# ArmingLou/seed-vc

Hardware: AMD Instinct MI355X
Metric: mel_frames_per_sec (higher is better)
Workload: dtype f16; 1 GPU; seed-uvit-tat-xlsr-tiny CFM 25 steps cfg 0.7 + HiFT, batch 64 x (P=430,S=430) per GPU; batch_per_gpu=64, global_batch=64, prompt_frames=430, diffusion_steps=25, vocoder_precision=fp16p8, lanes_per_gpu=2, parallelism=utterance-sharded x1, audio gather on rank 0

## Files before the change

### include/seedvc_hip.h

```cpp
#ifndef SEEDVC_HIP_H
#define SEEDVC_HIP_H

#include <stdint.h>

#ifdef __cplusplus
extern "C" {
#endif

#define SVC_ABI_VERSION 1

typedef struct svc_tensor_desc {
    const char* name;
    const float* data;
    int ndim;
    int64_t shape[4];
} svc_tensor_desc_t;

typedef struct svc_dit_config {
    int version;
    int hidden_dim, num_heads, depth, in_channels, content_dim, style_dim;
    int final_layer_type;
    int time_as_token, style_as_token, uvit_skip_connection, long_skip_connection, style_condition;
    int wn_hidden_dim, wn_num_layers, wn_kernel_size, wn_dilation_rate;
} svc_dit_config_t;

typedef struct svc_dit svc_dit_t;

int svc_dit_create(const svc_dit_config_t* cfg, const svc_tensor_desc_t* weights, int n_weights,
                   void* stream, svc_dit_t** out);
void svc_dit_destroy(svc_dit_t* m);

int svc_dit_set_microbatch(svc_dit_t* m, int utterances);

int svc_dit_set_fused_min_rows(svc_dit_t* m, long rows);
int svc_dit_fused_available(svc_dit_t* m);
int svc_dit_set_graphs(svc_dit_t* m, int on);

typedef struct svc_cfm_args {
    int B;
    int T;
    int P;
    const float* mu;
    const float* prompt;
    const float* style;
    const float* z;
    const int64_t* x_lens;
    const int64_t* prompt_lens;
    int n_timesteps;
    float temperature;
    float cfg_rate[2];
    int random_voice;
    float* out;
} svc_cfm_args_t;

int svc_cfm_sample(svc_dit_t* m, const svc_cfm_args_t* args, void* stream);

int svc_cfm_sample_seeded(svc_dit_t* m, const svc_cfm_args_t* args, const uint64_t* seeds, void* stream);
int svc_cfm_noise_draws(uint64_t seed, int C, int T, float* z, void* stream);

int svc_dit_forward(svc_dit_t* m, int N, int T, const float* x, const float* prompt_x, const int64_t* x_lens,
                    float t, const float* style, const float* mu, float* out, void* stream);

typedef struct svc_bigvgan_config {
    int num_mels, upsample_initial_channel, num_upsamples, num_kernels;
    int upsample_rates[8], upsample_kernel_sizes[8];
    int resblock_kernel_sizes[4], resblock_dilation_sizes[4][3];
    int use_tanh_at_final, use_bias_at_final, snake_logscale, snakebeta;
    int precision;
} svc_bigvgan_config_t;
typedef struct svc_bigvgan svc_bigvgan_t;
int svc_bigvgan_create(const svc_bigvgan_config_t* cfg, const svc_tensor_desc_t* weights, int n_weights,
                       void* stream, svc_bigvgan_t** out);
void svc_bigvgan_destroy(svc_bigvgan_t* m);
int svc_bigvgan_forward(svc_bigvgan_t* m, const float* mel, int B, int S, float* out, void* stream);
int svc_bigvgan_forward_ragged(svc_bigvgan_t* m, const float* mel, const int32_t* lens, int B, int S, float* out, void* stream);

typedef struct svc_hift_config {
    int in_channels, base_channels, nb_harmonics, sampling_rate;
    float nsf_alpha, nsf_sigma, nsf_voiced_threshold;
    int num_upsamples, upsample_rates[4], upsample_kernel_sizes[4];
    int istft_n_fft, istft_hop;
    int num_kernels, resblock_kernel_sizes[4], resblock_dilation_sizes[4][3];
    int source_resblock_kernel_sizes[4], source_resblock_dilation_sizes[4][3];
    float lrelu_slope, audio_limit;
    int f0_cond_channels;
    int precision;
} svc_hift_config_t;
typedef struct svc_hift svc_hift_t;
int svc_hift_create(const svc_hift_config_t* cfg, const svc_tensor_desc_t* weights, int n_weights,
                    void* stream, svc_hift_t** out);
void svc_hift_destroy(svc_hift_t* m);
int svc_hift_forward(svc_hift_t* m, const float* mel, const float* f0, const float* phase0, const float* noise,
                     int B, int S, float* out, float* f0_out, void* stream);
int svc_hift_forward_ragged(svc_hift_t* m, const float* mel, const int32_t* lens, const float* f0, const float* phase0,
                            const float* noise, int B, int S, float* out, float* f0_out, void* stream);
int svc_hift_forward_seeded(svc_hift_t* m, const float* mel, const int32_t* lens, const float* f0, const uint64_t* seeds, int B,
                            int S, float* out, float* f0_out, void* stream);
int svc_hift_noise_draws(uint64_t seed, int NH, long n, float* phase0, float* noise, void* stream);
int svc_bigvgan_set_microbatch(svc_bigvgan_t* m, int utterances);
int svc_hift_set_microbatch(svc_hift_t* m, int utterances);

typedef struct svc_ar_config {
    int dim, n_head, n_local_heads, head_dim, n_layer, intermediate_size, vocab_size, max_seq_len;
    float rope_base, norm_eps;
} svc_ar_config_t;
typedef struct svc_ar svc_ar_t;
int svc_ar_create(const svc_ar_config_t* cfg, const svc_tensor_desc_t* weights, int n_weights, void* stream, svc_ar_t** out);
void svc_ar_destroy(svc_ar_t* m);
int svc_ar_reset(svc_ar_t* m, void* stream);
int svc_ar_forward_generate(svc_ar_t* m, const float* x, int S, const int64_t* input_pos, const int64_t* kv_pos,
                            float* logits_out, void* stream);
int svc_ar_decode_step(svc_ar_t* m, const float* x, int set_pos, int64_t input_pos, int64_t kv_pos, float* logits_out,
                       void* stream);
int svc_ar_generate(svc_ar_t* m, const float* x_prefill, int S, const int64_t* input_pos, const int64_t* kv_pos,
                    const float* exp_noise, int max_new, int min_tokens_before_eos, float temperature, float top_p,
                    float repetition_penalty, int check_every, int32_t* tokens_out, int32_t* n_tokens, void* stream);
int svc_ar_set_max_batch(svc_ar_t* m, int max_batch, void* stream);
int svc_ar_prefill_slot(svc_ar_t* m, int slot, const float* x, int S, const int64_t* input_pos, const int64_t* kv_pos,
                        float* logits_out, void* stream);
int svc_ar_decode_step_batch(svc_ar_t* m, int B, const float* x, int set_pos, const int64_t* input_pos, const int64_t* kv_pos,
                             float* logits_out, void* stream);
int svc_ar_generate_batch(svc_ar_t* m, int B, const float* x_prefill, const int32_t* S, const int64_t* input_pos,
                          const int64_t* kv_pos, const float* exp_noise, int max_new, int min_tokens_before_eos, float temperature,
                          float top_p, float repetition_penalty, int check_every, int32_t* tokens_out, int32_t* n_tokens,
                          void* stream);
int svc_ar_generate_batch_seeded(svc_ar_t* m, int B, const float* x_prefill, const int32_t* S, const int64_t* input_pos,
                                 const int64_t* kv_pos, const uint64_t* seeds, int max_new, int min_tokens_before_eos,
                                 float temperature, float top_p, float repetition_penalty, int check_every, int32_t* tokens_out,
                                 int32_t* n_tokens, void* stream);
int svc_ar_exp_draws(svc_ar_t* m, uint64_t seed, int step0, int n_steps, float* out, void* stream);
int svc_ar_prefill_batch(svc_ar_t* m, int n, const int32_t* slots, const float* x, const int32_t* S, const int64_t* input_pos,
                         const int64_t* kv_pos, float* logits_out, void* stream);
int svc_ar_set_prefill_rows(svc_ar_t* m, int rows);
int svc_ar_prefill_passes(svc_ar_t* m);
typedef struct svc_ar_request {
    int32_t slot;
    int32_t S;
    const float* exp_noise;
    uint64_t seed;
    int32_t max_new;
    int32_t min_tokens_before_eos;
    float temperature, top_p, repetition_penalty;
    int32_t* tokens_out;
} svc_ar_request_t;
int svc_ar_admit(svc_ar_t* m, int n, const svc_ar_request_t* requests, const float* x_prefill, const int64_t* input_pos,
                 const int64_t* kv_pos, void* stream);
int svc_ar_run(svc_ar_t* m, int n_steps, int32_t* n_tokens, int32_t* done, void* stream);
int svc_ar_retire(svc_ar_t* m, int slot, void* stream);
int svc_ar_session_active(svc_ar_t* m);
int svc_ar_sample(svc_ar_t* m, const float* logits, const int32_t* prev_tokens, int n_prev, int suppress_token,
                  float temperature, float top_p, float repetition_penalty, const float* exp_noise, int32_t* idx_out,
                  float* probs_out, void* stream);

typedef struct svc_lr_config {
    int channels, in_channels, out_channels;
    int is_discrete, codebook_size;
    int n_convs;
    int interpolate;
    int has_final_conv;
    int f0_condition, n_f0_bins;
} svc_lr_config_t;
typedef struct svc_lr svc_lr_t;
int svc_lr_create(const svc_lr_config_t* cfg, const svc_tensor_desc_t* weights, int n_weights, void* stream, svc_lr_t** out);
void svc_lr_destroy(svc_lr_t* m);
int svc_lr_forward(svc_lr_t* m, const float* x, const int64_t* tokens, const int32_t* in_lens, int B, int tin_max,
                   const int32_t* ylens, int tout_max, const float* f0, const int32_t* f0_lens, int tf0_max, float* out,
                   void* stream);

int svc_v2_assemble_cond(const float* prompt_cond, const int32_t* prompt_lens, const float* cond, const int32_t* cond_lens, int B,
                         int Pmax, int Smax, int Dc, int T, float* out, void* stream);
int svc_mel_strip_prompt(const float* mel, const int32_t* prompt_lens, const int32_t* x_lens, int B, int C, int T, int Smax,
                         float pad_value, float* out, void* stream);

int svc_anti_alias_act_fwd(const void* x, void* y, const float* up12, const float* down12,
                           const float* log_alpha, const float* log_beta, int B, int C, int L, int dtype,
                           void* stream);

typedef struct svc_mel svc_mel_t;
int svc_mel_create(int n_fft, int hop, int win, int n_mels, const float* window, const float* mel_basis, void* stream,
                   svc_mel_t** out);
void svc_mel_destroy(svc_mel_t* m);
int svc_mel_frames(const svc_mel_t* m, int L);
int svc_mel_forward(svc_mel_t* m, const float* y, int B, int L, float* out, void* stream);
int svc_mel_min_len(int n_fft, int hop);
int svc_mel_forward_ragged(svc_mel_t* m, const float* y, const int32_t* lens, int B, int L, float pad_value, float* out, void* stream);

typedef struct svc_resampler svc_resampler_t;
int svc_resampler_create(int o, int n, int width, int ntaps, const int32_t* first, const float* taps, void* stream,
                         svc_resampler_t** out);
void svc_resampler_destroy(svc_resampler_t* r);
long svc_resample_len(int o, int n, long L);
long svc_resampler_tile(const svc_resampler_t* r);
int svc_resample(svc_resampler_t* r, const float* x, const int32_t* lens, int B, long L, float* out, long Lout, void* stream);

typedef struct svc_campplus_config {
    int feat_dim, embedding_size, growth_rate, bn_size, init_channels, m_channels;
    int n_blocks, block_layers[4], block_kernel[4], block_dilation[4];
    int seg_len;
} svc_campplus_config_t;
typedef struct svc_campplus svc_campplus_t;
int svc_campplus_create(const svc_campplus_config_t* cfg, const svc_tensor_desc_t* weights, int n_weights, void* stream,
                        svc_campplus_t** out);
void svc_campplus_destroy(svc_campplus_t* m);
int svc_campplus_forward(svc_campplus_t* m, const float* feat, int B, int T, float* out, void* stream);
int svc_kaldi_fbank_frames(int n_samples);
int svc_kaldi_fbank(svc_campplus_t* m, const float* wave, int n_samples, float* out, void* stream);
int svc_kaldi_fbank_ragged(svc_campplus_t* m, const float* wave, const int32_t* lens, int B, int L, int subtract_mean, float* out,
                           void* stream);
int svc_campplus_forward_ragged(svc_campplus_t* m, const float* feat, const int32_t* lens, int B, int T, float* out, void* stream);

typedef struct svc_rmvpe_config {
    int n_mels;
    int en_de_layers;
    int inter_layers;
    int n_blocks;
    int en_out_channels;
    int gru_hidden;
    int n_bins;
} svc_rmvpe_config_t;
typedef struct svc_rmvpe svc_rmvpe_t;
int svc_rmvpe_create(const svc_rmvpe_config_t* cfg, const svc_tensor_desc_t* weights, int n_weights, const float* mel_basis, void* stream,
                     svc_rmvpe_t** out);
void svc_rmvpe_destroy(svc_rmvpe_t* m);
int svc_rmvpe_frames(int n_samples);
int svc_rmvpe_min_len(void);
int svc_rmvpe_set_plane_budget(svc_rmvpe_t* m, long long bytes);
int svc_rmvpe_set_timing(svc_rmvpe_t* m, int on);
int svc_rmvpe_last_timing(svc_rmvpe_t* m, float* ms4);
int svc_rmvpe_mel(svc_rmvpe_t* m, const float* wave, const int32_t* lens, int B, int L, float* mel_out, void* stream);
int svc_rmvpe_salience(svc_rmvpe_t* m, const float* mel, const int32_t* frame_lens, int B, int T, float* out, void* stream);
int svc_rmvpe_decode(const float* salience, const int32_t* frame_lens, int B, int T, float thred, float* f0_out, void* stream);
int svc_rmvpe_f0(svc_rmvpe_t* m, const float* wave, const int32_t* lens, int B, int L, float thred, float* f0_out, void* stream);
int svc_f0_adjust(const float* f0_alt, const int32_t* alt_lens, const float* f0_ori, const int32_t* ori_lens, int B, int Talt, int Tori,
                  int auto_adjust, const float* semitones, float* out, float* medians, void* stream);

typedef struct svc_whisper_config {
    int n_mels, d_model, n_heads, n_layers, ffn_dim, max_source_positions, precision;
} svc_whisper_config_t;
typedef struct svc_whisper svc_whisper_t;

int svc_whisper_create(const svc_whisper_config_t* cfg, const svc_tensor_desc_t* weights, int n_weights, const float* mel_basis, void* stream,
                       svc_whisper_t** out);
void svc_whisper_destroy(svc_whisper_t* m);
int svc_whisper_n_windows(int P, int overlap_rows, long n_samples);
int svc_whisper_rows(int P, int overlap_rows, long n_samples);
int svc_whisper_set_window_group(svc_whisper_t* m, int windows);
int svc_whisper_set_timing(svc_whisper_t* m, int on);
int svc_whisper_last_timing(svc_whisper_t* m, float* ms4);
int svc_whisper_mel(svc_whisper_t* m, const float* wave, const int32_t* lens, int B, int L, float* feat, void* stream);
int svc_whisper_encode(svc_whisper_t* m, const float* feat, int B, float* out, void* stream);
int svc_whisper_content(svc_whisper_t* m, const float* wave, const int32_t* lens, int B, int L, int overlap_rows, float* out, int Rmax,
                        void* stream);

typedef struct svc_w2v_config {
    int conv_dim, n_conv, conv_kernel[8], conv_stride[8];
    int d_model, n_heads, n_layers, ffn_dim, pos_k, pos_groups;
    int feat_extract_norm_layer, do_stable_layer_norm, conv_bias;
    int window_samples;
    int precision;
} svc_w2v_config_t;
typedef struct svc_w2v svc_w2v_t;

int svc_w2v_create(const svc_w2v_config_t* cfg, const svc_tensor_desc_t* weights, int n_weights, void* stream, svc_w2v_t** out);
void svc_w2v_destroy(svc_w2v_t* m);
long svc_w2v_frames(const svc_w2v_config_t* cfg, long n_samples);
int svc_w2v_n_windows(const svc_w2v_config_t* cfg, int overlap_rows, long n_samples);
int svc_w2v_rows(const svc_w2v_config_t* cfg, int overlap_rows, long n_samples);
int svc_w2v_set_window_group(svc_w2v_t* m, int windows);
int svc_w2v_set_timing(svc_w2v_t* m, int on);
int svc_w2v_last_timing(svc_w2v_t* m, float* ms4);
int svc_w2v_normalize(svc_w2v_t* m, const float* wave, const int32_t* lens, int B, int L, float* out, void* stream);
int svc_w2v_features(svc_w2v_t* m, const float* wave_norm, const int32_t* lens, int B, int L, float* out, int Tmax, void* stream);
int svc_w2v_posconv(svc_w2v_t* m, const float* h, const int32_t* rows, int B, int T, float* out, void* stream);
int svc_w2v_encode(svc_w2v_t* m, const float* h, const int32_t* rows, int B, int T, float* out, void* stream);
int svc_w2v_content(svc_w2v_t* m, const float* wave, const int32_t* lens, int B, int L, int overlap_rows, float* out, int Rmax, void* stream);

#define SVC_ASTRAL_MAX_HEADS 2
typedef struct svc_astral_head_config {
    int dim, intermediate_dim;
    int n_blocks;
    int bits;
    int dw_kernel;
} svc_astral_head_config_t;
typedef struct svc_astral_config {
    svc_w2v_config_t ssl;
    int n_heads;
    svc_astral_head_config_t head[SVC_ASTRAL_MAX_HEADS];
} svc_astral_config_t;
typedef struct svc_astral svc_astral_t;

int svc_astral_create(const svc_astral_config_t* cfg, const svc_tensor_desc_t* ssl_weights, int n_ssl_weights,
                      const svc_tensor_desc_t* const* head_weights, const int* n_head_weights, void* stream, svc_astral_t** out);
void svc_astral_destroy(svc_astral_t* m);
int svc_astral_n_windows(const svc_astral_config_t* cfg, int overlap_rows, long n_samples);
int svc_astral_rows(const svc_astral_config_t* cfg, int overlap_rows, long n_samples);
int svc_astral_set_window_group(svc_astral_t* m, int windows);
int svc_astral_set_timing(svc_astral_t* m, int on);
int svc_astral_last_timing(svc_astral_t* m, float* ms4);
int svc_astral_ssl(svc_astral_t* m, const float* wave, const int32_t* lens, int B, int L, float* out, int T, void* stream);
int svc_astral_convnext(svc_astral_t* m, int head, const float* h, const int32_t* rows, int B, int T, float* x, void* stream);
int svc_astral_logits(svc_astral_t* m, int head, const float* x, const int32_t* rows, int B, int T, float* z, void* stream);
int svc_op_bsq_index(const float* z, int32_t* index, long rows, int bits, void* stream);
int svc_tokens_reduce(const int32_t* tokens, const int32_t* rows, int B, int R, int32_t* out, int32_t* counts, void* stream);
int svc_astral_tokens(svc_astral_t* m, const float* wave, const int32_t* lens, int B, int L, int overlap_rows, int32_t* tokens, int Rmax,
                      int reduce_head, int32_t* reduced, int32_t* counts, void* stream);

int svc_crossfade(float* chunk2, const float* chunk1_tail, const double* fade_in, const double* fade_out, int n,
                  void* stream);

int svc_chunks_gather_cond(const float* prompt_cond, const int32_t* prompt_lens, int U, int Pmax, const float* cond, int R,
                           const int32_t* utt, const int32_t* row0, const int32_t* rows, int N, int Dc, int T, float* mu,
                           void* stream);
int svc_chunks_assemble(const float* wave, long long stride, const int32_t* lens, const int32_t* first, const int32_t* last, int N,
                        const double* fade_in, const double* fade_out, int ov, float* out, long long out_len, void* stream);

int svc_sola_step(const float* wave, long long stride, int start, int N, float* sola_state, int max_slots, const int32_t* slots,
                  const float* fade_in, const float* fade_out, int block, int Lb, int Ls, float* out, int32_t* offsets,
                  void* stream);

int svc_rt_out(const svc_resampler_t* r,
               const float* wave, long long stride, int start, int n_in, int N,
               float* sola_state, int max_slots, const int32_t* slots,
               const int32_t* speech,
               const float* fade_in, const float* fade_out, int block, int Lb, int Ls,
               float* infer,
               float* out, int32_t* offsets, void* stream);

int svc_rt_push_tiles(int L16);
long long svc_rt_ring_floats(int max_slots, int L16);
int svc_rt_push(const svc_resampler_t* r,
                const float* block, long long stride, int Lin,
                int N, const int32_t* slots, int max_slots,
                int zc, int z16,
                float* hist,
                float* ring,
                int L16,
                float* ctx,
                void* stream);

int svc_rt_push_gated(const svc_resampler_t* r, const float* block, long long stride, int Lin, int N, const int32_t* slots,
                      int max_slots, int zc, int z16, float* hist, float* ring, int L16, float* ctx,
                      const float* gate_pow,
                      float* gate_e,
                      int32_t* gate_mask,
                      void* stream);

int svc_op_linear(const float* a, const float* w, const float* bias, float* c, int M, int N, int K, int dtype,
                  int act, void* stream);
int svc_op_conv1d(const float* x, const float* w, const float* bias, float* y, int B, int L, int Cin, int Cout,
                  int k, int dilation, int stride, int pad_left, int Lout, int pad_mode, int dtype, void* stream);
typedef struct {
    const float* x; const uint16_t* a_hi; const uint16_t* a_lo;
    const float* w; const float* bias;
    int32_t B, L, Cin, Cout, k, dilation, pad_left, Lout, dtype;
    const int32_t* seq_len;
    const float* res; const float* res2;
    float out_scale; int32_t act; float act_slope;
    int32_t c_rows, c_off;
    const float* post_a; const float* post_ib; int32_t next_p8;
    int32_t bm, force_gemm;
    float* y; uint16_t* plane_hi; uint16_t* plane_lo;
    int32_t took;
} svc_conv1d_ex_t;
int svc_op_conv1d_ex(svc_conv1d_ex_t* args, void* stream);
int svc_op_conv1d_last_took(void);
int svc_op_conv_transpose1d(const float* x, const float* w, const float* bias, float* y, int B, int L, int Cin,
                            int Cout, int k, int stride, int dtype, void* stream);
int svc_op_attention(const float* q, const float* k, const float* v, float* out, int N, int T, int H,
                     const int64_t* kv_lens_host, void* stream);
int svc_op_rmsnorm(const float* x, const float* gamma, const float* w, const float* b, int add_one, float* y,
                   int rows, int D, void* stream);
int svc_op_layernorm(const float* x, const float* gamma, const float* beta, float* y, int rows, int D, float eps, void* stream);

int svc_op_layernorm_gelu(const float* x, const float* gamma, const float* beta, float* y, int rows, int D, float eps, void* stream);

int svc_op_gemm_bench(int M, int N, int K, int dtype, int epi, int iters, int debug, float* out_ms, void* stream);
int svc_op_gemm_forms_diff(int M, int N, int K, int epi, int debug_a, int debug_b, long long* n_diff, void* stream);

int svc_prof_enable(int on);
int svc_prof_collect(double* out, int n_cls);

const char* svc_last_error(void);
int svc_abi_version(void);

#ifdef __cplusplus
}
#endif
#endif
```

### seed-vc_amd/_lib.py

```python
import ctypes as C
import os

import torch

_HERE = os.path.dirname(os.path.abspath(__file__))
LIB_PATH = os.path.join(_HERE, "libseedvc_hip.so")

EXPORTS = [
    "svc_abi_version", "svc_last_error",
    "svc_dit_create", "svc_dit_destroy", "svc_dit_set_microbatch", "svc_dit_set_fused_min_rows", "svc_dit_fused_available", "svc_dit_set_graphs", "svc_cfm_sample", "svc_dit_forward",
    "svc_cfm_sample_seeded", "svc_cfm_noise_draws", "svc_hift_forward_seeded", "svc_hift_noise_draws",
    "svc_bigvgan_create", "svc_bigvgan_destroy", "svc_bigvgan_forward", "svc_bigvgan_forward_ragged", "svc_bigvgan_set_microbatch",
    "svc_hift_create", "svc_hift_destroy", "svc_hift_forward", "svc_hift_forward_ragged", "svc_hift_set_microbatch",
    "svc_anti_alias_act_fwd",
    "svc_ar_create", "svc_ar_destroy", "svc_ar_reset", "svc_ar_forward_generate", "svc_ar_decode_step", "svc_ar_sample", "svc_ar_generate",
    "svc_ar_set_max_batch", "svc_ar_prefill_slot", "svc_ar_decode_step_batch", "svc_ar_generate_batch",
    "svc_ar_generate_batch_seeded", "svc_ar_exp_draws", "svc_v2_assemble_cond", "svc_mel_strip_prompt",
    "svc_ar_prefill_batch", "svc_ar_set_prefill_rows", "svc_ar_prefill_passes", "svc_ar_admit", "svc_ar_run", "svc_ar_retire",
    "svc_ar_session_active",
    "svc_lr_create", "svc_lr_destroy", "svc_lr_forward", "svc_crossfade",
    "svc_chunks_gather_cond", "svc_chunks_assemble", "svc_sola_step", "svc_rt_push", "svc_rt_push_tiles", "svc_rt_ring_floats",
    "svc_rt_out", "svc_rt_push_gated",
    "svc_campplus_create", "svc_campplus_destroy", "svc_campplus_forward", "svc_kaldi_fbank_frames", "svc_kaldi_fbank",
    "svc_kaldi_fbank_ragged", "svc_campplus_forward_ragged",
    "svc_mel_create", "svc_mel_destroy", "svc_mel_frames", "svc_mel_forward", "svc_mel_forward_ragged", "svc_mel_min_len",
    "svc_resampler_create", "svc_resampler_destroy", "svc_resample_len", "svc_resampler_tile", "svc_resample",
    "svc_rmvpe_create", "svc_rmvpe_destroy", "svc_rmvpe_frames", "svc_rmvpe_min_len", "svc_rmvpe_set_plane_budget", "svc_rmvpe_set_timing", "svc_rmvpe_last_timing", "svc_rmvpe_mel",
    "svc_rmvpe_salience", "svc_rmvpe_decode", "svc_rmvpe_f0", "svc_f0_adjust",
    "svc_whisper_create", "svc_whisper_destroy", "svc_whisper_n_windows", "svc_whisper_rows", "svc_whisper_set_window_group",
    "svc_whisper_set_timing", "svc_whisper_last_timing", "svc_whisper_mel", "svc_whisper_encode", "svc_whisper_content",
    "svc_w2v_create", "svc_w2v_destroy", "svc_w2v_frames", "svc_w2v_n_windows", "svc_w2v_rows", "svc_w2v_set_window_group",
    "svc_w2v_set_timing", "svc_w2v_last_timing", "svc_w2v_normalize", "svc_w2v_features", "svc_w2v_posconv", "svc_w2v_encode",
    "svc_w2v_content",
    "svc_astral_create", "svc_astral_destroy", "svc_astral_n_windows", "svc_astral_rows", "svc_astral_set_window_group",
    "svc_astral_set_timing", "svc_astral_last_timing", "svc_astral_ssl", "svc_astral_convnext", "svc_astral_logits", "svc_astral_tokens",
    "svc_op_bsq_index", "svc_tokens_reduce",
    "svc_prof_enable", "svc_prof_collect",
    "svc_op_linear", "svc_op_conv1d", "svc_op_conv1d_ex", "svc_op_conv1d_last_took", "svc_op_conv_transpose1d", "svc_op_attention", "svc_op_rmsnorm",
    "svc_op_layernorm", "svc_op_layernorm_gelu",
]


class TensorDesc(C.Structure):
    _fields_ = [("name", C.c_char_p), ("data", C.c_void_p), ("ndim", C.c_int), ("shape", C.c_int64 * 4)]


class DitConfig(C.Structure):
    _fields_ = [(n, C.c_int) for n in (
        "version", "hidden_dim", "num_heads", "depth", "in_channels", "content_dim", "style_dim",
        "final_layer_type", "time_as_token", "style_as_token", "uvit_skip_connection", "long_skip_connection",
        "style_condition", "wn_hidden_dim", "wn_num_layers", "wn_kernel_size", "wn_dilation_rate")]


class CfmArgs(C.Structure):
    _fields_ = [("B", C.c_int), ("T", C.c_int), ("P", C.c_int),
                ("mu", C.c_void_p), ("prompt", C.c_void_p), ("style", C.c_void_p), ("z", C.c_void_p),
                ("x_lens", C.POINTER(C.c_int64)), ("prompt_lens", C.POINTER(C.c_int64)),
                ("n_timesteps", C.c_int), ("temperature", C.c_float), ("cfg_rate", C.c_float * 2),
                ("random_voice", C.c_int), ("out", C.c_void_p)]


class BigVGANConfig(C.Structure):
    _fields_ = [("num_mels", C.c_int), ("upsample_initial_channel", C.c_int), ("num_upsamples", C.c_int),
                ("num_kernels", C.c_int), ("upsample_rates", C.c_int * 8), ("upsample_kernel_sizes", C.c_int * 8),
                ("resblock_kernel_sizes", C.c_int * 4), ("resblock_dilation_sizes", (C.c_int * 3) * 4),
                ("use_tanh_at_final", C.c_int), ("use_bias_at_final", C.c_int), ("snake_logscale", C.c_int),
                ("snakebeta", C.c_int), ("precision", C.c_int)]


class HiftConfig(C.Structure):
    _fields_ = [("in_channels", C.c_int), ("base_channels", C.c_int), ("nb_harmonics", C.c_int),
                ("sampling_rate", C.c_int), ("nsf_alpha", C.c_float), ("nsf_sigma", C.c_float),
                ("nsf_voiced_threshold", C.c_float), ("num_upsamples", C.c_int), ("upsample_rates", C.c_int * 4),
                ("upsample_kernel_sizes", C.c_int * 4), ("istft_n_fft", C.c_int), ("istft_hop", C.c_int),
                ("num_kernels", C.c_int), ("resblock_kernel_sizes", C.c_int * 4),
                ("resblock_dilation_sizes", (C.c_int * 3) * 4), ("source_resblock_kernel_sizes", C.c_int * 4),
                ("source_resblock_dilation_sizes", (C.c_int * 3) * 4), ("lrelu_slope", C.c_float),
                ("audio_limit", C.c_float), ("f0_cond_channels", C.c_int), ("precision", C.c_int)]


class ArConfig(C.Structure):
    _fields_ = [(n, C.c_int) for n in ("dim", "n_head", "n_local_heads", "head_dim", "n_layer", "intermediate_size",
                                       "vocab_size", "max_seq_len")] + [("rope_base", C.c_float), ("norm_eps", C.c_float)]


class ArRequest(C.Structure):
    _fields_ = [("slot", C.c_int32), ("S", C.c_int32), ("exp_noise", C.c_void_p), ("seed", C.c_uint64), ("max_new", C.c_int32),
                ("min_tokens_before_eos", C.c_int32), ("temperature", C.c_float), ("top_p", C.c_float),
                ("repetition_penalty", C.c_float), ("tokens_out", C.c_void_p)]


class CampplusConfig(C.Structure):
    _fields_ = [(n, C.c_int) for n in ("feat_dim", "embedding_size", "growth_rate", "bn_size", "init_channels", "m_channels", "n_blocks")] + \
               [("block_layers", C.c_int * 4), ("block_kernel", C.c_int * 4), ("block_dilation", C.c_int * 4), ("seg_len", C.c_int)]


class RmvpeConfig(C.Structure):
    _fields_ = [(n, C.c_int) for n in ("n_mels", "en_de_layers", "inter_layers", "n_blocks", "en_out_channels", "gru_hidden", "n_bins")]


class WhisperConfig(C.Structure):
    _fields_ = [(n, C.c_int) for n in ("n_mels", "d_model", "n_heads", "n_layers", "ffn_dim", "max_source_positions", "precision")]


class W2vConfig(C.Structure):
    _fields_ = [("conv_dim", C.c_int), ("n_conv", C.c_int), ("conv_kernel", C.c_int * 8), ("conv_stride", C.c_int * 8)] + \
               [(n, C.c_int) for n in ("d_model", "n_heads", "n_layers", "ffn_dim", "pos_k", "pos_groups", "feat_extract_norm_layer",
                                       "do_stable_layer_norm", "conv_bias", "window_samples", "precision")]


class AstralHeadConfig(C.Structure):
    _fields_ = [(n, C.c_int) for n in ("dim", "intermediate_dim", "n_blocks", "bits", "dw_kernel")]


class AstralConfig(C.Structure):
    _fields_ = [("ssl", W2vConfig), ("n_heads", C.c_int), ("head", AstralHeadConfig * 2)]


class LrConfig(C.Structure):
    _fields_ = [(n, C.c_int) for n in ("channels", "in_channels", "out_channels", "is_discrete", "codebook_size", "n_convs",
                                       "interpolate", "has_final_conv", "f0_condition", "n_f0_bins")]


class Conv1dEx(C.Structure):
    _fields_ = [("x", C.c_void_p), ("a_hi", C.c_void_p), ("a_lo", C.c_void_p), ("w", C.c_void_p), ("bias", C.c_void_p)] + \
               [(n, C.c_int32) for n in ("B", "L", "Cin", "Cout", "k", "dilation", "pad_left", "Lout", "dtype")] + \
               [("seq_len", C.POINTER(C.c_int32)), ("res", C.c_void_p), ("res2", C.c_void_p),
                ("out_scale", C.c_float), ("act", C.c_int32), ("act_slope", C.c_float), ("c_rows", C.c_int32), ("c_off", C.c_int32),
                ("post_a", C.c_void_p), ("post_ib", C.c_void_p), ("next_p8", C.c_int32), ("bm", C.c_int32), ("force_gemm", C.c_int32),
                ("y", C.c_void_p), ("plane_hi", C.c_void_p), ("plane_lo", C.c_void_p), ("took", C.c_int32)]


_lib = None


def lib():
    global _lib
    if _lib is None:
        if not os.path.exists(LIB_PATH):
            raise ImportError(f"{LIB_PATH} is missing: run `python -c 'import __graft_entry__ as g; g.build()'` "
                              f"(hipcc --offload-arch=gfx950); there is no CPU fallback")
        l = C.CDLL(LIB_PATH)
        l.svc_last_error.restype = C.c_char_p
        if l.svc_abi_version() != 1:
            raise ImportError("libseedvc_hip.so ABI version mismatch")
        l.svc_sola_step.argtypes = [C.c_void_p, C.c_longlong, C.c_int, C.c_int, C.c_void_p, C.c_int, C.POINTER(C.c_int32),
                                    C.c_void_p, C.c_void_p, C.c_int, C.c_int, C.c_int, C.c_void_p, C.c_void_p, C.c_void_p]
        l.svc_rt_push.argtypes = [C.c_void_p, C.c_void_p, C.c_longlong, C.c_int, C.c_int, C.POINTER(C.c_int32), C.c_int, C.c_int, C.c_int,
                                  C.c_void_p, C.c_void_p, C.c_int, C.c_void_p, C.c_void_p]
        l.svc_rt_push_gated.argtypes = l.svc_rt_push.argtypes[:-1] + [C.POINTER(C.c_float), C.c_void_p, C.c_void_p, C.c_void_p]
        l.svc_rt_out.argtypes = [C.c_void_p, C.c_void_p, C.c_longlong, C.c_int, C.c_int, C.c_int, C.c_void_p, C.c_int, C.POINTER(C.c_int32),
                                 C.POINTER(C.c_int32), C.c_void_p, C.c_void_p, C.c_int, C.c_int, C.c_int, C.c_void_p, C.c_void_p,
                                 C.c_void_p, C.c_void_p]
        l.svc_rt_push_tiles.argtypes = [C.c_int]
        l.svc_rt_ring_floats.argtypes = [C.c_int, C.c_int]
        l.svc_rt_ring_floats.restype = C.c_longlong
        l.svc_hift_forward_ragged.argtypes = [C.c_void_p, C.c_void_p, C.POINTER(C.c_int32), C.c_void_p, C.c_void_p, C.c_void_p,
                                              C.c_int, C.c_int, C.c_void_p, C.c_void_p, C.c_void_p]
        l.svc_op_conv1d_ex.argtypes = [C.POINTER(Conv1dEx), C.c_void_p]
        l.svc_cfm_sample_seeded.argtypes = [C.c_void_p, C.POINTER(CfmArgs), C.POINTER(C.c_uint64), C.c_void_p]
        l.svc_cfm_noise_draws.argtypes = [C.c_uint64, C.c_int, C.c_int, C.c_void_p, C.c_void_p]
        l.svc_hift_forward_seeded.argtypes = [C.c_void_p, C.c_void_p, C.POINTER(C.c_int32), C.c_void_p, C.POINTER(C.c_uint64),
                                              C.c_int, C.c_int, C.c_void_p, C.c_void_p, C.c_void_p]
        l.svc_hift_noise_draws.argtypes = [C.c_uint64, C.c_int, C.c_long, C.c_void_p, C.c_void_p, C.c_void_p]
        l.svc_mel_forward_ragged.argtypes = [C.c_void_p, C.c_void_p, C.POINTER(C.c_int32), C.c_int, C.c_int, C.c_float, C.c_void_p,
                                             C.c_void_p]
        l.svc_kaldi_fbank_ragged.argtypes = [C.c_void_p, C.c_void_p, C.POINTER(C.c_int32), C.c_int, C.c_int, C.c_int, C.c_void_p,
                                             C.c_void_p]
        l.svc_campplus_forward_ragged.argtypes = [C.c_void_p, C.c_void_p, C.POINTER(C.c_int32), C.c_int, C.c_int, C.c_void_p, C.c_void_p]
        i32p = C.POINTER(C.c_int32)
        l.svc_resampler_create.argtypes = [C.c_int, C.c_int, C.c_int, C.c_int, i32p, C.POINTER(C.c_float), C.c_void_p, C.POINTER(C.c_void_p)]
        l.svc_resampler_destroy.argtypes = [C.c_void_p]
        l.svc_resampler_destroy.restype = None
        l.svc_resample_len.argtypes = [C.c_int, C.c_int, C.c_long]
        l.svc_resample_len.restype = C.c_long
        l.svc_resampler_tile.argtypes = [C.c_void_p]
        l.svc_resampler_tile.restype = C.c_long
        l.svc_resample.argtypes = [C.c_void_p, C.c_void_p, i32p, C.c_int, C.c_long, C.c_void_p, C.c_long, C.c_void_p]
        l.svc_rmvpe_create.argtypes = [C.POINTER(RmvpeConfig), C.c_void_p, C.c_int, C.c_void_p, C.c_void_p, C.POINTER(C.c_void_p)]
        l.svc_rmvpe_set_plane_budget.argtypes = [C.c_void_p, C.c_longlong]
        l.svc_rmvpe_set_timing.argtypes = [C.c_void_p, C.c_int]
        l.svc_rmvpe_last_timing.argtypes = [C.c_void_p, C.POINTER(C.c_float)]
        l.svc_rmvpe_mel.argtypes = [C.c_void_p, C.c_void_p, i32p, C.c_int, C.c_int, C.c_void_p, C.c_void_p]
        l.svc_rmvpe_salience.argtypes = [C.c_void_p, C.c_void_p, i32p, C.c_int, C.c_int, C.c_void_p, C.c_void_p]
        l.svc_rmvpe_decode.argtypes = [C.c_void_p, i32p, C.c_int, C.c_int, C.c_float, C.c_void_p, C.c_void_p]
        l.svc_rmvpe_f0.argtypes = [C.c_void_p, C.c_void_p, i32p, C.c_int, C.c_int, C.c_float, C.c_void_p, C.c_void_p]
        l.svc_f0_adjust.argtypes = [C.c_void_p, i32p, C.c_void_p, i32p, C.c_int, C.c_int, C.c_int, C.c_int, C.POINTER(C.c_float),
                                    C.c_void_p, C.c_void_p, C.c_void_p]
        l.svc_whisper_create.argtypes = [C.POINTER(WhisperConfig), C.c_void_p, C.c_int, C.c_void_p, C.c_void_p, C.POINTER(C.c_void_p)]
        l.svc_whisper_destroy.argtypes = [C.c_void_p]
        l.svc_whisper_n_windows.argtypes = [C.c_int, C.c_int, C.c_long]
        l.svc_whisper_rows.argtypes = [C.c_int, C.c_int, C.c_long]
        l.svc_whisper_set_window_group.argtypes = [C.c_void_p, C.c_int]
        l.svc_whisper_set_timing.argtypes = [C.c_void_p, C.c_int]
        l.svc_whisper_last_timing.argtypes = [C.c_void_p, C.POINTER(C.c_float)]
        l.svc_whisper_mel.argtypes = [C.c_void_p, C.c_void_p, i32p, C.c_int, C.c_int, C.c_void_p, C.c_void_p]
        l.svc_whisper_encode.argtypes = [C.c_void_p, C.c_void_p, C.c_int, C.c_void_p, C.c_void_p]
        l.svc_whisper_content.argtypes = [C.c_void_p, C.c_void_p, i32p, C.c_int, C.c_int, C.c_int, C.c_void_p, C.c_int, C.c_void_p]
        cp = C.POINTER(W2vConfig)
        l.svc_w2v_create.argtypes = [cp, C.c_void_p, C.c_int, C.c_void_p, C.POINTER(C.c_void_p)]
        l.svc_w2v_destroy.argtypes = [C.c_void_p]
        l.svc_w2v_frames.argtypes = [cp, C.c_long]
        l.svc_w2v_frames.restype = C.c_long
        l.svc_w2v_n_windows.argtypes = [cp, C.c_int, C.c_long]
        l.svc_w2v_rows.argtypes = [cp, C.c_int, C.c_long]
        l.svc_w2v_set_window_group.argtypes = [C.c_void_p, C.c_int]
        l.svc_w2v_set_timing.argtypes = [C.c_void_p, C.c_int]
        l.svc_w2v_last_timing.argtypes = [C.c_void_p, C.POINTER(C.c_float)]
        l.svc_w2v_normalize.argtypes = [C.c_void_p, C.c_void_p, i32p, C.c_int, C.c_int, C.c_void_p, C.c_void_p]
        l.svc_w2v_features.argtypes = [C.c_void_p, C.c_void_p, i32p, C.c_int, C.c_int, C.c_void_p, C.c_int, C.c_void_p]
        l.svc_w2v_posconv.argtypes = [C.c_void_p, C.c_void_p, i32p, C.c_int, C.c_int, C.c_void_p, C.c_void_p]
        l.svc_w2v_encode.argtypes = [C.c_void_p, C.c_void_p, i32p, C.c_int, C.c_int, C.c_void_p, C.c_void_p]
        l.svc_w2v_content.argtypes = [C.c_void_p, C.c_void_p, i32p, C.c_int, C.c_int, C.c_int, C.c_void_p, C.c_int, C.c_void_p]
        ap = C.POINTER(AstralConfig)
        l.svc_astral_create.argtypes = [ap, C.c_void_p, C.c_int, C.POINTER(C.c_void_p), C.POINTER(C.c_int), C.c_void_p, C.POINTER(C.c_void_p)]
        l.svc_astral_destroy.argtypes = [C.c_void_p]
        l.svc_astral_n_windows.argtypes = [ap, C.c_int, C.c_long]
        l.svc_astral_rows.argtypes = [ap, C.c_int, C.c_long]
        l.svc_astral_set_window_group.argtypes = [C.c_void_p, C.c_int]
        l.svc_astral_set_timing.argtypes = [C.c_void_p, C.c_int]
        l.svc_astral_last_timing.argtypes = [C.c_void_p, C.POINTER(C.c_float)]
        l.svc_astral_ssl.argtypes = [C.c_void_p, C.c_void_p, i32p, C.c_int, C.c_int, C.c_void_p, C.c_int, C.c_void_p]
        l.svc_astral_convnext.argtypes = [C.c_void_p, C.c_int, C.c_void_p, i32p, C.c_int, C.c_int, C.c_void_p, C.c_void_p]
        l.svc_astral_logits.argtypes = [C.c_void_p, C.c_int, C.c_void_p, i32p, C.c_int, C.c_int, C.c_void_p, C.c_void_p]
        l.svc_op_bsq_index.argtypes = [C.c_void_p, C.c_void_p, C.c_long, C.c_int, C.c_void_p]
        l.svc_tokens_reduce.argtypes = [C.c_void_p, i32p, C.c_int, C.c_int, C.c_void_p, C.c_void_p, C.c_void_p]
        l.svc_astral_tokens.argtypes = [C.c_void_p, C.c_void_p, i32p, C.c_int, C.c_int, C.c_int, C.c_void_p, C.c_int, C.c_int, C.c_void_p,
                                        C.c_void_p, C.c_void_p]
        l.svc_op_layernorm_gelu.argtypes = [C.c_void_p, C.c_void_p, C.c_void_p, C.c_void_p, C.c_int, C.c_int, C.c_float, C.c_void_p]
        l.svc_op_layernorm.argtypes = [C.c_void_p, C.c_void_p, C.c_void_p, C.c_void_p, C.c_int, C.c_int, C.c_float, C.c_void_p]
        _lib = l
    return _lib


def check(rc):
    if rc != 0:
        raise RuntimeError("seedvc_hip: " + (lib().svc_last_error() or b"unknown error").decode())


def stream_ptr():
    return C.c_void_p(torch.cuda.current_stream().cuda_stream)


def ptr(t):
    return C.c_void_p(t.data_ptr()) if t is not None else C.c_void_p(0)


def f32c(t, device=None):
    t = t.detach()
    if device is not None:
        t = t.to(device)
    return t.to(torch.float32).contiguous()


def make_descs(state_dict, device):
    keep, items = [], []
    for k, v in state_dict.items():
        if not torch.is_tensor(v) or not (v.is_floating_point()):
            continue
        if v.dim() > 4:
            continue
        t = f32c(v, device)
        keep.append(t)
        items.append((k, t))
    arr = (TensorDesc * len(items))()
    for i, (k, t) in enumerate(items):
        kb = k.encode()
        keep.append(kb)
        arr[i].name = kb
        arr[i].data = t.data_ptr()
        arr[i].ndim = t.dim()
        for j in range(4):
            arr[i].shape[j] = t.shape[j] if j < t.dim() else 1
    return arr, len(items), keep


def int_list(v):
    return [int(x) for x in (v.tolist() if torch.is_tensor(v) else v)]


def i64_host(values):
    if values is None:
        return None
    vals = [int(v) for v in values]
    return (C.c_int64 * len(vals))(*vals)


def i32_host(values):
    return (C.c_int32 * len(values))(*values)


def seed_ints(seeds, n, what):
    vals = int_list(seeds)
    if len(vals) != n:
        raise ValueError(f"{what}: {len(vals)} seeds for {n} utterances")
    for v in vals:
        if not 0 <= v < 1 << 64:
            raise ValueError(f"{what}: seed {v} is outside [0, 2^64)")
    return vals


def seeds_host(seeds, n, what):
    return (C.c_uint64 * n)(*seed_ints(seeds, n, what))
```

### seed-vc_amd/cfm.py

```python
import ctypes as C

import torch

from . import _lib
from .specs import dit_config


def _cfg_struct(cfg):
    c = _lib.DitConfig()
    c.version = cfg["version"]
    c.hidden_dim, c.num_heads, c.depth = cfg["D"], cfg["H"], cfg["L"]
    c.in_channels, c.content_dim, c.style_dim = cfg["C"], cfg["Dc"], cfg["style_dim"]
    c.final_layer_type = 1 if cfg["head"] == "wavenet" else 0
    c.time_as_token, c.style_as_token = int(cfg["time_as_token"]), int(cfg["style_as_token"])
    c.uvit_skip_connection, c.long_skip_connection = int(cfg["uvit"]), int(cfg["long_skip"])
    c.style_condition = int(cfg["style_condition"])
    c.wn_hidden_dim = cfg.get("wn_dim", 0)
    c.wn_num_layers = cfg.get("wn_layers", 0)
    c.wn_kernel_size = cfg.get("wn_kernel", 0)
    c.wn_dilation_rate = cfg.get("wn_dilation", 1)
    return c


class Estimator:

    def __init__(self, cfg, state_dict, device="cuda:0"):
        self.cfg = cfg
        self.device = torch.device(device)
        self.in_channels = cfg["C"]
        self._h = C.c_void_p()
        with torch.cuda.device(self.device):
            descs, n, keep = _lib.make_descs(state_dict, self.device)
            cs = _cfg_struct(cfg)
            _lib.check(_lib.lib().svc_dit_create(C.byref(cs), descs, n, _lib.stream_ptr(), C.byref(self._h)))
            torch.cuda.current_stream().synchronize()
        del keep

    def setup_caches(self, max_batch_size=1, max_seq_length=8192):
        return None

    def set_microbatch(self, n):
        _lib.check(_lib.lib().svc_dit_set_microbatch(self._h, int(n)))

    def set_fused_min_rows(self, rows):
        _lib.check(_lib.lib().svc_dit_set_fused_min_rows(self._h, C.c_long(int(rows))))

    def set_graphs(self, on):
        _lib.check(_lib.lib().svc_dit_set_graphs(self._h, int(bool(on))))

    @property
    def fused_available(self):
        return bool(_lib.lib().svc_dit_fused_available(self._h))

    def __call__(self, x, prompt_x, x_lens, t, style, cond, mask_content=False):
        N, Cc, T = x.shape
        with torch.cuda.device(self.device):
            x, prompt_x, style, cond = (_lib.f32c(a, self.device) for a in (x, prompt_x, style, cond))
            out = torch.empty_like(x)
            tval = float(t.reshape(-1)[0]) if torch.is_tensor(t) else float(t)
            lens = None
            if x_lens is not None:
                xl = _lib.int_list(x_lens)
                if len(xl) == 1 and N > 1:
                    xl = xl * N
                lens = _lib.i64_host(xl)
            _lib.check(_lib.lib().svc_dit_forward(self._h, N, T, _lib.ptr(x), _lib.ptr(prompt_x), lens,
                                                  C.c_float(tval), _lib.ptr(style), _lib.ptr(cond), _lib.ptr(out),
                                                  _lib.stream_ptr()))
        return out

    def close(self):
        if self._h:
            _lib.lib().svc_dit_destroy(self._h)
            self._h = C.c_void_p()

    def __del__(self):
        try:
            self.close()
        except Exception:
            pass


class CFM:

    def __init__(self, cfg, state_dict, device="cuda:0"):
        self.cfg = cfg
        self.estimator = Estimator(cfg, state_dict, device)
        self.in_channels = cfg["C"]
        self.device = self.estimator.device

    @classmethod
    def from_preset(cls, name, state_dict, device="cuda:0", **overrides):
        return cls(dit_config(name, **overrides), state_dict, device)

    @torch.inference_mode()
    def inference(self, mu, x_lens, prompt, style, f0=None, n_timesteps=10, temperature=1.0,
                  inference_cfg_rate=0.5, random_voice=False, z=None, prompt_lens=None, seeds=None):
        if seeds is not None and z is not None:
            raise ValueError("CFM.inference: give seeds or z, not both")
        seeds_keep = _lib.seeds_host(seeds, mu.size(0), "CFM.inference") if seeds is not None else None
        if self.cfg["version"] == 2 and not isinstance(f0, (type(None), torch.Tensor)):
            n_timesteps, f0 = f0, None
        B, T = mu.size(0), mu.size(1)
        dev = self.device
        with torch.cuda.device(dev):
            mu, prompt, style = (_lib.f32c(a, dev) for a in (mu, prompt, style))
            if seeds is None:
                if z is None:
                    z = torch.randn([B, self.in_channels, T], device=dev)
                z = _lib.f32c(z, dev)
            out = torch.empty(B, self.in_channels, T, device=dev, dtype=torch.float32)
            a = _lib.CfmArgs()
            a.B, a.T, a.P = B, T, prompt.size(-1)
            a.mu, a.prompt, a.style, a.out = (t.data_ptr() for t in (mu, prompt, style, out))
            a.z = z.data_ptr() if z is not None else None
            xl = None
            if x_lens is not None:
                xl = _lib.int_list(x_lens)
                if len(xl) == 1 and B > 1:
                    xl = xl * B
            lens_keep = _lib.i64_host(xl)
            plens_keep = _lib.i64_host(prompt_lens)
            a.x_lens = lens_keep
            a.prompt_lens = plens_keep
            a.n_timesteps = int(n_timesteps)
            a.temperature = float(temperature)
            if isinstance(inference_cfg_rate, (list, tuple)):
                a.cfg_rate[0], a.cfg_rate[1] = float(inference_cfg_rate[0]), float(inference_cfg_rate[1])
            else:
                a.cfg_rate[0], a.cfg_rate[1] = float(inference_cfg_rate), float(inference_cfg_rate)
            a.random_voice = int(bool(random_voice))
            if seeds_keep is not None:
                _lib.check(_lib.lib().svc_cfm_sample_seeded(self.estimator._h, C.byref(a), seeds_keep, _lib.stream_ptr()))
            else:
                _lib.check(_lib.lib().svc_cfm_sample(self.estimator._h, C.byref(a), _lib.stream_ptr()))
        return out

    @torch.inference_mode()
    def noise_draws(self, seed, T):
        seed = _lib.seeds_host([seed], 1, "CFM.noise_draws")[0]
        with torch.cuda.device(self.device):
            z = torch.empty(1, self.in_channels, int(T), device=self.device, dtype=torch.float32)
            _lib.check(_lib.lib().svc_cfm_noise_draws(seed, self.in_channels, int(T), _lib.ptr(z), _lib.stream_ptr()))
        return z
```

### seed-vc_amd/csrc/common.h

```cpp
#pragma once
#include <atomic>
#include <hip/hip_runtime.h>
#include <stdint.h>
#include <stdio.h>
#include <string>

namespace svc {

typedef _Float16 half_t;
typedef _Float16 half8 __attribute__((ext_vector_type(8)));
typedef _Float16 half4 __attribute__((ext_vector_type(4)));
typedef _Float16 half2v __attribute__((ext_vector_type(2)));
typedef float float4v __attribute__((ext_vector_type(4)));
typedef unsigned int u32x4 __attribute__((ext_vector_type(4)));

void set_error(const std::string& msg);
const char* get_error();

#define SVC_CHECK_HIP(expr)                                                                  \
    do {                                                                                     \
        hipError_t _e = (expr);                                                              \
        if (_e != hipSuccess) {                                                              \
            svc::set_error(std::string(#expr) + ": " + hipGetErrorString(_e) + " at " + __FILE__ + \
                           ":" + std::to_string(__LINE__));                                  \
            return 1;                                                                        \
        }                                                                                    \
    } while (0)

#define SVC_REQUIRE(cond, msg)                                                               \
    do {                                                                                     \
        if (!(cond)) {                                                                       \
            svc::set_error(std::string("requirement failed: ") + #cond + " -- " + (msg));    \
            return 1;                                                                        \
        }                                                                                    \
    } while (0)

__device__ __forceinline__ float sin_sq(float x) {
    const float n = rintf(x * 0.318309886183790672f);
    float r = fmaf(n, -3.140625f, x);
    r = fmaf(n, -9.67502593994140625e-4f, r);
    r = fmaf(n, -1.509957990978376e-7f, r);
    const float r2 = r * r;
    float p = fmaf(r2, 2.6348154733568663e-06f, -0.00019822761532850564f);
    p = fmaf(p, r2, 0.008333242498338223f);
    p = fmaf(p, r2, -0.1666666567325592f);
    const float sn = fmaf(p * r2, r, r);
    return sn * sn;
}

struct DeviceState {
    int device = -1;
    void* zero_page = nullptr;
    std::atomic<unsigned long long> kconv_attr{0};
    std::atomic<bool> fused_attr{false};
};
DeviceState* device_state();
int current_device();

enum { PROF_KGEMM_F16 = 0, PROF_KGEMM_F32 = 1, PROF_ATTN = 2, PROF_FUSED = 3, PROF_N = 4 };
bool prof_enabled();
void prof_begin(int cls, hipStream_t st);
void prof_end(int cls, double flops, double bytes, hipStream_t st, unsigned long long tag = 0);

template <int MAXA, int DPT>
__device__ __forceinline__ void wait_tiles(int ahead) {
    static_assert(MAXA * DPT <= 63, "vmcnt is a 6-bit counter");
    if constexpr (MAXA <= 0) {
        asm volatile("s_waitcnt vmcnt(0)" ::: "memory");
    } else {
        if (ahead >= MAXA) asm volatile("s_waitcnt vmcnt(%0)" ::"n"(MAXA * DPT) : "memory");
        else wait_tiles<MAXA - 1, DPT>(ahead);
    }
}

__device__ __forceinline__ float act_apply(float v, int act, float slope);
__device__ __forceinline__ uint4 pack8(const float* v) {
    half8 h;
#pragma unroll
    for (int j = 0; j < 8; ++j) h[j] = (half_t)v[j];
    return *reinterpret_cast<uint4*>(&h);
}

static inline int cdiv(long a, long b) { return (int)((a + b - 1) / b); }
static inline long round_up(long a, long b) { return (a + b - 1) / b * b; }

constexpr int KG_MAX_TAPS = 48;

enum { KG_PAD_ZERO = 0, KG_PAD_REFLECT = 1, KG_PAD_CLAMP = 2 };
enum { KG_ACT_NONE = 0, KG_ACT_SILU = 1, KG_ACT_ELU = 2, KG_ACT_LRELU = 3, KG_ACT_TANH = 4, KG_ACT_ABS = 5,
       KG_ACT_CLAMP = 6 , KG_ACT_SIGMOID = 7,
       KG_ACT_GELU = 8  };
enum {
    KG_EPI_STORE = 0,
    KG_EPI_SWIGLU = 1,
    KG_EPI_TANHSIG = 2,
    KG_EPI_QKV_ROPE = 3,
    KG_EPI_STORE_GELU = 4,
};

__device__ __forceinline__ float gelu_erf(float v) { return 0.5f * v * (1.0f + erff(v * 0.70710678118654752f)); }

__device__ __forceinline__ float act_apply(float v, int act, float slope) {
    switch (act) {
        case KG_ACT_SILU: return v / (1.0f + __expf(-v));
        case KG_ACT_ELU: return v > 0.f ? v : (expm1f(v));
        case KG_ACT_LRELU: return v > 0.f ? v : v * slope;
        case KG_ACT_TANH: return tanhf(v);
        case KG_ACT_ABS: return fabsf(v);
        case KG_ACT_CLAMP: return fminf(fmaxf(v, -slope), slope);
        case KG_ACT_SIGMOID: return 1.0f / (1.0f + __expf(-v));
        default: return v;
    }
}
__device__ __forceinline__ void act_apply8(float* v, int act, float slope) {
#define SVC_ACT8(A)                                                     \
    case A:                                                             \
        _Pragma("unroll") for (int j = 0; j < 8; ++j) v[j] = act_apply(v[j], A, slope); \
        break;
    switch (act) {
        SVC_ACT8(KG_ACT_SILU)
        SVC_ACT8(KG_ACT_ELU)
        SVC_ACT8(KG_ACT_LRELU)
        SVC_ACT8(KG_ACT_TANH)
        SVC_ACT8(KG_ACT_ABS)
        SVC_ACT8(KG_ACT_CLAMP)
        SVC_ACT8(KG_ACT_SIGMOID)
        default: break;
    }
#undef SVC_ACT8
}

struct KGemmParams {
    const void* a_ptr[KG_MAX_TAPS];
    long a_ld[KG_MAX_TAPS];
    int a_shift[KG_MAX_TAPS];
    int a_ktiles[KG_MAX_TAPS];
    int n_taps;
    int Lout, a_seq_rows, a_off, a_stride, a_len, pad_mode;
    int reflect_min;
    const int* seq_len;
    const void* zero_page;
    float prof_flop_scale;
    int debug;
    int group_n;
    const void* w;
    long ldw;
    int M, N;
    int c_seq_rows, c_off;
    float* c32; long ldc32;
    half_t* c16; long ldc16;
    const float* post_a; const float* post_ib; int post_n; half_t* c16_lo;
    const float* bias;
    const float* rowvec; long ld_rowvec;
    const float* gate;   long ld_gate;
    const float* res;    long ldres;
    const float* res2;   long ldres2;
    float out_scale;
    int act; float act_slope;
    int post_relu;
    int vec_ok;
    const float* rope;
    int rope_D;
    float q_scale;
    half_t* vt; long vt_seq_stride; long vt_ld;
    int vt_mode;
};

int kgemm_launch(const KGemmParams& p, int dtype , int epi, hipStream_t st);
int kgemm_big_launch(const KGemmParams& p, int epi, hipStream_t st);

struct KConvParams {
    const void* a_hi; const void* a_lo;
    const void* w; long ldw;
    const float* bias;
    int B, Lin, Lout, N, cin_pad, k, dil, pad_left, nsub;
    int c_seq_rows, c_off;
    float* c32; long ldc32;
    half_t* c16; half_t* c16_lo; long ldc16;
    const float* post_a; const float* post_ib; int post_n;
    const float* res; long ldres;
    const float* res2; long ldres2;
    float out_scale;
    int act; float act_slope;
    const void* zero_page;
    int w8_exp;
    int c16_lo_fmt;
    const int* seq_len;
    int bm;
    int* took;
};
bool kconv_enabled();
int kconv_launch(const KConvParams& p, hipStream_t st);
__device__ __forceinline__ unsigned lo_pair_p8(float hi_as_float, float lo) {
    const float a = __builtin_amdgcn_fmed3f(hi_as_float, -448.f, 448.f), b = __builtin_amdgcn_fmed3f(lo * 2048.f, -448.f, 448.f);
    return (unsigned)__builtin_amdgcn_cvt_pk_fp8_f32(a, b, 0, false) & 0xffffu;
}
int kconv_pack_p8(const float* src, unsigned short* dst, int n0, int n1, int n2, long s0, long s1, long s2, long d0, long d1, long d2,
                  const float* scale, int* exp_out, hipStream_t st);

struct PanelParams {
    int M;
    int Lout, seq_rows, row_off;
    const half_t* wstream;
    int n_slots;
    float eps;
    int do_post;
    const half_t* ao;
    float* x;
    const float* gate_a; const float* gate_f;
    const float* g_ffn; const float* w_f; const float* b_f; int add_one;
    int I;
    half_t* c16;
    int do_skip;
    const half_t* skip_in; const float* bskip;
    int do_qkv;
    const float* g_attn; const float* w_a; const float* b_a;
    const float* rope; float q_scale;
    half_t* qk; half_t* vt; long vt_seq_stride; long vt_ld; int vt_mode;
    int do_final;
    const float* g_fin; const float* w_fin; const float* b_fin; half_t* n16;
};
bool fused_supported(int D, int I);
long fused_stream_halfs(int D, int I, bool post, bool skip, bool qkv);
long fused_pack_stream(half_t* dst, int D, int I, const float* wo, const float* w1, const float* w3, const float* w2,
                       const float* wskip, const float* wqkv, hipStream_t st);
int fused_panel_launch(const PanelParams& p, int D, bool gated, hipStream_t st);

struct AttnParams {
    const half_t* q; const half_t* k; long ld_qk;
    const half_t* vt; long vt_seq_stride; long vt_ld;
    half_t* out; long ld_out;
    int n_seq, H, seq_rows, Tq;
    int q_start;
    const int* kv_len; int kv_len_const;
    int vt_perm;
    int qt_form;
    float* out32;
};
__host__ __device__ inline int vt_perm_pos(int pos) {
    return (pos & ~31) | (((pos >> 2) & 3) << 3) | (((pos >> 4) & 1) << 2) | (pos & 3);
}
__host__ __device__ inline int vt_perm_pos16(int pos) {
    return (pos & ~12) | ((pos & 4) << 1) | ((pos & 8) >> 1);
}
__host__ __device__ inline int vt_pos(int pos, int mode) {
    return mode == 2 ? vt_perm_pos16(pos) : (mode == 1 ? vt_perm_pos(pos) : pos);
}
int attention_vt_mode(int n_seq, int H, int Tq);
int attention_launch(const AttnParams& p, hipStream_t st);
int attention_permute_vt(half_t* vt, long rows, long vt_ld, int mode, hipStream_t st);

int rmsnorm_mod_launch(const float* x, long ldx, half_t* y, long ldy, const float* gamma,
                       const float* w, const float* b, long ld_wb, int add_one,
                       int rows, int D, int seq_rows, float eps, hipStream_t st);
int layernorm_mod_launch(const float* x, long ldx, half_t* y, long ldy, const float* scale,
                         const float* shift, int rows, int D, float eps, hipStream_t st);

}
```

### seed-vc_amd/csrc/dit.hip

```cpp
#include <math.h>
#include <string.h>

#include <algorithm>
#include <vector>

#include "model_util.h"
#include "noise.h"

using namespace svc;

namespace {
constexpr int MAX_STREAMS = 3;
constexpr int ROPE_POS = 8192;

float bf16_round(float f) {
    uint32_t u;
    memcpy(&u, &f, 4);
    u = (u + 0x7FFF + ((u >> 16) & 1)) & 0xFFFF0000u;
    memcpy(&f, &u, 4);
    return f;
}

std::vector<float> linspace01(int n) {
    std::vector<float> v(n);
    const float step = 1.0f / (float)(n - 1);
    const int half = n / 2;
    for (int i = 0; i < n; ++i) v[i] = i < half ? 0.0f + step * (float)i : 1.0f - step * (float)(n - 1 - i);
    return v;
}
}

struct svc_dit {
    svc_dit_config_t cfg;
    int D, H, L, C, Dc, S, I, W, NL, WK, npre, C16, C32;
    bool v2, wavenet, adaptive_blocks;
    Arena wts, ws;
    struct StepGraph {
        std::vector<float> key;
        hipGraphExec_t exec = nullptr;
        int seen = 0;
    };
    std::vector<StepGraph> graphs;
    hipStream_t cap_stream = nullptr;
    int use_graphs = 0;
    void drop_graphs() {
        for (auto& g : graphs) if (g.exec) (void)hipGraphExecDestroy(g.exec);
        graphs.clear();
    }
    PinnedRing staging;
    hipStream_t create_stream;
    int device = -1;

    struct Layer {
        half_t *wqkv, *wo, *w13, *w2, *wskip;
        float *bskip, *g_attn, *g_ffn;
        half_t* stream = nullptr;
        int stream_slots = 0;
    };
    half_t* stream_pre = nullptr;
    int stream_pre_slots = 0;
    bool fused_ok = false;
    long fused_min_rows = 10240;
    std::vector<Layer> layers;
    float* g_final;
    std::vector<int> emit, recv;
    float *te_w0, *te_b0, *te_w2, *te_b2, *te_freqs;
    float *te2_w0, *te2_b0, *te2_w2, *te2_b2, *te2_freqs;
    float *mod_w, *mod_b;
    int mod_n;
    int mod_layer_n;
    half_t* w_merge_x;
    float* w_stat;
    float* stat_const;
    float* w_style_merge;
    float *style_in_w, *style_in_b;
    half_t *head_wa, *head_w2;
    float *head_b0, *head_b2;
    half_t *w_longskip, *w_conv1, *w_resproj, *w_fl, *w_conv2;
    float *b_longskip, *b_conv1, *b_resproj, *b_fl, *b_conv2;
    float *wn_cond_w, *wn_cond_b, *fl_mod_w, *fl_mod_b;
    std::vector<half_t*> wn_in, wn_res, wn_skip;
    std::vector<float*> wn_res_b, wn_skip_b;
    half_t* wn_tail = nullptr;
    float* b_tail = nullptr;
    long acts_stride = 0;
    float* rope;

    int cap_streams = 0, cap_B = 0, cap_T = 0, cap_steps = 0;
    int seq_rows = 0, vt_ld = 0;
    float *x32, *xin, *st_term, *v32, *u_rowvec, *tok_style, *prompt32, *wnx32, *flin32;
    half_t *x16, *n16, *qk16, *vt, *ao16, *ff16, *h16, *hm16, *xr16, *wnx16, *acts16, *fl16, *fo16;
    std::vector<half_t*> skip16;
    int *d_kvlen, *d_convlen, *d_plen;
    unsigned long long* d_seeds = nullptr;
    int* d_convlen_w = nullptr;
    int win0 = 0;
    float *d_tvals, *d_tfeat, *d_th, *d_t1, *d_t1s, *d_t2, *d_mod, *d_gcond, *d_flmod, *d_stylevec;
    int microbatch = 0;

    int pack(const StateDict& sd, hipStream_t st);
    int reserve(int n_streams, int B, int T, int n_steps, hipStream_t st);
    int tables(const std::vector<float>& tvals, hipStream_t st);
    int statics(int n_streams, const int (*flags)[3], int B, int T, const float* mu, const float* style_dev,
                hipStream_t st);
    int run_group(const svc_cfm_args_t* a, const uint64_t* seeds, int b0, int nb, int n_streams, const int (*flags)[3],
                  const std::vector<float>& tvals, const std::vector<float>& dts, float c0, float ca, float cb,
                  int stream_a, int stream_b, hipStream_t st);
    int sample(const svc_cfm_args_t* a, const uint64_t* seeds, hipStream_t st);
    int body(int n_streams, int B, int T, int step, hipStream_t st);
    int body_fused(int n_streams, int B, int T, int step, hipStream_t st);
    int head(int n_streams, int B, int T, int step, hipStream_t st);
};

namespace {

int pack_block(int dtype, const float* src, long src_ld, long src_col, int N, int K, void* dst, long ldw, long dst_col,
               long dst_row0, long dst_row_step, const float* scale, hipStream_t st) {
    return pack_any(dtype, src + src_col, dst, dst_row0 * ldw + dst_col, N, 1, K, src_ld, 0, 1, dst_row_step * ldw, 0, 1,
                    scale, st);
}

float* copy_vec(Arena& ar, const float* src, long n, hipStream_t st) {
    float* d = ar.alloc_n<float>(n, st);
    if (!d) return nullptr;
    if (hipMemcpyAsync(d, src, n * sizeof(float), hipMemcpyDeviceToDevice, st) != hipSuccess) {
        set_error("hipMemcpyAsync failed");
        return nullptr;
    }
    return d;
}

}

#define GETW(var, name, ...)                                              \
    const svc_tensor_desc_t* var = sd.get(name);                          \
    if (require_shape(var, name, {__VA_ARGS__})) return 1;

int svc_dit::pack(const StateDict& sd, hipStream_t st) {
    const long Dp = round_up(D, 128);
    auto new16 = [&](long rows, long ld) { return wts.alloc_n<half_t>(round_up(rows, 128) * ld, st); };
    layers.resize(L);
    for (int i = 0; i < L; ++i) {
        const std::string p = "transformer.layers." + std::to_string(i) + ".";
        Layer& ly = layers[i];
        GETW(wqkv, p + "attention.wqkv.weight", 3 * D, D);
        GETW(wo, p + "attention.wo.weight", D, D);
        GETW(w1, p + "feed_forward.w1.weight", I, D);
        GETW(w3, p + "feed_forward.w3.weight", I, D);
        GETW(w2, p + "feed_forward.w2.weight", D, I);
        ly.wqkv = new16(3 * D, D);
        ly.wo = new16(D, D);
        ly.w13 = new16(2 * I, D);
        ly.w2 = new16(D, I);
        if (!ly.wqkv || !ly.wo || !ly.w13 || !ly.w2) return 1;
        if (pack_block(0, wqkv->data, D, 0, 3 * D, D, ly.wqkv, D, 0, 0, 1, nullptr, st)) return 1;
        if (pack_block(0, wo->data, D, 0, D, D, ly.wo, D, 0, 0, 1, nullptr, st)) return 1;
        if (pack_block(0, w1->data, D, 0, I, D, ly.w13, D, 0, 0, 2, nullptr, st)) return 1;
        if (pack_block(0, w3->data, D, 0, I, D, ly.w13, D, 0, 1, 2, nullptr, st)) return 1;
        if (pack_block(0, w2->data, I, 0, D, I, ly.w2, I, 0, 0, 1, nullptr, st)) return 1;
        const std::string an = v2 ? p + "attention_norm.norm.weight" : p + "attention_norm.norm.weight";
        const std::string fn = v2 ? p + "ffn_norm.weight" : p + "ffn_norm.norm.weight";
        GETW(ga, an, D);
        GETW(gf, fn, D);
        ly.g_attn = copy_vec(wts, ga->data, D, st);
        ly.g_ffn = copy_vec(wts, gf->data, D, st);
        if (!ly.g_attn || !ly.g_ffn) return 1;
        ly.wskip = nullptr;
        ly.bskip = nullptr;
        if (std::find(recv.begin(), recv.end(), i) != recv.end()) {
            GETW(ws_, p + "skip_in_linear.weight", D, 2 * D);
            GETW(bs_, p + "skip_in_linear.bias", D);
            ly.wskip = new16(D, 2 * D);
            if (!ly.wskip) return 1;
            if (pack_block(0, ws_->data, 2 * D, 0, D, 2 * D, ly.wskip, 2 * D, 0, 0, 1, nullptr, st)) return 1;
            ly.bskip = copy_vec(wts, bs_->data, D, st);
            if (!ly.bskip) return 1;
        }
    }
    {
        GETW(gn, "transformer.norm.norm.weight", D);
        g_final = copy_vec(wts, gn->data, D, st);
        if (!g_final) return 1;
    }
    fused_ok = fused_supported(D, I);
    if (fused_ok) {
        auto W = [&](const std::string& k) { return sd.get(k)->data; };
        const int slot_halfs = (D / 16) * 512;
        for (int i = 0; i < L; ++i) {
            const std::string p = "transformer.layers." + std::to_string(i) + ".";
            const bool last = i == L - 1;
            const bool nskip = !last && layers[i + 1].wskip != nullptr;
            const std::string pn = "transformer.layers." + std::to_string(i + 1) + ".";
            const long halfs = fused_stream_halfs(D, I, true, nskip, !last);
            layers[i].stream = wts.alloc_n<half_t>(halfs, st);
            if (!layers[i].stream) return 1;
            const long wr = fused_pack_stream(layers[i].stream, D, I, W(p + "attention.wo.weight"), W(p + "feed_forward.w1.weight"),
                                              W(p + "feed_forward.w3.weight"), W(p + "feed_forward.w2.weight"),
                                              nskip ? W(pn + "skip_in_linear.weight") : nullptr,
                                              last ? nullptr : W(pn + "attention.wqkv.weight"), st);
            if (wr != halfs) { set_error("fused stream packing failed"); return 1; }
            layers[i].stream_slots = (int)(halfs / slot_halfs);
        }
        const long halfs = fused_stream_halfs(D, I, false, false, true);
        stream_pre = wts.alloc_n<half_t>(halfs, st);
        if (!stream_pre) return 1;
        if (fused_pack_stream(stream_pre, D, I, nullptr, nullptr, nullptr, nullptr, nullptr,
                              W("transformer.layers.0.attention.wqkv.weight"), st) != halfs) { set_error("fused stream packing failed"); return 1; }
        stream_pre_slots = (int)(halfs / slot_halfs);
    }
    mod_layer_n = adaptive_blocks ? (v2 ? 6 * D : 4 * D) : 0;
    mod_n = L * mod_layer_n + 2 * D;
    mod_w = wts.alloc_n<float>((long)mod_n * D, st);
    mod_b = wts.alloc_n<float>(mod_n, st);
    if (!mod_w || !mod_b) return 1;
    auto put_mod = [&](const std::string& wname, const std::string& bname, int rows, long row0) -> int {
        GETW(w, wname, rows, D);
        GETW(b, bname, rows);
        if (pack_f32_launch(w->data, mod_w + row0 * D, rows, 1, D, D, 0, 1, D, 0, 1, nullptr, st)) return 1;
        SVC_CHECK_HIP(hipMemcpyAsync(mod_b + row0, b->data, rows * sizeof(float), hipMemcpyDeviceToDevice, st));
        return 0;
    };
    for (int i = 0; i < L && adaptive_blocks; ++i) {
        const std::string p = "transformer.layers." + std::to_string(i) + ".";
        if (v2) {
            if (put_mod(p + "attention_norm.linear.weight", p + "attention_norm.linear.bias", 6 * D, (long)i * mod_layer_n)) return 1;
        } else {
            if (put_mod(p + "attention_norm.project_layer.weight", p + "attention_norm.project_layer.bias", 2 * D, (long)i * mod_layer_n)) return 1;
            if (put_mod(p + "ffn_norm.project_layer.weight", p + "ffn_norm.project_layer.bias", 2 * D, (long)i * mod_layer_n + 2 * D)) return 1;
        }
    }
    if (v2) {
        if (put_mod("transformer.norm.linear.weight", "transformer.norm.linear.bias", 2 * D, (long)L * mod_layer_n)) return 1;
    } else {
        if (put_mod("transformer.norm.project_layer.weight", "transformer.norm.project_layer.bias", 2 * D, (long)L * mod_layer_n)) return 1;
    }
    auto put_temb = [&](const std::string& p, int dim, float** w0, float** b0, float** w2, float** b2, float** fr) -> int {
        GETW(a, p + ".mlp.0.weight", dim, 256);
        GETW(b, p + ".mlp.0.bias", dim);
        GETW(c, p + ".mlp.2.weight", dim, dim);
        GETW(d, p + ".mlp.2.bias", dim);
        *w0 = copy_vec(wts, a->data, (long)dim * 256, st);
        *b0 = copy_vec(wts, b->data, dim, st);
        *w2 = copy_vec(wts, c->data, (long)dim * dim, st);
        *b2 = copy_vec(wts, d->data, dim, st);
        if (!*w0 || !*b0 || !*w2 || !*b2) return 1;
        if (const auto* f = sd.get(p + ".freqs")) {
            if (require_shape(f, p + ".freqs", {128})) return 1;
            *fr = copy_vec(wts, f->data, 128, st);
        } else {
            std::vector<float> h(128);
            for (int i = 0; i < 128; ++i) h[i] = expf(-logf(10000.0f) * (float)i / 128.0f);
            *fr = wts.alloc_n<float>(128, st);
            if (*fr) SVC_CHECK_HIP(hipMemcpyAsync(*fr, h.data(), 512, hipMemcpyHostToDevice, st));
            SVC_CHECK_HIP(hipStreamSynchronize(st));
        }
        return *fr ? 0 : 1;
    };
    if (put_temb("t_embedder", D, &te_w0, &te_b0, &te_w2, &te_b2, &te_freqs)) return 1;

    const bool style_in_merge = !v2 && cfg.style_condition && !cfg.style_as_token;
    const int Kin = D + 2 * C + (style_in_merge ? S : 0);
    GETW(wm, "cond_x_merge_linear.weight", D, Kin);
    GETW(bm, "cond_x_merge_linear.bias", D);
    GETW(wcp, "cond_projection.weight", D, Dc);
    GETW(bcp, "cond_projection.bias", D);
    w_merge_x = new16(D, C16);
    if (!w_merge_x) return 1;
    if (pack_block(0, wm->data, Kin, 0, D, C, w_merge_x, C16, 0, 0, 1, nullptr, st)) return 1;
    const long Ks = C32 + Dc;
    w_stat = wts.alloc_n<float>(Dp * Ks, st);
    stat_const = wts.alloc_n<float>(D, st);
    if (!w_stat || !stat_const) return 1;
    if (pack_block(1, wm->data, Kin, C, D, C, w_stat, Ks, 0, 0, 1, nullptr, st)) return 1;
    {
        float* wcpT = ws.alloc_n<float>((long)Dc * D, st);
        if (!wcpT) return 1;
        if (pack_f32_launch(wcp->data, wcpT, D, 1, Dc, Dc, 0, 1, 1, 0, D, nullptr, st)) return 1;
        if (small_linear_launch(wm->data + 2 * C, Kin, wcpT, D, nullptr, w_stat + C32, Ks, D, Dc, D, KG_ACT_NONE, st)) return 1;
        if (small_linear_launch(bcp->data, D, wm->data + 2 * C, Kin, bm->data, stat_const, D, 1, D, D, KG_ACT_NONE, st)) return 1;
    }
    w_style_merge = nullptr;
    if (style_in_merge) {
        w_style_merge = wts.alloc_n<float>((long)D * S, st);
        if (!w_style_merge) return 1;
        if (pack_f32_launch(wm->data + 2 * C + D, w_style_merge, D, 1, S, Kin, 0, 1, S, 0, 1, nullptr, st)) return 1;
    }
    style_in_w = style_in_b = nullptr;
    if (v2 || cfg.style_as_token) {
        GETW(sw, "style_in.weight", D, S);
        GETW(sb, "style_in.bias", D);
        style_in_w = copy_vec(wts, sw->data, (long)D * S, st);
        style_in_b = copy_vec(wts, sb->data, D, st);
        if (!style_in_w || !style_in_b) return 1;
    }
    if (!wavenet) {
        GETW(a, "final_mlp.0.weight", D, D);
        GETW(b, "final_mlp.0.bias", D);
        GETW(c, "final_mlp.2.weight", C, D);
        GETW(d, "final_mlp.2.bias", C);
        head_wa = new16(D, D);
        head_w2 = new16(C, D);
        if (!head_wa || !head_w2) return 1;
        if (pack_block(0, a->data, D, 0, D, D, head_wa, D, 0, 0, 1, nullptr, st)) return 1;
        if (pack_block(0, c->data, D, 0, C, D, head_w2, D, 0, 0, 1, nullptr, st)) return 1;
        head_b0 = copy_vec(wts, b->data, D, st);
        head_b2 = copy_vec(wts, d->data, C, st);
        if (!head_b0 || !head_b2) return 1;
    } else {
        if (put_temb("t_embedder2", W, &te2_w0, &te2_b0, &te2_w2, &te2_b2, &te2_freqs)) return 1;
        if (cfg.long_skip_connection) {
            GETW(a, "skip_linear.weight", D, D + C);
            GETW(b, "skip_linear.bias", D);
            w_longskip = new16(D, D + C16);
            if (!w_longskip) return 1;
            if (pack_block(0, a->data, D + C, 0, D, D + C, w_longskip, D + C16, 0, 0, 1, nullptr, st)) return 1;
            b_longskip = copy_vec(wts, b->data, D, st);
            if (!b_longskip) return 1;
        }
        GETW(c1w, "conv1.weight", W, D);
        GETW(c1b, "conv1.bias", W);
        GETW(rpw, "res_projection.weight", W, D);
        GETW(rpb, "res_projection.bias", W);
        GETW(c2w, "conv2.weight", C, W, 1);
        GETW(c2b, "conv2.bias", C);
        w_conv1 = new16(W, D);
        w_resproj = new16(W, D);
        w_conv2 = new16(C, W);
        if (!w_conv1 || !w_resproj || !w_conv2) return 1;
        if (pack_block(0, c1w->data, D, 0, W, D, w_conv1, D, 0, 0, 1, nullptr, st)) return 1;
        if (pack_block(0, rpw->data, D, 0, W, D, w_resproj, D, 0, 0, 1, nullptr, st)) return 1;
        if (pack_block(0, c2w->data, W, 0, C, W, w_conv2, W, 0, 0, 1, nullptr, st)) return 1;
        b_conv1 = copy_vec(wts, c1b->data, W, st);
        b_resproj = copy_vec(wts, rpb->data, W, st);
        b_conv2 = copy_vec(wts, c2b->data, C, st);
        if (!b_conv1 || !b_resproj || !b_conv2) return 1;
        {
            WeightSrc fl;
            if (resolve_weight(sd, "final_layer.linear", wts, st, &fl)) return 1;
            if (require_shape(fl.desc, "final_layer.linear.weight", {W, W})) return 1;
            GETW(flb, "final_layer.linear.bias", W);
            GETW(mw, "final_layer.adaLN_modulation.1.weight", 2 * W, W);
            GETW(mb, "final_layer.adaLN_modulation.1.bias", 2 * W);
            w_fl = new16(W, W);
            if (!w_fl) return 1;
            if (pack_block(0, fl.v, W, 0, W, W, w_fl, W, 0, 0, 1, fl.scale, st)) return 1;
            b_fl = copy_vec(wts, flb->data, W, st);
            fl_mod_w = copy_vec(wts, mw->data, 2L * W * W, st);
            fl_mod_b = copy_vec(wts, mb->data, 2 * W, st);
            if (!b_fl || !fl_mod_w || !fl_mod_b) return 1;
        }
        {
            WeightSrc cl;
            if (resolve_weight(sd, "wavenet.cond_layer.conv.conv", wts, st, &cl)) return 1;
            if (require_shape(cl.desc, "wavenet.cond_layer.conv.conv.weight", {2L * W * NL, W, 1})) return 1;
            GETW(clb, "wavenet.cond_layer.conv.conv.bias", 2L * W * NL);
            wn_cond_w = wts.alloc_n<float>(2L * W * NL * W, st);
            wn_cond_b = wts.alloc_n<float>(2L * W * NL, st);
            float* tmp_b = ws.alloc_n<float>(2L * W * NL, st);
            if (!wn_cond_w || !wn_cond_b || !tmp_b) return 1;
            wn_in.resize(NL);
            wn_res.assign(NL, nullptr);
            wn_skip.resize(NL);
            wn_res_b.assign(NL, nullptr);
            wn_skip_b.resize(NL);
            for (int i = 0; i < NL; ++i) {
                const std::string li = std::to_string(i);
                for (int half = 0; half < 2; ++half) {
                    const long src_row0 = 2L * W * i + (long)half * W;
                    if (pack_f32_launch(cl.v + src_row0 * W, wn_cond_w + (2L * W * i + half) * W, W, 1, W, W, 0, 1, 2L * W, 0, 1,
                                        cl.scale ? cl.scale + src_row0 : nullptr, st)) return 1;
                    if (pack_f32_launch(clb->data + src_row0, tmp_b + 2L * W * i + half, W, 1, 1, 1, 0, 0, 2, 0, 0, nullptr, st)) return 1;
                }
                WeightSrc in;
                if (resolve_weight(sd, "wavenet.in_layers." + li + ".conv.conv", wts, st, &in)) return 1;
                if (require_shape(in.desc, "wavenet.in_layers." + li + ".conv.conv.weight", {2L * W, W, WK})) return 1;
                GETW(inb, "wavenet.in_layers." + li + ".conv.conv.bias", 2L * W);
                wn_in[i] = new16(2 * W, (long)WK * W);
                float* inb_perm = ws.alloc_n<float>(2L * W, st);
                if (!wn_in[i] || !inb_perm) return 1;
                for (int half = 0; half < 2; ++half) {
                    if (pack_f16_launch(in.v + (long)half * W * W * WK, wn_in[i] + (long)half * WK * W, W, WK, W,
                                        (long)W * WK, 1, WK, 2L * WK * W, W, 1, in.scale ? in.scale + (long)half * W : nullptr, st)) return 1;
                    if (pack_f32_launch(inb->data + (long)half * W, inb_perm + half, W, 1, 1, 1, 0, 0, 2, 0, 0, nullptr, st)) return 1;
                }
                {
                    float* dst = wn_cond_b + 2L * W * i;
                    if (add_rowvec_launch(dst, tmp_b + 2L * W * i, 0, inb_perm, 1, 2 * W, st)) return 1;
                }
                WeightSrc rs;
                const int rs_out = i < NL - 1 ? 2 * W : W;
                if (resolve_weight(sd, "wavenet.res_skip_layers." + li + ".conv.conv", wts, st, &rs)) return 1;
                if (require_shape(rs.desc, "wavenet.res_skip_layers." + li + ".conv.conv.weight", {rs_out, W, 1})) return 1;
                GETW(rsb, "wavenet.res_skip_layers." + li + ".conv.conv.bias", rs_out);
                const long skip_row0 = i < NL - 1 ? W : 0;
                if (i < NL - 1) {
                    wn_res[i] = new16(W, W);
                    if (!wn_res[i]) return 1;
                    if (pack_block(0, rs.v, W, 0, W, W, wn_res[i], W, 0, 0, 1, rs.scale, st)) return 1;
                    wn_res_b[i] = copy_vec(wts, rsb->data, W, st);
                    if (!wn_res_b[i]) return 1;
                }
                wn_skip[i] = new16(W, W);
                if (!wn_skip[i]) return 1;
                if (pack_block(0, rs.v + skip_row0 * W, W, 0, W, W, wn_skip[i], W, 0, 0, 1,
                               rs.scale ? rs.scale + skip_row0 : nullptr, st)) return 1;
                wn_skip_b[i] = copy_vec(wts, rsb->data + skip_row0, W, st);
                if (!wn_skip_b[i]) return 1;
            }
        }
    }
    if (wavenet) {
        const long Kt = (long)NL * W + D;
        wn_tail = new16(W, Kt);
        b_tail = wts.alloc_n<float>(W, st);
        if (!wn_tail || !b_tail) return 1;
        for (int i = 0; i < NL; ++i)
            SVC_CHECK_HIP(hipMemcpy2DAsync(wn_tail + (long)i * W, Kt * 2, wn_skip[i], (size_t)W * 2, (size_t)W * 2, W, hipMemcpyDeviceToDevice, st));
        SVC_CHECK_HIP(hipMemcpy2DAsync(wn_tail + (long)NL * W, Kt * 2, w_resproj, (size_t)D * 2, (size_t)D * 2, W, hipMemcpyDeviceToDevice, st));
        if (add_rowvec_launch(b_tail, b_resproj, 0, wn_skip_b[0], 1, W, st)) return 1;
        for (int i = 1; i < NL; ++i)
            if (add_rowvec_launch(b_tail, b_tail, 0, wn_skip_b[i], 1, W, st)) return 1;
    }
    {
        std::vector<float> tab((size_t)ROPE_POS * 32 * 2);
        for (int i = 0; i < 32; ++i) {
            const float e = (float)(2 * i) / 64.0f;
            const float f = 1.0f / powf(10000.0f, e);
            for (int t = 0; t < ROPE_POS; ++t) {
                const float a = (float)t * f;
                float c = (float)cos((double)a), s = (float)sin((double)a);
                if (v2) { c = bf16_round(c); s = bf16_round(s); }
                tab[((size_t)t * 32 + i) * 2] = c;
                tab[((size_t)t * 32 + i) * 2 + 1] = s;
            }
        }
        rope = wts.alloc_n<float>(tab.size(), st);
        if (!rope) return 1;
        SVC_CHECK_HIP(hipMemcpyAsync(rope, tab.data(), tab.size() * 4, hipMemcpyHostToDevice, st));
        SVC_CHECK_HIP(hipStreamSynchronize(st));
    }
    SVC_CHECK_HIP(hipStreamSynchronize(st));
    ws.release();
    return 0;
}

int svc_dit::reserve(int n_streams, int B, int T, int n_steps, hipStream_t st) {
    if (n_streams <= cap_streams && B <= cap_B && T <= cap_T && n_steps <= cap_steps) {
        seq_rows = (int)round_up(T + npre, 8);
        vt_ld = (int)round_up(seq_rows, 64);
        return 0;
    }
    SVC_CHECK_HIP(hipStreamSynchronize(st));
    drop_graphs();
    ws.release();
    cap_streams = std::max(cap_streams, n_streams);
    cap_B = std::max(cap_B, B);
    cap_T = std::max(cap_T, T);
    cap_steps = std::max(cap_steps, n_steps);
    const long rows_seq = round_up(cap_T + npre, 8);
    const long nseq = (long)cap_streams * cap_B;
    const long M = nseq * rows_seq;
    const long vtl = round_up(rows_seq, 64);
    x32 = ws.alloc_n<float>((long)cap_B * rows_seq * C16, st);
    x16 = ws.alloc_n<half_t>(M * C16, st);
    xin = ws.alloc_n<float>(M * D, st);
    st_term = ws.alloc_n<float>(M * D, st);
    v32 = ws.alloc_n<float>(M * C16, st);
    u_rowvec = ws.alloc_n<float>(nseq * D, st);
    tok_style = ws.alloc_n<float>(nseq * D, st);
    prompt32 = ws.alloc_n<float>((long)cap_B * rows_seq * C32, st);
    n16 = ws.alloc_n<half_t>(M * D, st);
    qk16 = ws.alloc_n<half_t>(M * 2 * D, st);
    vt = ws.alloc_n<half_t>(nseq * D * vtl, st);
    ao16 = ws.alloc_n<half_t>(M * D, st);
    ff16 = ws.alloc_n<half_t>(M * I, st);
    h16 = ws.alloc_n<half_t>(M * D, st);
    skip16.assign(emit.size(), nullptr);
    for (auto& p : skip16) {
        p = ws.alloc_n<half_t>(M * D, st);
        if (!p) return 1;
    }
    if (!x32 || !x16 || !xin || !st_term || !v32 || !u_rowvec || !tok_style || !prompt32 || !n16 || !qk16 || !vt ||
        !ao16 || !ff16 || !h16)
        return 1;
    hm16 = xr16 = wnx16 = acts16 = fl16 = fo16 = nullptr;
    wnx32 = flin32 = nullptr;
    if (!wavenet) {
        hm16 = ws.alloc_n<half_t>(M * D, st);
        if (!hm16) return 1;
    } else {
        xr16 = ws.alloc_n<half_t>(M * D, st);
        wnx32 = ws.alloc_n<float>(M * W, st);
        wnx16 = ws.alloc_n<half_t>(M * W, st);
        acts_stride = M * W;
        acts16 = ws.alloc_n<half_t>((long)NL * acts_stride, st);
        flin32 = ws.alloc_n<float>(M * W, st);
        fl16 = ws.alloc_n<half_t>(M * W, st);
        fo16 = ws.alloc_n<half_t>(M * W, st);
        if (!xr16 || !wnx32 || !wnx16 || !acts16 || !flin32 || !fl16 || !fo16) return 1;
    }
    d_kvlen = ws.alloc_n<int>(nseq, st);
    d_convlen = ws.alloc_n<int>(nseq, st);
    d_convlen_w = ws.alloc_n<int>(nseq, st);
    d_plen = ws.alloc_n<int>(cap_B, st);
    d_seeds = ws.alloc_n<unsigned long long>(cap_B, st);
    const long Sx = cap_steps;
    d_tvals = ws.alloc_n<float>(Sx, st);
    d_tfeat = ws.alloc_n<float>(Sx * 256, st);
    d_th = ws.alloc_n<float>(Sx * std::max(D, W), st);
    d_t1 = ws.alloc_n<float>(Sx * D, st);
    d_t1s = ws.alloc_n<float>(Sx * D, st);
    d_t2 = ws.alloc_n<float>(Sx * std::max(W, 1), st);
    d_mod = ws.alloc_n<float>(Sx * mod_n, st);
    d_gcond = ws.alloc_n<float>(Sx * std::max(2L * W * NL, 1L), st);
    d_flmod = ws.alloc_n<float>(Sx * std::max(2 * W, 1), st);
    d_stylevec = ws.alloc_n<float>((long)cap_B * D, st);
    if (!d_kvlen || !d_convlen || !d_convlen_w || !d_plen || !d_seeds || !d_tvals || !d_tfeat || !d_th || !d_t1 || !d_t1s || !d_t2 || !d_mod ||
        !d_gcond || !d_flmod || !d_stylevec)
        return 1;
    seq_rows = (int)round_up(T + npre, 8);
    vt_ld = (int)round_up(seq_rows, 64);
    SVC_CHECK_HIP(hipStreamSynchronize(st));
    return 0;
}

int svc_dit::tables(const std::vector<float>& tvals, hipStream_t st) {
    const int n = (int)tvals.size();
    {
        float* h = reinterpret_cast<float*>(staging.acquire(n * sizeof(float)));
        if (!h) return 1;
        memcpy(h, tvals.data(), n * sizeof(float));
        SVC_CHECK_HIP(hipMemcpyAsync(d_tvals, h, n * sizeof(float), hipMemcpyHostToDevice, st));
        if (staging.commit(st)) return 1;
    }
    if (timestep_feat_launch(d_tvals, te_freqs, d_tfeat, n, st)) return 1;
    if (small_linear_launch(d_tfeat, 256, te_w0, 256, te_b0, d_th, D, n, D, 256, KG_ACT_SILU, st)) return 1;
    if (small_linear_launch(d_th, D, te_w2, D, te_b2, d_t1, D, n, D, D, KG_ACT_NONE, st)) return 1;
    if (silu_launch(d_t1, d_t1s, (long)n * D, st)) return 1;
    if (small_linear_launch(v2 ? d_t1s : d_t1, D, mod_w, D, mod_b, d_mod, mod_n, n, mod_n, D, KG_ACT_NONE, st)) return 1;
    if (wavenet) {
        if (small_linear_launch(d_tfeat, 256, te2_w0, 256, te2_b0, d_th, W, n, W, 256, KG_ACT_SILU, st)) return 1;
        if (small_linear_launch(d_th, W, te2_w2, W, te2_b2, d_t2, W, n, W, W, KG_ACT_NONE, st)) return 1;
        if (small_linear_launch(d_t2, W, wn_cond_w, W, wn_cond_b, d_gcond, 2L * W * NL, n, 2 * W * NL, W, KG_ACT_NONE, st)) return 1;
        if (small_linear_launch(d_t1s, D, fl_mod_w, W, fl_mod_b, d_flmod, 2 * W, n, 2 * W, W, KG_ACT_NONE, st)) return 1;
    }
    return 0;
}


namespace {
KGemmParams gemm_base(int M, int N, int Lout) {
    KGemmParams p;
    memset(&p, 0, sizeof(p));
    p.M = M;
    p.N = N;
    p.Lout = Lout;
    p.a_seq_rows = Lout;
    p.c_seq_rows = Lout;
    p.a_stride = 1;
    p.a_len = Lout;
    p.n_taps = 1;
    p.vec_ok = 1;
    return p;
}
}

int svc_dit::body(int n_streams, int B, int T, int step, hipStream_t st) {
    const int nseq = n_streams * B;
    const int M = nseq * seq_rows;
    const float* mod = d_mod + (long)step * mod_n;
    if (prefix_rows_launch(xin, nseq, seq_rows, D, npre, T + npre, d_t1 + (long)step * D, tok_style,
                           cfg.time_as_token ? 1 : 0, st)) return 1;
    {
        KGemmParams p = gemm_base(nseq * T, D, T);
        p.a_ptr[0] = x16; p.a_ld[0] = C16; p.a_ktiles[0] = C16 / 64;
        p.a_seq_rows = seq_rows; p.a_len = T;
        p.w = w_merge_x; p.ldw = C16;
        p.c_seq_rows = seq_rows; p.c_off = npre;
        p.c32 = xin; p.ldc32 = D;
        p.res = st_term; p.ldres = D;
        if (kgemm_launch(p, 0, KG_EPI_STORE, st)) return 1;
    }
    if (fused_ok && (long)M >= fused_min_rows) {
        if (body_fused(n_streams, B, T, step, st)) return 1;
        return head(n_streams, B, T, step, st);
    }
    const int Lw = seq_rows - win0;
    auto gemm_win = [&](int N) {
        KGemmParams p = gemm_base(nseq * Lw, N, Lw);
        p.a_seq_rows = seq_rows; p.c_seq_rows = seq_rows;
        p.a_off = win0; p.c_off = win0;
        return p;
    };
    size_t emit_i = 0;
    std::vector<int> skip_stack;
    for (int i = 0; i < L; ++i) {
        const bool tail_only = i == L - 1 && win0 > 0;

        const Layer& ly = layers[i];
        const float* lmod = adaptive_blocks ? mod + (long)i * mod_layer_n : nullptr;
        const bool is_recv = ly.wskip != nullptr;
        if (is_recv) {
            const int src = skip_stack.back();
            skip_stack.pop_back();
            KGemmParams p = gemm_base(M, D, seq_rows);
            p.n_taps = 2;
            p.a_ptr[0] = h16; p.a_ld[0] = D; p.a_ktiles[0] = D / 64;
            p.a_ptr[1] = skip16[src]; p.a_ld[1] = D; p.a_ktiles[1] = D / 64;
            p.w = ly.wskip; p.ldw = 2 * D;
            p.bias = ly.bskip;
            p.c32 = xin; p.ldc32 = D;
            if (kgemm_launch(p, 0, KG_EPI_STORE, st)) return 1;
        }
        const float *w_a = nullptr, *b_a = nullptr, *gate_a = nullptr, *w_f = nullptr, *b_f = nullptr, *gate_f = nullptr;
        if (lmod) {
            if (v2) {
                b_a = lmod; w_a = lmod + D; gate_a = lmod + 2 * D;
                b_f = lmod + 3 * D; w_f = lmod + 4 * D; gate_f = lmod + 5 * D;
            } else {
                w_a = lmod; b_a = lmod + D; w_f = lmod + 2 * D; b_f = lmod + 3 * D;
            }
        }
        if (rmsnorm_mod_launch(xin, D, n16, D, ly.g_attn, w_a, b_a, 0, v2 ? 1 : 0, M, D, seq_rows, 1e-5f, st)) return 1;
        {
            KGemmParams p = gemm_base(M, 3 * D, seq_rows);
            p.a_ptr[0] = n16; p.a_ld[0] = D; p.a_ktiles[0] = D / 64;
            p.w = ly.wqkv; p.ldw = D;
            p.c16 = qk16; p.ldc16 = 2 * D;
            p.rope = rope; p.rope_D = D; p.q_scale = 0.125f * 1.4426950408889634f;
            p.vt = vt; p.vt_seq_stride = (long)D * vt_ld; p.vt_ld = vt_ld; p.vt_mode = attention_vt_mode(nseq, H, seq_rows);
            if (kgemm_launch(p, 0, KG_EPI_QKV_ROPE, st)) return 1;
        }
        {
            AttnParams a;
            memset(&a, 0, sizeof(a));
            a.q = qk16; a.k = qk16 + D; a.ld_qk = 2 * D;
            a.vt = vt; a.vt_seq_stride = (long)D * vt_ld; a.vt_ld = vt_ld; a.vt_perm = attention_vt_mode(nseq, H, seq_rows);
            a.out = ao16; a.ld_out = D;
            a.n_seq = nseq; a.H = H; a.seq_rows = seq_rows; a.Tq = seq_rows;
            a.q_start = tail_only ? win0 : 0;
            a.kv_len = d_kvlen;
            if (attention_launch(a, st)) return 1;
        }
        {
            KGemmParams p = tail_only ? gemm_win(D) : gemm_base(M, D, seq_rows);
            p.a_ptr[0] = ao16; p.a_ld[0] = D; p.a_ktiles[0] = D / 64;
            p.w = ly.wo; p.ldw = D;
            p.gate = gate_a; p.ld_gate = 0;
            p.res = xin; p.ldres = D;
            p.c32 = xin; p.ldc32 = D;
            if (kgemm_launch(p, 0, KG_EPI_STORE, st)) return 1;
        }
        if (rmsnorm_mod_launch(xin, D, n16, D, ly.g_ffn, w_f, b_f, 0, v2 ? 1 : 0, M, D, seq_rows, 1e-5f, st)) return 1;
        {
            KGemmParams p = tail_only ? gemm_win(2 * I) : gemm_base(M, 2 * I, seq_rows);
            p.a_ptr[0] = n16; p.a_ld[0] = D; p.a_ktiles[0] = D / 64;
            p.w = ly.w13; p.ldw = D;
            p.c16 = ff16; p.ldc16 = I;
            if (kgemm_launch(p, 0, KG_EPI_SWIGLU, st)) return 1;
        }
        {
            KGemmParams p = tail_only ? gemm_win(D) : gemm_base(M, D, seq_rows);
            p.a_ptr[0] = ff16; p.a_ld[0] = I; p.a_ktiles[0] = I / 64;
            p.w = ly.w2; p.ldw = I;
            p.gate = gate_f; p.ld_gate = 0;
            p.res = xin; p.ldres = D;
            p.c32 = xin; p.ldc32 = D;
            const bool is_emit = std::find(emit.begin(), emit.end(), i) != emit.end();
            const bool next_recv = i + 1 < L && layers[i + 1].wskip != nullptr;
            if (is_emit) {
                p.c16 = skip16[emit_i]; p.ldc16 = D;
                skip_stack.push_back((int)emit_i);
                ++emit_i;
            } else if (next_recv) {
                p.c16 = h16; p.ldc16 = D;
            }
            if (kgemm_launch(p, 0, KG_EPI_STORE, st)) return 1;
        }
    }
    {
        const float* fm = mod + (long)L * mod_layer_n;
        const float* w = fm;
        const float* b = fm + D;
        if (rmsnorm_mod_launch(xin, D, n16, D, g_final, w, b, 0, v2 ? 1 : 0, M, D, seq_rows, 1e-5f, st)) return 1;
    }
    return head(n_streams, B, T, step, st);
}

int svc_dit::head(int n_streams, int B, int T, int step, hipStream_t st) {
    const int nseq = n_streams * B;
    const int M = nseq * seq_rows;
    const int Lw = seq_rows - win0;
    auto gemm_win = [&](int N) {
        KGemmParams p = gemm_base(nseq * Lw, N, Lw);
        p.a_seq_rows = seq_rows; p.c_seq_rows = seq_rows;
        p.a_off = win0; p.c_off = win0;
        return p;
    };
    if (!wavenet) {
        {
            KGemmParams p = gemm_win(D);
            p.a_ptr[0] = n16; p.a_ld[0] = D; p.a_ktiles[0] = D / 64;
            p.w = head_wa; p.ldw = D; p.bias = head_b0; p.act = KG_ACT_SILU;
            p.c16 = hm16; p.ldc16 = D;
            if (kgemm_launch(p, 0, KG_EPI_STORE, st)) return 1;
        }
        {
            KGemmParams p = gemm_win(C);
            p.a_ptr[0] = hm16; p.a_ld[0] = D; p.a_ktiles[0] = D / 64;
            p.w = head_w2; p.ldw = D; p.bias = head_b2;
            p.c32 = v32; p.ldc32 = C16;
            if (kgemm_launch(p, 0, KG_EPI_STORE, st)) return 1;
        }
        return 0;
    }
    const half_t* xres16 = n16;
    if (cfg.long_skip_connection) {
        KGemmParams p = gemm_win(D);
        p.n_taps = 2;
        p.a_ptr[0] = n16; p.a_ld[0] = D; p.a_ktiles[0] = D / 64;
        p.a_ptr[1] = x16; p.a_ld[1] = C16; p.a_ktiles[1] = C16 / 64;
        p.w = w_longskip; p.ldw = D + C16; p.bias = b_longskip;
        p.c16 = xr16; p.ldc16 = D;
        if (kgemm_launch(p, 0, KG_EPI_STORE, st)) return 1;
        xres16 = xr16;
    }
    {
        KGemmParams p = gemm_win(W);
        p.a_ptr[0] = xres16; p.a_ld[0] = D; p.a_ktiles[0] = D / 64;
        p.w = w_conv1; p.ldw = D; p.bias = b_conv1;
        p.c32 = wnx32; p.ldc32 = W; p.c16 = wnx16; p.ldc16 = W;
        if (kgemm_launch(p, 0, KG_EPI_STORE, st)) return 1;
    }
    for (int i = 0; i < NL; ++i) {
        int dil = 1;
        for (int j = 0; j < i; ++j) dil *= cfg.wn_dilation_rate;
        {
            KGemmParams p = gemm_win(2 * W);
            p.n_taps = WK;
            const int total = (WK - 1) * dil;
            const int left = total - total / 2;
            for (int t = 0; t < WK; ++t) {
                p.a_ptr[t] = wnx16; p.a_ld[t] = W; p.a_ktiles[t] = W / 64; p.a_shift[t] = t * dil - left;
            }
            p.pad_mode = KG_PAD_REFLECT;
            p.reflect_min = std::max(left, total - left) + 1;
            p.seq_len = d_convlen_w;
            p.w = wn_in[i]; p.ldw = (long)WK * W;
            p.rowvec = d_gcond + (long)step * 2 * W * NL + 2L * W * i; p.ld_rowvec = 0;
            p.c16 = acts16 + (long)i * acts_stride; p.ldc16 = W;
            if (kgemm_launch(p, 0, KG_EPI_TANHSIG, st)) return 1;
        }
        if (i < NL - 1) {
            KGemmParams p = gemm_win(W);
            p.a_ptr[0] = acts16 + (long)i * acts_stride; p.a_ld[0] = W; p.a_ktiles[0] = W / 64;
            p.w = wn_res[i]; p.ldw = W; p.bias = wn_res_b[i];
            p.res = wnx32; p.ldres = W;
            p.c32 = wnx32; p.ldc32 = W; p.c16 = wnx16; p.ldc16 = W;
            if (kgemm_launch(p, 0, KG_EPI_STORE, st)) return 1;
        }
    }
    {
        KGemmParams p = gemm_win(W);
        p.n_taps = NL + 1;
        for (int i = 0; i < NL; ++i) {
            p.a_ptr[i] = acts16 + (long)i * acts_stride; p.a_ld[i] = W; p.a_ktiles[i] = W / 64;
        }
        p.a_ptr[NL] = xres16; p.a_ld[NL] = D; p.a_ktiles[NL] = D / 64;
        p.w = wn_tail; p.ldw = (long)NL * W + D; p.bias = b_tail;
        p.c32 = flin32; p.ldc32 = W;
        if (kgemm_launch(p, 0, KG_EPI_STORE, st)) return 1;
    }
    {
        const float* fm = d_flmod + (long)step * 2 * W;
        if (layernorm_mod_launch(flin32, W, fl16, W, fm + W, fm, M, W, 1e-6f, st)) return 1;
    }
    {
        KGemmParams p = gemm_win(W);
        p.a_ptr[0] = fl16; p.a_ld[0] = W; p.a_ktiles[0] = W / 64;
        p.w = w_fl; p.ldw = W; p.bias = b_fl;
        p.c16 = fo16; p.ldc16 = W;
        if (kgemm_launch(p, 0, KG_EPI_STORE, st)) return 1;
    }
    {
        KGemmParams p = gemm_win(C);
        p.a_ptr[0] = fo16; p.a_ld[0] = W; p.a_ktiles[0] = W / 64;
        p.w = w_conv2; p.ldw = W; p.bias = b_conv2;
        p.c32 = v32; p.ldc32 = C16;
        if (kgemm_launch(p, 0, KG_EPI_STORE, st)) return 1;
    }
    return 0;
}

int svc_dit::body_fused(int n_streams, int B, int T, int step, hipStream_t st) {
    const int nseq = n_streams * B;
    const int M = nseq * seq_rows;
    const float* mod = d_mod + (long)step * mod_n;
    auto mods = [&](int i, const float** w_a, const float** b_a, const float** gate_a, const float** w_f, const float** b_f,
                    const float** gate_f) {
        *w_a = *b_a = *gate_a = *w_f = *b_f = *gate_f = nullptr;
        if (!adaptive_blocks) return;
        const float* lmod = mod + (long)i * mod_layer_n;
        if (v2) {
            *b_a = lmod; *w_a = lmod + D; *gate_a = lmod + 2 * D;
            *b_f = lmod + 3 * D; *w_f = lmod + 4 * D; *gate_f = lmod + 5 * D;
        } else {
            *w_a = lmod; *b_a = lmod + D; *w_f = lmod + 2 * D; *b_f = lmod + 3 * D;
        }
    };
    auto base = [&]() {
        PanelParams p;
        memset(&p, 0, sizeof(p));
        p.M = M; p.Lout = seq_rows; p.seq_rows = seq_rows; p.row_off = 0;
        p.eps = 1e-5f; p.add_one = v2 ? 1 : 0; p.I = I; p.x = xin;
        return p;
    };
    auto set_qkv = [&](PanelParams& p, int layer) {
        const float *w_a, *b_a, *ga, *w_f, *b_f, *gf;
        mods(layer, &w_a, &b_a, &ga, &w_f, &b_f, &gf);
        p.do_qkv = 1;
        p.g_attn = layers[layer].g_attn; p.w_a = w_a; p.b_a = b_a;
        p.rope = rope; p.q_scale = 0.125f * 1.4426950408889634f;
        p.qk = qk16; p.vt = vt; p.vt_seq_stride = (long)D * vt_ld; p.vt_ld = vt_ld; p.vt_mode = attention_vt_mode(nseq, H, seq_rows);
    };
    {
        PanelParams p = base();
        p.wstream = stream_pre; p.n_slots = stream_pre_slots;
        set_qkv(p, 0);
        if (fused_panel_launch(p, D, v2, st)) return 1;
    }
    size_t emit_i = 0;
    std::vector<int> skip_stack;
    for (int i = 0; i < L; ++i) {
        const bool last = i == L - 1;
        const bool tail_only = last && win0 > 0;
        {
            AttnParams a;
            memset(&a, 0, sizeof(a));
            a.q = qk16; a.k = qk16 + D; a.ld_qk = 2 * D;
            a.vt = vt; a.vt_seq_stride = (long)D * vt_ld; a.vt_ld = vt_ld; a.vt_perm = attention_vt_mode(nseq, H, seq_rows);
            a.out = ao16; a.ld_out = D;
            a.n_seq = nseq; a.H = H; a.seq_rows = seq_rows; a.Tq = seq_rows;
            a.q_start = tail_only ? win0 : 0;
            a.kv_len = d_kvlen;
            if (attention_launch(a, st)) return 1;
        }
        PanelParams p = base();
        const float *w_a, *b_a, *ga, *w_f, *b_f, *gf;
        mods(i, &w_a, &b_a, &ga, &w_f, &b_f, &gf);
        p.wstream = layers[i].stream; p.n_slots = layers[i].stream_slots;
        p.do_post = 1; p.ao = ao16;
        p.gate_a = ga; p.gate_f = gf; p.g_ffn = layers[i].g_ffn; p.w_f = w_f; p.b_f = b_f;
        if (std::find(emit.begin(), emit.end(), i) != emit.end()) {
            p.c16 = skip16[emit_i];
            skip_stack.push_back((int)emit_i);
            ++emit_i;
        }
        if (!last) {
            if (layers[i + 1].wskip) {
                p.do_skip = 1;
                p.skip_in = skip16[skip_stack.back()];
                skip_stack.pop_back();
                p.bskip = layers[i + 1].bskip;
            }
            set_qkv(p, i + 1);
        } else {
            const float* fm = mod + (long)L * mod_layer_n;
            p.do_final = 1; p.g_fin = g_final; p.w_fin = fm; p.b_fin = fm + D; p.n16 = n16;
            if (tail_only) { p.Lout = seq_rows - win0; p.row_off = win0; p.M = nseq * p.Lout; }
        }
        if (fused_panel_launch(p, D, v2, st)) return 1;
    }
    return 0;
}

int svc_dit::statics(int n_streams, const int (*flags)[3], int B, int T, const float* mu, const float* style_dev,
                     hipStream_t st) {
    const long Ks = C32 + Dc;
    if (w_style_merge)
        if (small_linear_launch(style_dev, S, w_style_merge, S, nullptr, d_stylevec, D, B, D, S, KG_ACT_NONE, st)) return 1;
    for (int j = 0; j < n_streams; ++j) {
        const bool use_p = flags[j][0], use_s = flags[j][1], use_m = flags[j][2];
        float* u = u_rowvec + (long)j * B * D;
        if (add_rowvec_launch(u, (use_s && w_style_merge) ? d_stylevec : nullptr, D, stat_const, B, D, st)) return 1;
        float* dst = st_term + (long)j * B * seq_rows * D;
        {
            KGemmParams p = gemm_base(B * T, D, T);
            p.a_ptr[0] = mu; p.a_ld[0] = Dc; p.a_ktiles[0] = use_m ? Dc / 32 : 0;
            p.a_seq_rows = T; p.a_len = T;
            p.w = w_stat + C32; p.ldw = Ks;
            p.c_seq_rows = seq_rows; p.c_off = npre;
            p.c32 = dst; p.ldc32 = D;
            p.rowvec = u; p.ld_rowvec = D;
            if (kgemm_launch(p, 1, KG_EPI_STORE, st)) return 1;
        }
        if (use_p) {
            KGemmParams p = gemm_base(B * T, D, T);
            p.a_ptr[0] = prompt32; p.a_ld[0] = C32; p.a_ktiles[0] = C32 / 32;
            p.a_seq_rows = seq_rows; p.a_len = T;
            p.w = w_stat; p.ldw = Ks;
            p.c_seq_rows = seq_rows; p.c_off = npre;
            p.c32 = dst; p.ldc32 = D;
            p.res = dst; p.ldres = D;
            if (kgemm_launch(p, 1, KG_EPI_STORE, st)) return 1;
        }
        if (style_in_w) {
            float* tk = tok_style + (long)j * B * D;
            if (use_s) {
                if (small_linear_launch(style_dev, S, style_in_w, S, style_in_b, tk, D, B, D, S, KG_ACT_NONE, st)) return 1;
            } else {
                if (add_rowvec_launch(tk, nullptr, 0, style_in_b, B, D, st)) return 1;
            }
        }
    }
    return 0;
}

namespace {
__global__ void init_state_kernel(float* __restrict__ x, long ldx, half_t* __restrict__ x16, long ldx16, int rows, int B,
                                  int T, int C, const int* __restrict__ prompt_len, int n_copies, long copy_stride) {
    const long i = (long)blockIdx.x * blockDim.x + threadIdx.x;
    if (i >= (long)B * T * C) return;
    const int c = (int)(i % C);
    const long bt = i / C;
    const int t = (int)(bt % T), b = (int)(bt / T);
    const long o = ((long)b * rows + t) * ldx + c;
    float v = x[o];
    if (t < prompt_len[b]) v = 0.f;
    x[o] = v;
    for (int k = 0; k < n_copies; ++k) x16[k * copy_stride + ((long)b * rows + t) * ldx16 + c] = (half_t)v;
}

__global__ __launch_bounds__(256) void init_state_seeded_kernel(const unsigned long long* __restrict__ seeds, float temperature,
                                                                float* __restrict__ x, long ldx, half_t* __restrict__ x16, long ldx16,
                                                                int rows, int B, int T, int C, const int* __restrict__ prompt_len,
                                                                int n_copies, long copy_stride) {
    const long i = (long)blockIdx.x * blockDim.x + threadIdx.x;
    const int C4 = C >> 2;
    if (i >= (long)B * rows * C4) return;
    const int c4 = (int)(i % C4);
    const long bt = i / C4;
    const int t = (int)(bt % rows), b = (int)(bt / rows);
    float v[4] = {0.f, 0.f, 0.f, 0.f};
    if (t < T && t >= prompt_len[b]) {
        noise_normal4(seeds[b], NOISE_CFM_Z, (unsigned)c4, (unsigned)t, v);
#pragma unroll
        for (int j = 0; j < 4; ++j) v[j] *= temperature;
    }
    const long row = (long)b * rows + t;
    *reinterpret_cast<float4v*>(x + row * ldx + 4 * c4) = (float4v){v[0], v[1], v[2], v[3]};
    if (t < T) {
        const half4 h = {(half_t)v[0], (half_t)v[1], (half_t)v[2], (half_t)v[3]};
        for (int k = 0; k < n_copies; ++k) *reinterpret_cast<half4*>(x16 + k * copy_stride + row * ldx16 + 4 * c4) = h;
    }
}

__global__ void euler_kernel(float* __restrict__ x, long ldx, half_t* __restrict__ x16, long ldx16, int rows,
                             const float* __restrict__ v, long ldv, long v_stream_stride, int v_off, int B, int T, int C,
                             const int* __restrict__ prompt_len, float dt, float c0, float ca, float cb, int stream_a,
                             int stream_b, int n_copies, long copy_stride) {
    const long i = (long)blockIdx.x * blockDim.x + threadIdx.x;
    if (i >= (long)B * T * C) return;
    const int c = (int)(i % C);
    const long bt = i / C;
    const int t = (int)(bt % T), b = (int)(bt / T);
    const long vo = ((long)b * rows + v_off + t) * ldv + c;
    float d = c0 * v[vo];
    if (stream_a >= 0) d -= ca * v[vo + stream_a * v_stream_stride];
    if (stream_b >= 0) d -= cb * v[vo + stream_b * v_stream_stride];
    const long xo = ((long)b * rows + t) * ldx + c;
    float nx = x[xo] + dt * d;
    if (t < prompt_len[b]) nx = 0.f;
    x[xo] = nx;
    for (int k = 0; k < n_copies; ++k) x16[k * copy_stride + ((long)b * rows + t) * ldx16 + c] = (half_t)nx;
}

__global__ void prompt_rows_kernel(const float* __restrict__ src, int C, int P, float* __restrict__ dst, long ld, int rows,
                                   int T, const int* __restrict__ prompt_len, int B) {
    const long i = (long)blockIdx.x * blockDim.x + threadIdx.x;
    if (i >= (long)B * T * C) return;
    const int t = (int)(i % T);
    const long bc = i / T;
    const int c = (int)(bc % C), b = (int)(bc / C);
    const float v = (t < prompt_len[b] && t < P) ? src[((long)b * C + c) * P + t] : 0.f;
    dst[((long)b * rows + t) * ld + c] = v;
}
}

int svc_dit::run_group(const svc_cfm_args_t* a, const uint64_t* seeds, int b0, int nb, int n_streams, const int (*flags)[3],
                       const std::vector<float>& tvals, const std::vector<float>& dts, float c0, float ca, float cb,
                       int stream_a, int stream_b, hipStream_t st) {
    const int T = a->T, P = a->P;
    const int n_steps = (int)tvals.size();
    if (reserve(n_streams, nb, T, n_steps, st)) return 1;
    std::vector<int> kv(n_streams * nb), cv(n_streams * nb), pl(nb);
    for (int b = 0; b < nb; ++b) {
        const int len = a->x_lens ? (int)a->x_lens[b0 + b] : T;
        const int plen = a->prompt_lens ? (int)a->prompt_lens[b0 + b] : P;
        SVC_REQUIRE(len >= 1 && len <= T, "x_lens out of range");
        SVC_REQUIRE(plen >= 0 && plen <= P && plen <= len, "prompt_lens out of range");
        pl[b] = plen;
        for (int j = 0; j < n_streams; ++j) {
            kv[j * nb + b] = len + npre;
            cv[j * nb + b] = len;
        }
    }
    {
        int halo = 0;
        if (wavenet) {
            int dil = 1;
            for (int i = 0; i < NL; ++i) {
                const int total = (WK - 1) * dil;
                halo += total - total / 2;
                dil *= cfg.wn_dilation_rate;
            }
        }
        const int min_pl = *std::min_element(pl.begin(), pl.end());
        win0 = std::max(0, npre + min_pl - halo) & ~7;
    }
    std::vector<int> cvw(cv.size());
    for (size_t i = 0; i < cv.size(); ++i) cvw[i] = cv[i] - (win0 - npre > 0 ? win0 - npre : 0);
    {
        const size_t n = kv.size();
        const size_t n_int = round_up(3 * n + pl.size(), 2);
        int* h = reinterpret_cast<int*>(staging.acquire(n_int * sizeof(int) + (seeds ? (size_t)nb * 8 : 0)));
        if (!h) return 1;
        memcpy(h, kv.data(), n * 4); memcpy(h + n, cv.data(), n * 4); memcpy(h + 2 * n, cvw.data(), n * 4);
        memcpy(h + 3 * n, pl.data(), pl.size() * 4);
        if (seeds) {
            memcpy(h + n_int, seeds + b0, (size_t)nb * 8);
            SVC_CHECK_HIP(hipMemcpyAsync(d_seeds, h + n_int, (size_t)nb * 8, hipMemcpyHostToDevice, st));
        }
        SVC_CHECK_HIP(hipMemcpyAsync(d_kvlen, h, n * 4, hipMemcpyHostToDevice, st));
        SVC_CHECK_HIP(hipMemcpyAsync(d_convlen, h + n, n * 4, hipMemcpyHostToDevice, st));
        SVC_CHECK_HIP(hipMemcpyAsync(d_convlen_w, h + 2 * n, n * 4, hipMemcpyHostToDevice, st));
        SVC_CHECK_HIP(hipMemcpyAsync(d_plen, h + 3 * n, pl.size() * 4, hipMemcpyHostToDevice, st));
        if (staging.commit(st)) return 1;
    }
    if (tables(tvals, st)) return 1;

    const long copy_stride = (long)nb * seq_rows * C16;
    const long n_el = (long)nb * T * C;
    if (seeds) {
        hipLaunchKernelGGL(init_state_seeded_kernel, dim3(cdiv((long)nb * seq_rows * (C / 4), 256)), dim3(256), 0, st, d_seeds,
                           a->temperature, x32, (long)C16, x16, (long)C16, seq_rows, nb, T, C, d_plen, n_streams, copy_stride);
    } else {
        if (bct_to_btc_launch(a->z + (long)b0 * C * T, nb, C, T, x32, C16, nullptr, 0, seq_rows, T, a->temperature, st)) return 1;
        hipLaunchKernelGGL(init_state_kernel, dim3(cdiv(n_el, 256)), dim3(256), 0, st, x32, (long)C16, x16, (long)C16, seq_rows,
                           nb, T, C, d_plen, n_streams, copy_stride);
    }
    SVC_CHECK_HIP(hipGetLastError());
    hipLaunchKernelGGL(prompt_rows_kernel, dim3(cdiv(n_el, 256)), dim3(256), 0, st, a->prompt + (long)b0 * C * P, C, P,
                       prompt32, (long)C32, seq_rows, T, d_plen, nb);
    SVC_CHECK_HIP(hipGetLastError());
    if (statics(n_streams, flags, nb, T, a->mu + (long)b0 * T * Dc, a->style + (long)b0 * S, st)) return 1;

    auto steps = [&](hipStream_t s_) -> int {
        for (int s = 0; s < n_steps; ++s) {
            if (body(n_streams, nb, T, s, s_)) return 1;
            hipLaunchKernelGGL(euler_kernel, dim3(cdiv(n_el, 256)), dim3(256), 0, s_, x32, (long)C16, x16, (long)C16, seq_rows,
                               v32, (long)C16, (long)nb * seq_rows * C16, npre, nb, T, C, d_plen, dts[s], c0, ca, cb,
                               stream_a, stream_b, n_streams, copy_stride);
            SVC_CHECK_HIP(hipGetLastError());
        }
        return 0;
    };
    static const int graph_env = [] { const char* e = getenv("SVC_DIT_GRAPH"); return e ? (e[0] == '0' ? 0 : 1) : -1; }();
    bool done = false;
    if ((graph_env >= 0 ? graph_env : use_graphs) && !prof_enabled()) {
        std::vector<float> key = {(float)n_streams, (float)nb, (float)T, (float)n_steps, (float)win0, (float)seq_rows, c0, ca, cb,
                                  (float)stream_a, (float)stream_b, (float)fused_min_rows};
        key.insert(key.end(), dts.begin(), dts.end());
        StepGraph* g = nullptr;
        for (auto& c : graphs) if (c.key == key) { g = &c; break; }
        if (!g) {
            if (graphs.size() >= 8) { if (graphs.front().exec) (void)hipGraphExecDestroy(graphs.front().exec); graphs.erase(graphs.begin()); }
            graphs.push_back(StepGraph());
            g = &graphs.back();
            g->key = key;
        }
        if (g->seen++ >= 1 && !g->exec) {
            if (!cap_stream && hipStreamCreateWithFlags(&cap_stream, hipStreamNonBlocking) != hipSuccess) { (void)hipGetLastError(); cap_stream = nullptr; }
            hipGraph_t gr = nullptr;
            if (cap_stream && hipStreamBeginCapture(cap_stream, hipStreamCaptureModeThreadLocal) == hipSuccess) {
                const int rc = steps(cap_stream);
                const hipError_t e = hipStreamEndCapture(cap_stream, &gr);
                if (rc == 0 && e == hipSuccess && gr && hipGraphInstantiate(&g->exec, gr, nullptr, nullptr, 0) != hipSuccess) g->exec = nullptr;
                if (gr) (void)hipGraphDestroy(gr);
                if (rc || e != hipSuccess) { (void)hipGetLastError(); g->exec = nullptr; if (rc) return 1; }
            } else {
                (void)hipGetLastError();
            }
        }
        if (g->exec) {
            SVC_CHECK_HIP(hipGraphLaunch(g->exec, st));
            done = true;
        }
    }
    if (!done && steps(st)) return 1;
    return btc_to_bct_launch(x32, C16, seq_rows, a->out + (long)b0 * C * T, nb, C, T, st);
}

extern "C" {

int svc_dit_create(const svc_dit_config_t* cfg, const svc_tensor_desc_t* weights, int n_weights, void* stream,
                   svc_dit_t** out) {
    SVC_REQUIRE(cfg && weights && out, "null argument");
    SVC_REQUIRE(cfg->hidden_dim == cfg->num_heads * 64, "head_dim must be 64 (hidden_dim = 64 * num_heads)");
    SVC_REQUIRE(cfg->content_dim % 32 == 0, "content_dim must be a multiple of 32");
    SVC_REQUIRE(cfg->in_channels % 8 == 0 && cfg->in_channels <= 128, "in_channels must be a multiple of 8, <= 128");
    svc_dit* m = new svc_dit();
    m->cfg = *cfg;
    m->device = current_device();
    m->v2 = cfg->version == 2;
    m->D = cfg->hidden_dim; m->H = cfg->num_heads; m->L = cfg->depth; m->C = cfg->in_channels;
    m->Dc = cfg->content_dim; m->S = cfg->style_dim;
    {
        const int n_hidden = (int)(2 * (4 * m->D) / 3);
        m->I = (int)round_up(n_hidden, 256);
    }
    m->wavenet = cfg->final_layer_type == 1;
    m->W = m->wavenet ? cfg->wn_hidden_dim : 0;
    m->NL = m->wavenet ? cfg->wn_num_layers : 0;
    m->WK = m->wavenet ? cfg->wn_kernel_size : 0;
    m->npre = (cfg->time_as_token ? 1 : 0) + (cfg->style_as_token ? 1 : 0);
    m->C16 = (int)round_up(m->C, 64);
    m->C32 = (int)round_up(m->C, 32);
    m->adaptive_blocks = m->v2 || !cfg->time_as_token;
    if (m->wavenet) {
        if (m->W % 64 != 0 || m->W != m->D || m->WK * 1 > KG_MAX_TAPS || m->npre != 0) {
            set_error("wavenet head needs wn_hidden_dim == hidden_dim (FinalLayer modulates with t1), no prefix tokens");
            delete m;
            return 1;
        }
    }
    if (!m->v2 && cfg->uvit_skip_connection) {
        for (int i = 0; i < m->L; ++i) {
            if (i < m->L / 2) m->emit.push_back(i);
            if (i > m->L / 2) m->recv.push_back(i);
        }
    }
    hipStream_t st = (hipStream_t)stream;
    StateDict sd(weights, n_weights);
    if (m->pack(sd, st)) {
        delete m;
        return 1;
    }
    *out = m;
    return 0;
}

void svc_dit_destroy(svc_dit_t* m) {
    if (m) {
        m->drop_graphs();
        if (m->cap_stream) (void)hipStreamDestroy(m->cap_stream);
    }
    delete m;
}

int svc_dit_set_microbatch(svc_dit_t* m, int utterances) {
    SVC_REQUIRE(m && utterances >= 0, "bad argument");
    m->microbatch = utterances;
    return 0;
}

int svc_dit_set_fused_min_rows(svc_dit_t* m, long rows) {
    SVC_REQUIRE(m, "null argument");
    m->fused_min_rows = rows < 0 ? 10240 : rows;
    return 0;
}

int svc_dit_fused_available(svc_dit_t* m) { return m && m->fused_ok ? 1 : 0; }

int svc_dit_set_graphs(svc_dit_t* m, int on) {
    SVC_REQUIRE(m, "null argument");
    m->use_graphs = on ? 1 : 0;
    if (!on) m->drop_graphs();
    return 0;
}

int svc_cfm_sample(svc_dit_t* m, const svc_cfm_args_t* a, void* stream) {
    SVC_REQUIRE(m && a, "null argument");
    return m->sample(a, nullptr, (hipStream_t)stream);
}

int svc_cfm_sample_seeded(svc_dit_t* m, const svc_cfm_args_t* a, const uint64_t* seeds, void* stream) {
    SVC_REQUIRE(m && a, "null argument");
    SVC_REQUIRE(seeds, "svc_cfm_sample_seeded: seeds is NULL (HOST [B], one per utterance)");
    return m->sample(a, seeds, (hipStream_t)stream);
}

}

int svc_dit::sample(const svc_cfm_args_t* a, const uint64_t* seeds, hipStream_t st) {
    svc_dit* m = this;
    SVC_REQUIRE(a->B >= 1 && a->T >= 1 && a->P >= 0 && a->P <= a->T && a->n_timesteps >= 1, "bad sampler shape");
    SVC_REQUIRE(a->T + m->npre <= ROPE_POS, "sequence longer than the RoPE table");
    SVC_REQUIRE(a->mu && (a->prompt || a->P == 0) && a->style && (a->z || seeds) && a->out, "null tensor");
    SVC_REQUIRE(current_device() == m->device, "this handle was created on another device (make it current before the call)");
    const int N = a->n_timesteps;
    std::vector<float> ts = linspace01(N + 1);
    std::vector<float> tvals(N), dts(N);
    if (!m->v2) {
        float t = ts[0];
        for (int s = 1; s <= N; ++s) {
            const float dt = ts[s] - ts[s - 1];
            tvals[s - 1] = t;
            dts[s - 1] = dt;
            t = t + dt;
        }
    } else {
        for (auto& v : ts) v = v + (-1.0f) * (cosf((float)M_PI / 2.0f * v) - 1.0f + v);
        float t = ts[0], dt = ts[1] - ts[0];
        for (int s = 1; s <= N; ++s) {
            tvals[s - 1] = t;
            dts[s - 1] = dt;
            t = t + dt;
            if (s < N) dt = ts[s + 1] - t;
        }
    }
    int flags[MAX_STREAMS][3] = {{1, 1, 1}, {0, 0, 0}, {0, 0, 0}};
    int n_streams = 1, sa = -1, sb = -1;
    float c0 = 1.f, ca = 0.f, cb = 0.f;
    const float ra = a->cfg_rate[0], rb = a->cfg_rate[1];
    if (!m->v2) {
        if (ra > 0.f) { n_streams = 2; sa = 1; c0 = 1.f + ra; ca = ra; }
    } else if (a->random_voice) {
        n_streams = 2; flags[0][0] = 0; flags[0][1] = 0; sa = 1; c0 = 1.f + ra; ca = ra;
    } else if (ra == 0.f && rb == 0.f) {
        n_streams = 1;
    } else if (ra == 0.f) {
        n_streams = 2; flags[1][2] = 1; sa = 1; c0 = 1.f + rb; ca = rb;
    } else if (rb == 0.f) {
        n_streams = 2; sa = 1; c0 = 1.f + ra; ca = ra;
    } else {
        n_streams = 3; flags[1][2] = 1; sa = 2; sb = 1; c0 = 1.f + ra + rb; ca = ra; cb = rb;
    }
    int mb = m->microbatch > 0 ? m->microbatch : 32;
    for (int b0 = 0; b0 < a->B; b0 += mb) {
        const int nb = std::min(mb, a->B - b0);
        if (m->run_group(a, seeds, b0, nb, n_streams, flags, tvals, dts, c0, ca, cb, sa, sb, st)) return 1;
    }
    return 0;
}

extern "C" {

int svc_dit_forward(svc_dit_t* m, int N, int T, const float* x, const float* prompt_x, const int64_t* x_lens, float t,
                    const float* style, const float* mu, float* out, void* stream) {
    SVC_REQUIRE(m && x && prompt_x && style && mu && out, "null argument");
    SVC_REQUIRE(N >= 1 && T >= 1 && T + m->npre <= ROPE_POS, "bad estimator shape");
    SVC_REQUIRE(current_device() == m->device, "this handle was created on another device (make it current before the call)");
    hipStream_t st = (hipStream_t)stream;
    const int flags[1][3] = {{1, 1, 1}};
    if (m->reserve(1, N, T, 1, st)) return 1;
    std::vector<int> kv(N), cv(N), pl(N);
    for (int b = 0; b < N; ++b) {
        const int len = x_lens ? (int)x_lens[b] : T;
        SVC_REQUIRE(len >= 1 && len <= T, "x_lens out of range");
        kv[b] = len + m->npre; cv[b] = len; pl[b] = T;
    }
    m->win0 = 0;
    {
        int* h = reinterpret_cast<int*>(m->staging.acquire(3 * (size_t)N * sizeof(int)));
        if (!h) return 1;
        memcpy(h, kv.data(), N * 4); memcpy(h + N, cv.data(), N * 4); memcpy(h + 2 * N, pl.data(), N * 4);
        SVC_CHECK_HIP(hipMemcpyAsync(m->d_kvlen, h, N * 4, hipMemcpyHostToDevice, st));
        SVC_CHECK_HIP(hipMemcpyAsync(m->d_convlen, h + N, N * 4, hipMemcpyHostToDevice, st));
        SVC_CHECK_HIP(hipMemcpyAsync(m->d_convlen_w, h + N, N * 4, hipMemcpyHostToDevice, st));
        SVC_CHECK_HIP(hipMemcpyAsync(m->d_plen, h + 2 * N, N * 4, hipMemcpyHostToDevice, st));
        if (m->staging.commit(st)) return 1;
    }
    std::vector<float> tv(1, t);
    if (m->tables(tv, st)) return 1;
    const int C = m->C, C16 = m->C16, C32 = m->C32, rows = m->seq_rows;
    if (bct_to_btc_launch(x, N, C, T, m->x32, C16, m->x16, C16, rows, T, 1.0f, st)) return 1;
    const long n_el = (long)N * T * C;
    hipLaunchKernelGGL(prompt_rows_kernel, dim3(cdiv(n_el, 256)), dim3(256), 0, st, prompt_x, C, T, m->prompt32, (long)C32,
                       rows, T, m->d_plen, N);
    SVC_CHECK_HIP(hipGetLastError());
    if (m->statics(1, flags, N, T, mu, style, st)) return 1;
    if (m->body(1, N, T, 0, st)) return 1;
    return btc_to_bct_launch(m->v32 + (long)m->npre * C16, C16, rows, out, N, C, T, st);
}

}
```

### seed-vc_amd/csrc/fused.hip

```cpp
#include <stdlib.h>

#include <utility>

#include "common.h"

namespace svc {

namespace {

typedef __attribute__((address_space(1))) const void* gptr_t;
typedef __attribute__((address_space(3))) void* lptr_t;

template <int D>
struct PG {
    static constexpr int NT = D / 16;
    static constexpr int KC = D / 32;
    static constexpr int SLOT_BYTES = NT * 1024;
    static constexpr int NS = D == 384 ? 5 : 4;
    static constexpr int RING = NS * SLOT_BYTES;
    static constexpr int PF = D == 384 ? 6 : 4;
    static constexpr int NVEC = 9;
    static constexpr int LDS = RING + NVEC * D * 4;
};

__device__ __forceinline__ half8 frag_read(unsigned lds_addr, int off) {
    half8 r;
    asm volatile("ds_read_b128 %0, %1 offset:%2" : "=v"(r) : "v"(lds_addr), "n"(0) : "memory");
    (void)off;
    return r;
}
template <int OFF>
__device__ __forceinline__ void frag_read_to(half8& r, unsigned lds_addr) {
    asm volatile("ds_read_b128 %0, %1 offset:%2" : "=v"(r) : "v"(lds_addr), "n"(OFF));
}
template <int N>
__device__ __forceinline__ void frag_wait(half8& r) {
    asm volatile("s_waitcnt lgkmcnt(%1)" : "+v"(r) : "n"(N));
}

template <int NF, int PF, int TM, int RFI, typename F, typename R>
__device__ __forceinline__ void stream_frags(const char* base, F&& body, R&& refill) {
    static_assert(NF * 1024 <= 65536 && PF >= 1 && PF <= 8, "ds_read offset field");
    const unsigned la = (unsigned)(uintptr_t)(lptr_t)const_cast<char*>(base);
    half8 q[PF];
    [&]<int... I>(std::integer_sequence<int, I...>) { (frag_read_to<I * 1024>(q[I], la), ...); }(std::make_integer_sequence<int, PF>{});
    [&]<int... Fi>(std::integer_sequence<int, Fi...>) {
        ([&] {
            constexpr int f = Fi;
            constexpr int pending = (NF - f < PF ? NF - f : PF) - 1;
            frag_wait<pending>(q[f % PF]);
            const half8 w = q[f % PF];
            body(f, w);
            if constexpr (f + PF < NF) frag_read_to<(f + PF) * 1024>(q[f % PF], la);
            if constexpr (f % RFI == RFI - 1) refill(f / RFI);
            __builtin_amdgcn_sched_barrier(0);
        }(), ...);
    }(std::make_integer_sequence<int, NF>{});
}

__device__ __forceinline__ void mfma_v(float4v& c, const half8 a, const half8 b) {
    asm volatile("v_mfma_f32_16x16x32_f16 %0, %1, %2, %0" : "+v"(c) : "v"(a), "v"(b));
}
__device__ __forceinline__ void mfma_guard(float4v (&a)[4][2]) {
    asm volatile("s_nop 15\n\ts_nop 3"
                 : "+v"(a[0][0]), "+v"(a[0][1]), "+v"(a[1][0]), "+v"(a[1][1]), "+v"(a[2][0]), "+v"(a[2][1]), "+v"(a[3][0]), "+v"(a[3][1]));
}
__device__ __forceinline__ void mfma_guard(float4v (&a)[4][1]) {}
template <int NF, typename F, typename R>
__device__ __forceinline__ void stream_frags_asm(const char* base, F&& body, R&& refill) {
    static_assert(NF % 4 == 0, "fragment groups of 4");
    half8 q[2][4];
#pragma unroll
    for (int i = 0; i < 4; ++i) q[0][i] = *reinterpret_cast<const half8*>(base + i * 1024);
#pragma unroll
    for (int g = 0; g < NF / 4; ++g) {
        if (g + 1 < NF / 4) {
#pragma unroll
            for (int i = 0; i < 4; ++i) q[(g + 1) & 1][i] = *reinterpret_cast<const half8*>(base + ((g + 1) * 4 + i) * 1024);
        }
        __builtin_amdgcn_sched_barrier(0);
#pragma unroll
        for (int i = 0; i < 4; ++i) body(g * 4 + i, q[g & 1][i]);
        refill(g);
        __builtin_amdgcn_sched_barrier(0);
    }
}

enum { V_AF = 0, V_BF = 1, V_GA = 2, V_GF = 3, V_AA = 4, V_BA = 5, V_BS = 6, V_AN = 7, V_BN = 8 };

template <int D, bool GATED, int TM>
__global__ __launch_bounds__(128 / (16 * TM) * 64, 128 / (16 * TM) / 4) void dit_panel_kernel(const PanelParams p) {
    using G = PG<D>;
    constexpr int NT = G::NT, KC = G::KC, NS = G::NS, PF = G::PF;
    constexpr int NW = 128 / (16 * TM), NTHR = NW * 64, DPS = NT / NW, RFI = NT / DPS;
    constexpr bool ASM_SIDE = D == 512 && TM == 2;
    extern __shared__ __attribute__((aligned(16))) char smem[];
    float* vec = reinterpret_cast<float*>(smem + G::RING);

    const int tid = threadIdx.x, lane = tid & 63;
    const int wave = __builtin_amdgcn_readfirstlane(tid >> 6);
    const int fr = lane & 15, fq = lane >> 4;
    const int m0 = blockIdx.x * 128 + wave * (16 * TM);

    for (int c = tid; c < D; c += NTHR) {
        const float one = p.add_one ? 1.f : 0.f;
        vec[V_AF * D + c] = p.g_ffn ? p.g_ffn[c] * (p.w_f ? one + p.w_f[c] : 1.f) : 0.f;
        vec[V_BF * D + c] = p.b_f ? p.b_f[c] : 0.f;
        vec[V_GA * D + c] = p.gate_a ? p.gate_a[c] : 1.f;
        vec[V_GF * D + c] = p.gate_f ? p.gate_f[c] : 1.f;
        vec[V_AA * D + c] = p.g_attn ? p.g_attn[c] * (p.w_a ? one + p.w_a[c] : 1.f) : 0.f;
        vec[V_BA * D + c] = p.b_a ? p.b_a[c] : 0.f;
        vec[V_BS * D + c] = p.bskip ? p.bskip[c] : 0.f;
        vec[V_AN * D + c] = p.g_fin ? p.g_fin[c] * (p.w_fin ? one + p.w_fin[c] : 1.f) : 0.f;
        vec[V_BN * D + c] = p.b_fin ? p.b_fin[c] : 0.f;
    }
    __syncthreads();

    const char* wsrc = reinterpret_cast<const char*>(p.wstream) + wave * (G::SLOT_BYTES / NW) + lane * 16;
    int s_next = 0, stage = 0, fill = NS - 1, s_issued = 0;
    auto piece = [&](const char* src, char* dst, int i) {
        const char* s4 = src + (i >> 2) * 4096;
        char* d4 = dst + (i >> 2) * 4096;
        switch (i & 3) {
            case 0: __builtin_amdgcn_global_load_lds((gptr_t)s4, (lptr_t)d4, 16, 0, 0); break;
            case 1: __builtin_amdgcn_global_load_lds((gptr_t)s4, (lptr_t)d4, 16, 1024, 0); break;
            case 2: __builtin_amdgcn_global_load_lds((gptr_t)s4, (lptr_t)d4, 16, 2048, 0); break;
            default: __builtin_amdgcn_global_load_lds((gptr_t)s4, (lptr_t)d4, 16, 3072, 0); break;
        }
    };
    const char* rf_src = nullptr;
    char* rf_dst = nullptr;
    auto acquire = [&]() -> const char* {
        const int ahead = p.n_slots - 1 - s_next;
        if constexpr (NS == 5) {
            if (ahead >= 3) asm volatile("s_waitcnt vmcnt(%0)" ::"n"(3 * DPS) : "memory");
            else if (ahead == 2) asm volatile("s_waitcnt vmcnt(%0)" ::"n"(2 * DPS) : "memory");
            else if (ahead == 1) asm volatile("s_waitcnt vmcnt(%0)" ::"n"(DPS) : "memory");
            else asm volatile("s_waitcnt vmcnt(0)" ::: "memory");
        } else {
            if (ahead >= 2) asm volatile("s_waitcnt vmcnt(%0)" ::"n"(2 * DPS) : "memory");
            else if (ahead == 1) asm volatile("s_waitcnt vmcnt(%0)" ::"n"(DPS) : "memory");
            else asm volatile("s_waitcnt vmcnt(0)" ::: "memory");
        }
        asm volatile("s_barrier" ::: "memory");
        const int src_slot = s_issued < p.n_slots ? s_issued : p.n_slots - 1;
        rf_src = wsrc + (long)src_slot * G::SLOT_BYTES;
        rf_dst = smem + fill * G::SLOT_BYTES + wave * (G::SLOT_BYTES / NW);
        ++s_issued;
        const char* ptr = smem + stage * G::SLOT_BYTES + lane * 16;
        stage = stage + 1 == NS ? 0 : stage + 1;
        fill = fill + 1 == NS ? 0 : fill + 1;
        ++s_next;
        return ptr;
    };
    auto refill = [&](int i) { piece(rf_src, rf_dst, i); };
#define FRAG(base, idx) (*reinterpret_cast<const half8*>((base) + (idx) * 1024))
#define MFMA(a, b, c) __builtin_amdgcn_mfma_f32_16x16x32_f16((a), (b), (c), 0, 0, 0)

#pragma unroll
    for (int s_ = 0; s_ < NS - 1; ++s_) {
        const int src_slot = s_ < p.n_slots ? s_ : p.n_slots - 1;
#pragma unroll
        for (int i = 0; i < DPS; ++i)
            piece(wsrc + (long)src_slot * G::SLOT_BYTES, smem + s_ * G::SLOT_BYTES + wave * (G::SLOT_BYTES / NW), i);
        ++s_issued;
    }

    long grow[TM];
    bool rok[TM];
#pragma unroll
    for (int mt = 0; mt < TM; ++mt) {
        const int m = m0 + 16 * mt + fr;
        rok[mt] = m < p.M;
        const int mm = rok[mt] ? m : p.M - 1;
        const int seq = mm / p.Lout;
        grow[mt] = (long)seq * p.seq_rows + p.row_off + (mm - seq * p.Lout);
    }

    float4v acc[NT][TM];
    half8 xn[KC][TM];

    auto norm_to_xn = [&](const float* va, const float* vb) {
        float rs[TM];
#pragma unroll
        for (int mt = 0; mt < TM; ++mt) {
            float ss = 0.f;
#pragma unroll
            for (int t = 0; t < NT; ++t)
#pragma unroll
                for (int r = 0; r < 4; ++r) ss += acc[t][mt][r] * acc[t][mt][r];
            ss += __shfl_xor(ss, 16);
            ss += __shfl_xor(ss, 32);
            rs[mt] = rsqrtf(ss / (float)D + p.eps);
        }
#pragma unroll
        for (int c = 0; c < KC; ++c) {
            const float4v a0 = *reinterpret_cast<const float4v*>(va + 32 * c + 4 * fq);
            const float4v a1 = *reinterpret_cast<const float4v*>(va + 32 * c + 16 + 4 * fq);
            const float4v b0 = *reinterpret_cast<const float4v*>(vb + 32 * c + 4 * fq);
            const float4v b1 = *reinterpret_cast<const float4v*>(vb + 32 * c + 16 + 4 * fq);
#pragma unroll
            for (int mt = 0; mt < TM; ++mt) {
                half8 h;
#pragma unroll
                for (int j = 0; j < 4; ++j) {
                    h[j] = (half_t)(acc[2 * c][mt][j] * rs[mt] * a0[j] + b0[j]);
                    h[4 + j] = (half_t)(acc[2 * c + 1][mt][j] * rs[mt] * a1[j] + b1[j]);
                }
                xn[c][mt] = h;
            }
        }
    };
    auto store_x = [&]() {
#pragma unroll
        for (int mt = 0; mt < TM; ++mt)
            if (rok[mt]) {
#pragma unroll
                for (int t = 0; t < NT; ++t) *reinterpret_cast<float4v*>(p.x + grow[mt] * D + 16 * t + 4 * fq) = acc[t][mt];
            }
    };

    if (p.do_post) {
        {
            half8 af[KC][TM];
#pragma unroll
            for (int mt = 0; mt < TM; ++mt) {
#pragma unroll
                for (int kc = 0; kc < KC; ++kc)
                    af[kc][mt] = *reinterpret_cast<const half8*>(p.ao + grow[mt] * D + 32 * kc + 8 * fq);
#pragma unroll
                for (int t = 0; t < NT; ++t)
                    acc[t][mt] = GATED ? (float4v){0.f, 0.f, 0.f, 0.f}
                                       : *reinterpret_cast<const float4v*>(p.x + grow[mt] * D + 16 * t + 4 * fq);
            }
#pragma unroll
            for (int kc = 0; kc < KC; ++kc) {
                const char* base = acquire();
                stream_frags<NT, PF, TM, RFI>(base, [&](int t, half8 w) {
#pragma unroll
                    for (int mt = 0; mt < TM; ++mt) acc[t][mt] = MFMA(w, af[kc][mt], acc[t][mt]);
                }, refill);
            }
        }
        if constexpr (GATED) {
#pragma unroll
            for (int mt = 0; mt < TM; ++mt)
#pragma unroll
                for (int t = 0; t < NT; ++t) {
                    const float4v xi = *reinterpret_cast<const float4v*>(p.x + grow[mt] * D + 16 * t + 4 * fq);
                    const float4v ga = *reinterpret_cast<const float4v*>(vec + V_GA * D + 16 * t + 4 * fq);
#pragma unroll
                    for (int r = 0; r < 4; ++r) acc[t][mt][r] = xi[r] + ga[r] * acc[t][mt][r];
                }
            store_x();
        }
        norm_to_xn(vec + V_AF * D, vec + V_BF * D);
        if constexpr (GATED) {
#pragma unroll
            for (int mt = 0; mt < TM; ++mt)
#pragma unroll
                for (int t = 0; t < NT; ++t) acc[t][mt] = (float4v){0.f, 0.f, 0.f, 0.f};
        }
        const int n_chunks = p.I / 32;
        for (int c = 0; c < n_chunks; ++c) {
            float4v a1[4][TM];
#pragma unroll
            for (int t = 0; t < 4; ++t)
#pragma unroll
                for (int mt = 0; mt < TM; ++mt) a1[t][mt] = (float4v){0.f, 0.f, 0.f, 0.f};
            {
                const char* base = acquire();
                if constexpr (ASM_SIDE) {
                    stream_frags_asm<NT>(base, [&](int f, half8 w) {
                        _Pragma("unroll") for (int mt = 0; mt < TM; ++mt) mfma_v(a1[f & 3][mt], w, xn[f >> 2][mt]);
                    }, refill);
                } else {
                    stream_frags<NT, PF, TM, RFI>(base, [&](int f, half8 w) {
                        _Pragma("unroll") for (int mt = 0; mt < TM; ++mt) a1[f & 3][mt] = MFMA(w, xn[f >> 2][mt], a1[f & 3][mt]);
                    }, refill);
                }
            }
            {
                const char* base = acquire();
                if constexpr (ASM_SIDE) {
                    stream_frags_asm<NT>(base, [&](int f, half8 w) {
                        _Pragma("unroll") for (int mt = 0; mt < TM; ++mt) mfma_v(a1[f & 3][mt], w, xn[KC / 2 + (f >> 2)][mt]);
                    }, refill);
                    mfma_guard(a1);
                } else {
                    stream_frags<NT, PF, TM, RFI>(base, [&](int f, half8 w) {
                        _Pragma("unroll") for (int mt = 0; mt < TM; ++mt) a1[f & 3][mt] = MFMA(w, xn[KC / 2 + (f >> 2)][mt], a1[f & 3][mt]);
                    }, refill);
                }
            }
            half8 hf[TM];
            constexpr float LOG2E = 1.4426950408889634f;
#pragma unroll
            for (int mt = 0; mt < TM; ++mt)
#pragma unroll
                for (int t = 0; t < 4; ++t)
#pragma unroll
                    for (int i = 0; i < 2; ++i) {
                        const float a = a1[t][mt][2 * i], b = a1[t][mt][2 * i + 1];
                        hf[mt][2 * t + i] = (half_t)(a * __builtin_amdgcn_rcpf(1.0f + __builtin_amdgcn_exp2f(-a * LOG2E)) * b);
                    }
            {
                const char* base = acquire();
                stream_frags<NT, PF, TM, RFI>(base, [&](int t, half8 w) {
#pragma unroll
                    for (int mt = 0; mt < TM; ++mt) acc[t][mt] = MFMA(w, hf[mt], acc[t][mt]);
                }, refill);
            }
        }
        if constexpr (GATED) {
#pragma unroll
            for (int mt = 0; mt < TM; ++mt)
#pragma unroll
                for (int t = 0; t < NT; ++t) {
                    const float4v xi = *reinterpret_cast<const float4v*>(p.x + grow[mt] * D + 16 * t + 4 * fq);
                    const float4v gf = *reinterpret_cast<const float4v*>(vec + V_GF * D + 16 * t + 4 * fq);
#pragma unroll
                    for (int r = 0; r < 4; ++r) acc[t][mt][r] = xi[r] + gf[r] * acc[t][mt][r];
                }
        }
        if (!p.do_skip) store_x();
        if (p.c16) {
#pragma unroll
            for (int mt = 0; mt < TM; ++mt)
                if (rok[mt]) {
#pragma unroll
                    for (int t = 0; t < NT; ++t) {
                        const half4 h = {(half_t)acc[t][mt][0], (half_t)acc[t][mt][1], (half_t)acc[t][mt][2], (half_t)acc[t][mt][3]};
                        *reinterpret_cast<half4*>(p.c16 + grow[mt] * D + 16 * t + 4 * fq) = h;
                    }
                }
        }
    } else {
#pragma unroll
        for (int mt = 0; mt < TM; ++mt)
#pragma unroll
            for (int t = 0; t < NT; ++t) acc[t][mt] = *reinterpret_cast<const float4v*>(p.x + grow[mt] * D + 16 * t + 4 * fq);
    }

    if (p.do_skip) {
#pragma unroll
        for (int c = 0; c < KC; ++c)
#pragma unroll
            for (int mt = 0; mt < TM; ++mt) {
                half8 h;
#pragma unroll
                for (int j = 0; j < 4; ++j) {
                    h[j] = (half_t)acc[2 * c][mt][j];
                    h[4 + j] = (half_t)acc[2 * c + 1][mt][j];
                }
                xn[c][mt] = h;
            }
#pragma unroll
        for (int t = 0; t < NT; ++t)
#pragma unroll
            for (int mt = 0; mt < TM; ++mt) acc[t][mt] = *reinterpret_cast<const float4v*>(vec + V_BS * D + 16 * t + 4 * fq);
#pragma unroll
        for (int kc = 0; kc < KC; ++kc) {
            const char* base = acquire();
            stream_frags<NT, PF, TM, RFI>(base, [&](int t, half8 w) {
#pragma unroll
                for (int mt = 0; mt < TM; ++mt) acc[t][mt] = MFMA(w, xn[kc][mt], acc[t][mt]);
            }, refill);
        }
#pragma unroll
        for (int mt = 0; mt < TM; ++mt)
#pragma unroll
            for (int kc = 0; kc < KC; ++kc)
                xn[kc][mt] = *reinterpret_cast<const half8*>(p.skip_in + grow[mt] * D + 32 * kc + 8 * fq);
#pragma unroll
        for (int kc = 0; kc < KC; ++kc) {
            const char* base = acquire();
            stream_frags<NT, PF, TM, RFI>(base, [&](int t, half8 w) {
#pragma unroll
                for (int mt = 0; mt < TM; ++mt) acc[t][mt] = MFMA(w, xn[kc][mt], acc[t][mt]);
            }, refill);
        }
        store_x();
    }

    if (p.do_final) {
        float rs[TM];
#pragma unroll
        for (int mt = 0; mt < TM; ++mt) {
            float ss = 0.f;
#pragma unroll
            for (int t = 0; t < NT; ++t)
#pragma unroll
                for (int r = 0; r < 4; ++r) ss += acc[t][mt][r] * acc[t][mt][r];
            ss += __shfl_xor(ss, 16);
            ss += __shfl_xor(ss, 32);
            rs[mt] = rsqrtf(ss / (float)D + p.eps);
        }
#pragma unroll
        for (int t = 0; t < NT; ++t) {
            const float4v a = *reinterpret_cast<const float4v*>(vec + V_AN * D + 16 * t + 4 * fq);
            const float4v b = *reinterpret_cast<const float4v*>(vec + V_BN * D + 16 * t + 4 * fq);
#pragma unroll
            for (int mt = 0; mt < TM; ++mt)
                if (rok[mt]) {
                    half4 h;
#pragma unroll
                    for (int r = 0; r < 4; ++r) h[r] = (half_t)(acc[t][mt][r] * rs[mt] * a[r] + b[r]);
                    *reinterpret_cast<half4*>(p.n16 + grow[mt] * D + 16 * t + 4 * fq) = h;
                }
        }
    }

    if (p.do_qkv) {
        norm_to_xn(vec + V_AA * D, vec + V_BA * D);
        float rp[TM][16];
        int posl[TM];
#pragma unroll
        for (int mt = 0; mt < TM; ++mt) {
            const int m = m0 + 16 * mt + fr;
            const int mm = m < p.M ? m : p.M - 1;
            posl[mt] = p.row_off + mm % p.Lout;
            const float* tb = p.rope + ((long)posl[mt] * 32 + 8 * fq) * 2;
#pragma unroll
            for (int q4 = 0; q4 < 4; ++q4) {
                const float4v t4 = *reinterpret_cast<const float4v*>(tb + 4 * q4);
#pragma unroll
                for (int j = 0; j < 4; ++j) rp[mt][4 * q4 + j] = t4[j];
            }
        }
        const int n_groups = 3 * D / 64, n_qk = 2 * D / 64;
        for (int grp = 0; grp < n_groups; ++grp) {
            float4v a1[4][TM];
#pragma unroll
            for (int t = 0; t < 4; ++t)
#pragma unroll
                for (int mt = 0; mt < TM; ++mt) a1[t][mt] = (float4v){0.f, 0.f, 0.f, 0.f};
            if (grp < n_qk) {
#pragma unroll
                for (int hs = 0; hs < 2; ++hs) {
                    const char* base = acquire();
                    if constexpr (ASM_SIDE) {
                        stream_frags_asm<NT>(base, [&](int f, half8 w) {
                            _Pragma("unroll") for (int mt = 0; mt < TM; ++mt) mfma_v(a1[f & 3][mt], w, xn[hs * (KC / 2) + (f >> 2)][mt]);
                        }, refill);
                        if (hs == 1) mfma_guard(a1);
                    } else {
                        stream_frags<NT, PF, TM, RFI>(base, [&](int f, half8 w) {
                            _Pragma("unroll") for (int mt = 0; mt < TM; ++mt) a1[f & 3][mt] = MFMA(w, xn[hs * (KC / 2) + (f >> 2)][mt], a1[f & 3][mt]);
                        }, refill);
                    }
                }
                const float sc = grp < D / 64 ? p.q_scale : 1.0f;
#pragma unroll
                for (int mt = 0; mt < TM; ++mt) {
                    float o[16];
#pragma unroll
                    for (int i = 0; i < 8; ++i) {
                        const float x0 = a1[i >> 1][mt][2 * (i & 1)], x1 = a1[i >> 1][mt][2 * (i & 1) + 1];
                        const float cs = rp[mt][2 * i], sn = rp[mt][2 * i + 1];
                        o[2 * i] = (x0 * cs - x1 * sn) * sc;
                        o[2 * i + 1] = (x1 * cs + x0 * sn) * sc;
                    }
                    if (rok[mt]) {
                        half_t* dst = p.qk + grow[mt] * (2 * D) + 64 * grp + 16 * fq;
                        *reinterpret_cast<uint4*>(dst) = pack8(o);
                        *reinterpret_cast<uint4*>(dst + 8) = pack8(o + 8);
                    }
                }
            } else {
#pragma unroll
                for (int hs = 0; hs < 2; ++hs) {
                    const char* base = acquire();
                    if constexpr (ASM_SIDE) {
                        stream_frags_asm<NT>(base, [&](int f, half8 w) {
                            _Pragma("unroll") for (int mt = 0; mt < TM; ++mt) mfma_v(a1[f & 3][mt], xn[hs * (KC / 2) + (f >> 2)][mt], w);
                        }, refill);
                        if (hs == 1) mfma_guard(a1);
                    } else {
                        stream_frags<NT, PF, TM, RFI>(base, [&](int f, half8 w) {
                            _Pragma("unroll") for (int mt = 0; mt < TM; ++mt) a1[f & 3][mt] = MFMA(xn[hs * (KC / 2) + (f >> 2)][mt], w, a1[f & 3][mt]);
                        }, refill);
                    }
                }
#pragma unroll
                for (int mt = 0; mt < TM; ++mt) {
                    const int m = m0 + 16 * mt + 4 * fq;
                    if (m < p.M) {
                        const int seq = m / p.Lout;
                        const int pos = p.row_off + (m - seq * p.Lout);
#pragma unroll
                        for (int t = 0; t < 4; ++t) {
                            const int d = 64 * (grp - n_qk) + 16 * t + fr;
                            const half4 h = {(half_t)a1[t][mt][0], (half_t)a1[t][mt][1], (half_t)a1[t][mt][2], (half_t)a1[t][mt][3]};
                            *reinterpret_cast<half4*>(p.vt + (long)seq * p.vt_seq_stride + (long)d * p.vt_ld + vt_pos(pos, p.vt_mode ? p.vt_mode : 1)) = h;
                        }
                    }
                }
            }
        }
    }
    asm volatile("s_waitcnt vmcnt(0)" ::: "memory");
#undef FRAG
#undef MFMA
}

__global__ void pack_stream_kernel(half_t* __restrict__ dst, long n_elems, int mode, int D, int I, const float* __restrict__ w0,
                                   const float* __restrict__ w1, const float* __restrict__ w2) {
    const long e = (long)blockIdx.x * blockDim.x + threadIdx.x;
    if (e >= n_elems) return;
    const int NT = D / 16, KC = D / 32;
    const long f = e >> 9;
    const int l = (int)((e >> 3) & 63), j = (int)(e & 7);
    const int fr = l & 15, g = l >> 4;
    const int kperm = 16 * (j >> 2) + 4 * g + (j & 3);
    const int knat = 8 * g + j;
    float v = 0.f;
    if (mode == 0) {
        const int kc = (int)(f / NT), t = (int)(f % NT);
        v = w0[(long)(16 * t + fr) * D + 32 * kc + knat];
    } else if (mode == 1) {
        const long per = 3L * NT;
        const int c = (int)(f / per), q = (int)(f % per);
        if (q < 2 * NT) {
            const int kc = q / 4, t = q % 4;
            const int h = 32 * c + 8 * (fr >> 2) + 2 * t + ((fr & 3) >> 1);
            const float* src = (fr & 1) ? w1 : w0;
            v = src[(long)h * D + 32 * kc + kperm];
        } else {
            const int t = q - 2 * NT;
            v = w2[(long)(16 * t + fr) * I + 32 * c + knat];
        }
    } else if (mode == 2) {
        const int kc = (int)(f / NT), t = (int)(f % NT);
        const int k = kc < KC ? 32 * kc + kperm : D + 32 * (kc - KC) + knat;
        v = w0[(long)(16 * t + fr) * (2 * D) + k];
    } else {
        const int grp = (int)(f / (4 * KC)), q = (int)(f % (4 * KC));
        const int kc = q / 4, t = q % 4;
        const int n = grp < 2 * D / 64 ? 64 * grp + 16 * (fr >> 2) + 4 * t + (fr & 3) : 64 * grp + 16 * t + fr;
        v = w0[(long)n * D + 32 * kc + kperm];
    }
    dst[e] = (half_t)v;
}

}

bool fused_supported(int D, int I) {
    static const bool off = [] { const char* e = getenv("SVC_FUSED"); return e && e[0] == '0'; }();
    return !off && (D == 384 || D == 512) && I % 32 == 0;
}

static long slots_post(int D, int I) { return D / 32 + 3L * (I / 32); }
static long slots_skip(int D) { return 2L * (D / 32); }
static long slots_qkv(int D) { return 2L * (3 * D / 64); }

long fused_stream_halfs(int D, int I, bool post, bool skip, bool qkv) {
    const long slot_halfs = (long)(D / 16) * 512;
    return ((post ? slots_post(D, I) : 0) + (skip ? slots_skip(D) : 0) + (qkv ? slots_qkv(D) : 0)) * slot_halfs;
}

long fused_pack_stream(half_t* dst, int D, int I, const float* wo, const float* w1, const float* w3, const float* w2,
                       const float* wskip, const float* wqkv, hipStream_t st) {
    const long slot_halfs = (long)(D / 16) * 512;
    long off = 0;
    auto run = [&](int mode, long slots, const float* a, const float* b, const float* c) -> bool {
        const long n = slots * slot_halfs;
        hipLaunchKernelGGL(pack_stream_kernel, dim3(cdiv(n, 256)), dim3(256), 0, st, dst + off, n, mode, D, I, a, b, c);
        off += n;
        return hipGetLastError() == hipSuccess;
    };
    if (wo) {
        if (!run(0, D / 32, wo, nullptr, nullptr)) return 0;
        if (!run(1, 3L * (I / 32), w1, w3, w2)) return 0;
    }
    if (wskip && !run(2, slots_skip(D), wskip, nullptr, nullptr)) return 0;
    if (wqkv && !run(3, slots_qkv(D), wqkv, nullptr, nullptr)) return 0;
    return off;
}

int fused_panel_launch(const PanelParams& p, int D, bool gated, hipStream_t st) {
    SVC_REQUIRE(D == 384 || D == 512, "fused panel kernel: D must be 384 or 512");
    SVC_REQUIRE(p.M > 0 && p.Lout > 0 && p.I % 32 == 0, "fused panel kernel: shape");
    SVC_REQUIRE(!p.do_qkv || (p.M % 4 == 0 && p.Lout % 4 == 0 && p.row_off % 4 == 0), "fused panel kernel: v^T stores need 4-row groups");
    DeviceState* ds = device_state();
    if (!ds) return 1;
    if (!ds->fused_attr.load(std::memory_order_acquire)) {
#define SVC_PANEL_ATTR(DD, GG, TT) SVC_CHECK_HIP(hipFuncSetAttribute(reinterpret_cast<const void*>(dit_panel_kernel<DD, GG, TT>), hipFuncAttributeMaxDynamicSharedMemorySize, PG<DD>::LDS))
        SVC_PANEL_ATTR(384, false, 1); SVC_PANEL_ATTR(384, true, 1); SVC_PANEL_ATTR(512, false, 1); SVC_PANEL_ATTR(512, true, 1);
        SVC_PANEL_ATTR(384, false, 2); SVC_PANEL_ATTR(384, true, 2); SVC_PANEL_ATTR(512, false, 2); SVC_PANEL_ATTR(512, true, 2);
#undef SVC_PANEL_ATTR
        ds->fused_attr.store(true, std::memory_order_release);
    }
    const long want = (p.do_post ? slots_post(D, p.I) : 0) + (p.do_skip ? slots_skip(D) : 0) + (p.do_qkv ? slots_qkv(D) : 0);
    SVC_REQUIRE(want == p.n_slots, "fused panel kernel: slot count does not match the enabled phases");
    const int grid = cdiv(p.M, 128);
    const bool prof = prof_enabled();
    if (prof) prof_begin(PROF_FUSED, st);
    static const int tm_env = [] { const char* e = getenv("SVC_FUSED_TM"); return e ? atoi(e) : 0; }();
    const int tm = (tm_env == 1 || tm_env == 2) ? tm_env : (D == 384 ? 2 : 1);
#define SVC_PANEL_LAUNCH(DD, GG, TT) hipLaunchKernelGGL((dit_panel_kernel<DD, GG, TT>), dim3(grid), dim3(128 / (16 * TT) * 64), PG<DD>::LDS, st, p)
    if (tm == 2) {
        if (D == 384) { if (gated) SVC_PANEL_LAUNCH(384, true, 2); else SVC_PANEL_LAUNCH(384, false, 2); }
        else { if (gated) SVC_PANEL_LAUNCH(512, true, 2); else SVC_PANEL_LAUNCH(512, false, 2); }
    } else {
        if (D == 384) { if (gated) SVC_PANEL_LAUNCH(384, true, 1); else SVC_PANEL_LAUNCH(384, false, 1); }
        else { if (gated) SVC_PANEL_LAUNCH(512, true, 1); else SVC_PANEL_LAUNCH(512, false, 1); }
    }
#undef SVC_PANEL_LAUNCH
    SVC_CHECK_HIP(hipGetLastError());
    if (prof) {
        const double M = p.M, Dd = D;
        double macs = 0;
        if (p.do_post) macs += Dd * Dd + 3.0 * Dd * p.I;
        if (p.do_skip) macs += 2.0 * Dd * Dd;
        if (p.do_qkv) macs += 3.0 * Dd * Dd;
        double bytes = 2.0 * macs;
        bytes += M * Dd * ((p.do_post ? 4 + 2 : 4) + ((p.do_post && !p.do_skip) || p.do_skip ? 4 : 0) + (p.c16 ? 2 : 0) +
                           (p.do_skip ? 2 : 0) + (p.do_qkv ? 6 : 0) + (p.do_final ? 2 : 0));
        const unsigned long long tag = ((unsigned long long)p.M << 40) | ((unsigned long long)(D & 0xFFFFF) << 20) |
                                       ((unsigned long long)(p.I & 0xFFFF) << 4) |
                                       (unsigned)((p.do_post ? 1 : 0) | (p.do_skip ? 2 : 0) | (p.do_qkv ? 4 : 0) | (p.do_final ? 8 : 0));
        prof_end(PROF_FUSED, 2.0 * M * macs, bytes, st, tag);
    }
    return 0;
}

}
```

Measured before the change: 139,100 mel-frames/s.

## Fuse input merge GEMM and output head into first and last fused panels

Adds two seam variants of the fused DiT panel kernel. One folds the prefix-token fill and the input merge projection (x16 times w_merge plus the style/time term) into the first panel that computes QKV. The other folds the final head (linear, activation, linear to mel channels) into the last panel after the final norm. The aim is to remove separate kernel launches and the round trips of the hidden state through global memory at both ends of each estimator step. This costs extra template instantiations, register pressure in the fused kernel, and a new stream-packing layout for the merge and head weights. Both seams are on by default and can be switched off through a mask.

```diff
diff --git a/include/seedvc_hip.h b/include/seedvc_hip.h
--- a/include/seedvc_hip.h
+++ b/include/seedvc_hip.h
@@ -33,6 +33,7 @@
 int svc_dit_set_microbatch(svc_dit_t* m, int utterances);
 
 int svc_dit_set_fused_min_rows(svc_dit_t* m, long rows);
+int svc_dit_set_fused_seams(svc_dit_t* m, int mask);
 int svc_dit_fused_available(svc_dit_t* m);
 int svc_dit_set_graphs(svc_dit_t* m, int on);
 
diff --git a/seed-vc_amd/_lib.py b/seed-vc_amd/_lib.py
--- a/seed-vc_amd/_lib.py
+++ b/seed-vc_amd/_lib.py
@@ -8,7 +8,7 @@
 
 EXPORTS = [
     "svc_abi_version", "svc_last_error",
-    "svc_dit_create", "svc_dit_destroy", "svc_dit_set_microbatch", "svc_dit_set_fused_min_rows", "svc_dit_fused_available", "svc_dit_set_graphs", "svc_cfm_sample", "svc_dit_forward",
+    "svc_dit_create", "svc_dit_destroy", "svc_dit_set_microbatch", "svc_dit_set_fused_min_rows", "svc_dit_set_fused_seams", "svc_dit_fused_available", "svc_dit_set_graphs", "svc_cfm_sample", "svc_dit_forward",
     "svc_cfm_sample_seeded", "svc_cfm_noise_draws", "svc_hift_forward_seeded", "svc_hift_noise_draws",
     "svc_bigvgan_create", "svc_bigvgan_destroy", "svc_bigvgan_forward", "svc_bigvgan_forward_ragged", "svc_bigvgan_set_microbatch",
     "svc_hift_create", "svc_hift_destroy", "svc_hift_forward", "svc_hift_forward_ragged", "svc_hift_set_microbatch",
diff --git a/seed-vc_amd/cfm.py b/seed-vc_amd/cfm.py
--- a/seed-vc_amd/cfm.py
+++ b/seed-vc_amd/cfm.py
@@ -44,6 +44,9 @@
 
     def set_fused_min_rows(self, rows):
         _lib.check(_lib.lib().svc_dit_set_fused_min_rows(self._h, C.c_long(int(rows))))
+
+    def set_fused_seams(self, mask):
+        _lib.check(_lib.lib().svc_dit_set_fused_seams(self._h, int(mask)))
 
     def set_graphs(self, on):
         _lib.check(_lib.lib().svc_dit_set_graphs(self._h, int(bool(on))))
diff --git a/seed-vc_amd/csrc/common.h b/seed-vc_amd/csrc/common.h
--- a/seed-vc_amd/csrc/common.h
+++ b/seed-vc_amd/csrc/common.h
@@ -219,11 +219,24 @@
     half_t* qk; half_t* vt; long vt_seq_stride; long vt_ld; int vt_mode;
     int do_final;
     const float* g_fin; const float* w_fin; const float* b_fin; half_t* n16;
-};
+    int seam;
+    const half_t* x16;
+    const float* st_term;
+    const float* tok_time; const float* tok_style;
+    const float* zero_row;
+    int npre, time_first, T;
+    const float* head_b0; const float* head_b2;
+    float* v32; int ldv; int head_C;
+};
+enum { PANEL_SEAM_NONE = 0, PANEL_SEAM_MERGE = 1, PANEL_SEAM_HEAD = 2 };
+enum { PANEL_MERGE_K = 128 };
 bool fused_supported(int D, int I);
+long fused_seam_slots(int D, int seam, int C);
 long fused_stream_halfs(int D, int I, bool post, bool skip, bool qkv);
 long fused_pack_stream(half_t* dst, int D, int I, const float* wo, const float* w1, const float* w3, const float* w2,
                        const float* wskip, const float* wqkv, hipStream_t st);
+long fused_pack_merge(half_t* dst, int D, const float* w_merge, int ldw, int C, hipStream_t st);
+long fused_pack_head(half_t* dst, int D, const float* wa, const float* w2, int C, hipStream_t st);
 int fused_panel_launch(const PanelParams& p, int D, bool gated, hipStream_t st);
 
 struct AttnParams {
diff --git a/seed-vc_amd/csrc/dit.hip b/seed-vc_amd/csrc/dit.hip
--- a/seed-vc_amd/csrc/dit.hip
+++ b/seed-vc_amd/csrc/dit.hip
@@ -59,6 +59,11 @@
     };
     half_t* stream_pre = nullptr;
     int stream_pre_slots = 0;
+    half_t* stream_first = nullptr;
+    float* zero_row = nullptr;
+    int merge_slots = 0, head_slots = 0;
+    bool merge_ok = false, head_ok = false;
+    int seams = 3;
     bool fused_ok = false;
     long fused_min_rows = 10240;
     std::vector<Layer> layers;
@@ -108,7 +113,7 @@
                   int stream_a, int stream_b, hipStream_t st);
     int sample(const svc_cfm_args_t* a, const uint64_t* seeds, hipStream_t st);
     int body(int n_streams, int B, int T, int step, hipStream_t st);
-    int body_fused(int n_streams, int B, int T, int step, hipStream_t st);
+    int body_fused(int n_streams, int B, int T, int step, bool seam_merge, bool seam_head, hipStream_t st);
     int head(int n_streams, int B, int T, int step, hipStream_t st);
 };
 
@@ -192,7 +197,9 @@
             const bool nskip = !last && layers[i + 1].wskip != nullptr;
             const std::string pn = "transformer.layers." + std::to_string(i + 1) + ".";
             const long halfs = fused_stream_halfs(D, I, true, nskip, !last);
-            layers[i].stream = wts.alloc_n<half_t>(halfs, st);
+            head_ok = !wavenet && C % 16 == 0;
+            if (last && head_ok) head_slots = (int)fused_seam_slots(D, PANEL_SEAM_HEAD, C);
+            layers[i].stream = wts.alloc_n<half_t>(halfs + (last ? (long)head_slots * slot_halfs : 0), st);
             if (!layers[i].stream) return 1;
             const long wr = fused_pack_stream(layers[i].stream, D, I, W(p + "attention.wo.weight"), W(p + "feed_forward.w1.weight"),
                                               W(p + "feed_forward.w3.weight"), W(p + "feed_forward.w2.weight"),
@@ -202,8 +209,13 @@
             layers[i].stream_slots = (int)(halfs / slot_halfs);
         }
         const long halfs = fused_stream_halfs(D, I, false, false, true);
-        stream_pre = wts.alloc_n<half_t>(halfs, st);
-        if (!stream_pre) return 1;
+        merge_ok = C16 == PANEL_MERGE_K;
+        if (merge_ok) merge_slots = (int)fused_seam_slots(D, PANEL_SEAM_MERGE, C);
+        stream_first = wts.alloc_n<half_t>((long)merge_slots * slot_halfs + halfs, st);
+        if (!stream_first) return 1;
+        stream_pre = stream_first + (long)merge_slots * slot_halfs;
+        zero_row = wts.alloc_n<float>(D, st);
+        if (!zero_row) return 1;
         if (fused_pack_stream(stream_pre, D, I, nullptr, nullptr, nullptr, nullptr, nullptr,
                               W("transformer.layers.0.attention.wqkv.weight"), st) != halfs) { set_error("fused stream packing failed"); return 1; }
         stream_pre_slots = (int)(halfs / slot_halfs);
@@ -267,6 +279,10 @@
     w_merge_x = new16(D, C16);
     if (!w_merge_x) return 1;
     if (pack_block(0, wm->data, Kin, 0, D, C, w_merge_x, C16, 0, 0, 1, nullptr, st)) return 1;
+    if (merge_ok && fused_pack_merge(stream_first, D, wm->data, Kin, C, st) != (long)merge_slots * (D / 16) * 512) {
+        set_error("fused stream packing failed");
+        return 1;
+    }
     const long Ks = C32 + Dc;
     w_stat = wts.alloc_n<float>(Dp * Ks, st);
     stat_const = wts.alloc_n<float>(D, st);
@@ -303,6 +319,11 @@
         if (!head_wa || !head_w2) return 1;
         if (pack_block(0, a->data, D, 0, D, D, head_wa, D, 0, 0, 1, nullptr, st)) return 1;
         if (pack_block(0, c->data, D, 0, C, D, head_w2, D, 0, 0, 1, nullptr, st)) return 1;
+        if (head_ok) {
+            const long slot_halfs = (long)(D / 16) * 512;
+            half_t* dst = layers[L - 1].stream + (long)layers[L - 1].stream_slots * slot_halfs;
+            if (fused_pack_head(dst, D, a->data, c->data, C, st) != head_slots * slot_halfs) { set_error("fused stream packing failed"); return 1; }
+        }
         head_b0 = copy_vec(wts, b->data, D, st);
         head_b2 = copy_vec(wts, d->data, C, st);
         if (!head_b0 || !head_b2) return 1;
@@ -569,9 +590,11 @@
     const int nseq = n_streams * B;
     const int M = nseq * seq_rows;
     const float* mod = d_mod + (long)step * mod_n;
-    if (prefix_rows_launch(xin, nseq, seq_rows, D, npre, T + npre, d_t1 + (long)step * D, tok_style,
-                           cfg.time_as_token ? 1 : 0, st)) return 1;
-    {
+    const bool fused = fused_ok && (long)M >= fused_min_rows;
+    const bool seam_merge = fused && merge_ok && (seams & 1), seam_head = fused && head_ok && (seams & 2);
+    if (!seam_merge && prefix_rows_launch(xin, nseq, seq_rows, D, npre, T + npre, d_t1 + (long)step * D, tok_style,
+                                          cfg.time_as_token ? 1 : 0, st)) return 1;
+    if (!seam_merge) {
         KGemmParams p = gemm_base(nseq * T, D, T);
         p.a_ptr[0] = x16; p.a_ld[0] = C16; p.a_ktiles[0] = C16 / 64;
         p.a_seq_rows = seq_rows; p.a_len = T;
@@ -581,9 +604,9 @@
         p.res = st_term; p.ldres = D;
         if (kgemm_launch(p, 0, KG_EPI_STORE, st)) return 1;
     }
-    if (fused_ok && (long)M >= fused_min_rows) {
-        if (body_fused(n_streams, B, T, step, st)) return 1;
-        return head(n_streams, B, T, step, st);
+    if (fused) {
+        if (body_fused(n_streams, B, T, step, seam_merge, seam_head, st)) return 1;
+        return seam_head ? 0 : head(n_streams, B, T, step, st);
     }
     const int Lw = seq_rows - win0;
     auto gemm_win = [&](int N) {
@@ -792,7 +815,7 @@
     return 0;
 }
 
-int svc_dit::body_fused(int n_streams, int B, int T, int step, hipStream_t st) {
+int svc_dit::body_fused(int n_streams, int B, int T, int step, bool seam_merge, bool seam_head, hipStream_t st) {
     const int nseq = n_streams * B;
     const int M = nseq * seq_rows;
     const float* mod = d_mod + (long)step * mod_n;
@@ -827,6 +850,12 @@
         PanelParams p = base();
         p.wstream = stream_pre; p.n_slots = stream_pre_slots;
         set_qkv(p, 0);
+        if (seam_merge) {
+            p.seam = PANEL_SEAM_MERGE;
+            p.wstream = stream_first; p.n_slots = merge_slots + stream_pre_slots;
+            p.x16 = x16; p.st_term = st_term; p.zero_row = zero_row; p.T = T; p.npre = npre;
+            p.tok_time = d_t1 + (long)step * D; p.tok_style = tok_style; p.time_first = cfg.time_as_token ? 1 : 0;
+        }
         if (fused_panel_launch(p, D, v2, st)) return 1;
     }
     size_t emit_i = 0;
@@ -868,6 +897,11 @@
             const float* fm = mod + (long)L * mod_layer_n;
             p.do_final = 1; p.g_fin = g_final; p.w_fin = fm; p.b_fin = fm + D; p.n16 = n16;
             if (tail_only) { p.Lout = seq_rows - win0; p.row_off = win0; p.M = nseq * p.Lout; }
+            if (seam_head) {
+                p.seam = PANEL_SEAM_HEAD;
+                p.n_slots = layers[i].stream_slots + head_slots;
+                p.head_b0 = head_b0; p.head_b2 = head_b2; p.v32 = v32; p.ldv = C16; p.head_C = C;
+            }
         }
         if (fused_panel_launch(p, D, v2, st)) return 1;
     }
@@ -1069,7 +1103,7 @@
     bool done = false;
     if ((graph_env >= 0 ? graph_env : use_graphs) && !prof_enabled()) {
         std::vector<float> key = {(float)n_streams, (float)nb, (float)T, (float)n_steps, (float)win0, (float)seq_rows, c0, ca, cb,
-                                  (float)stream_a, (float)stream_b, (float)fused_min_rows};
+                                  (float)stream_a, (float)stream_b, (float)fused_min_rows, (float)seams};
         key.insert(key.end(), dts.begin(), dts.end());
         StepGraph* g = nullptr;
         for (auto& c : graphs) if (c.key == key) { g = &c; break; }
@@ -1167,6 +1201,12 @@
 int svc_dit_set_fused_min_rows(svc_dit_t* m, long rows) {
     SVC_REQUIRE(m, "null argument");
     m->fused_min_rows = rows < 0 ? 10240 : rows;
+    return 0;
+}
+
+int svc_dit_set_fused_seams(svc_dit_t* m, int mask) {
+    SVC_REQUIRE(m && mask >= 0 && mask <= 3, "svc_dit_set_fused_seams: mask is bit 0 (merge) | bit 1 (head)");
+    m->seams = mask;
     return 0;
 }
 
diff --git a/seed-vc_amd/csrc/fused.hip b/seed-vc_amd/csrc/fused.hip
--- a/seed-vc_amd/csrc/fused.hip
+++ b/seed-vc_amd/csrc/fused.hip
@@ -1,5 +1,6 @@
 #include <stdlib.h>
 
+#include <type_traits>
 #include <utility>
 
 #include "common.h"
@@ -88,7 +89,7 @@
 
 enum { V_AF = 0, V_BF = 1, V_GA = 2, V_GF = 3, V_AA = 4, V_BA = 5, V_BS = 6, V_AN = 7, V_BN = 8 };
 
-template <int D, bool GATED, int TM>
+template <int D, bool GATED, int TM, int SEAM>
 __global__ __launch_bounds__(128 / (16 * TM) * 64, 128 / (16 * TM) / 4) void dit_panel_kernel(const PanelParams p) {
     using G = PG<D>;
     constexpr int NT = G::NT, KC = G::KC, NS = G::NS, PF = G::PF;
@@ -101,6 +102,9 @@
     const int wave = __builtin_amdgcn_readfirstlane(tid >> 6);
     const int fr = lane & 15, fq = lane >> 4;
     const int m0 = blockIdx.x * 128 + wave * (16 * TM);
+#define DO_POST (SEAM == PANEL_SEAM_MERGE ? 0 : SEAM == PANEL_SEAM_HEAD ? 1 : p.do_post)
+#define DO_SKIP (SEAM == PANEL_SEAM_NONE ? p.do_skip : 0)
+#define DO_QKV (SEAM == PANEL_SEAM_MERGE ? 1 : SEAM == PANEL_SEAM_HEAD ? 0 : p.do_qkv)
 
     for (int c = tid; c < D; c += NTHR) {
         const float one = p.add_one ? 1.f : 0.f;
@@ -113,6 +117,10 @@
         vec[V_BS * D + c] = p.bskip ? p.bskip[c] : 0.f;
         vec[V_AN * D + c] = p.g_fin ? p.g_fin[c] * (p.w_fin ? one + p.w_fin[c] : 1.f) : 0.f;
         vec[V_BN * D + c] = p.b_fin ? p.b_fin[c] : 0.f;
+        if constexpr (SEAM == PANEL_SEAM_HEAD) {
+            vec[V_AA * D + c] = p.head_b0[c];
+            vec[V_BA * D + c] = c < p.head_C ? p.head_b2[c] : 0.f;
+        }
     }
     __syncthreads();
 
@@ -180,7 +188,7 @@
     float4v acc[NT][TM];
     half8 xn[KC][TM];
 
-    auto norm_to_xn = [&](const float* va, const float* vb) {
+    auto norm_to_xn = [&](const float* va, const float* vb, auto fenced) {
         float rs[TM];
 #pragma unroll
         for (int mt = 0; mt < TM; ++mt) {
@@ -209,6 +217,11 @@
                 }
                 xn[c][mt] = h;
             }
+            if constexpr (decltype(fenced)::value) {
+#pragma unroll
+                for (int mt = 0; mt < TM; ++mt) asm volatile("" : "+v"(xn[c][mt]));
+                __builtin_amdgcn_sched_barrier(0);
+            }
         }
     };
     auto store_x = [&]() {
@@ -220,7 +233,7 @@
             }
     };
 
-    if (p.do_post) {
+    if (DO_POST) {
         {
             half8 af[KC][TM];
 #pragma unroll
@@ -254,7 +267,7 @@
                 }
             store_x();
         }
-        norm_to_xn(vec + V_AF * D, vec + V_BF * D);
+        norm_to_xn(vec + V_AF * D, vec + V_BF * D, std::false_type{});
         if constexpr (GATED) {
 #pragma unroll
             for (int mt = 0; mt < TM; ++mt)
@@ -323,7 +336,7 @@
                     for (int r = 0; r < 4; ++r) acc[t][mt][r] = xi[r] + gf[r] * acc[t][mt][r];
                 }
         }
-        if (!p.do_skip) store_x();
+        if (!DO_SKIP && SEAM != PANEL_SEAM_HEAD) store_x();
         if (p.c16) {
 #pragma unroll
             for (int mt = 0; mt < TM; ++mt)
@@ -335,6 +348,35 @@
                     }
                 }
         }
+    } else if constexpr (SEAM == PANEL_SEAM_MERGE) {
+        constexpr int KM = PANEL_MERGE_K / 32;
+        half8 af[KM][TM];
+#pragma unroll
+        for (int mt = 0; mt < TM; ++mt) {
+            const int m = m0 + 16 * mt + fr;
+            const int mm = m < p.M ? m : p.M - 1;
+            const int seq = mm / p.Lout;
+            const int pos = p.row_off + (mm - seq * p.Lout);
+            const int t = pos - p.npre;
+            const bool is_data = t >= 0 && t < p.T;
+            const int tc = t < 0 ? 0 : (t < p.T ? t : p.T - 1);
+            const half_t* xr = is_data ? p.x16 + ((long)seq * p.seq_rows + tc) * PANEL_MERGE_K : reinterpret_cast<const half_t*>(p.zero_row);
+            const float* tok = (p.time_first && pos == 0) ? p.tok_time : p.tok_style + (long)seq * D;
+            const float* rsrc = is_data ? p.st_term + ((long)seq * p.seq_rows + p.npre + tc) * D : (t < 0 ? tok : p.zero_row);
+#pragma unroll
+            for (int kc = 0; kc < KM; ++kc) af[kc][mt] = *reinterpret_cast<const half8*>(xr + 32 * kc + 8 * fq);
+#pragma unroll
+            for (int t_ = 0; t_ < NT; ++t_) acc[t_][mt] = *reinterpret_cast<const float4v*>(rsrc + 16 * t_ + 4 * fq);
+        }
+#pragma unroll
+        for (int kc = 0; kc < KM; ++kc) {
+            const char* base = acquire();
+            stream_frags<NT, PF, TM, RFI>(base, [&](int t, half8 w) {
+#pragma unroll
+                for (int mt = 0; mt < TM; ++mt) acc[t][mt] = MFMA(w, af[kc][mt], acc[t][mt]);
+            }, refill);
+        }
+        store_x();
     } else {
 #pragma unroll
         for (int mt = 0; mt < TM; ++mt)
@@ -342,7 +384,7 @@
             for (int t = 0; t < NT; ++t) acc[t][mt] = *reinterpret_cast<const float4v*>(p.x + grow[mt] * D + 16 * t + 4 * fq);
     }
 
-    if (p.do_skip) {
+    if (DO_SKIP) {
 #pragma unroll
         for (int c = 0; c < KC; ++c)
 #pragma unroll
@@ -383,7 +425,69 @@
         store_x();
     }
 
-    if (p.do_final) {
+    if constexpr (SEAM == PANEL_SEAM_HEAD) {
+        norm_to_xn(vec + V_AN * D, vec + V_BN * D, std::true_type{});
+#pragma unroll
+        for (int t = 0; t < NT; ++t)
+#pragma unroll
+            for (int mt = 0; mt < TM; ++mt) acc[t][mt] = (float4v){0.f, 0.f, 0.f, 0.f};
+#pragma unroll
+        for (int kc = 0; kc < KC; ++kc) {
+            const char* base = acquire();
+            stream_frags<NT, PF, TM, RFI>(base, [&](int t, half8 w) {
+#pragma unroll
+                for (int mt = 0; mt < TM; ++mt) acc[t][mt] = MFMA(w, xn[kc][mt], acc[t][mt]);
+            }, refill);
+        }
+        constexpr float LOG2E = 1.4426950408889634f;
+#pragma unroll
+        for (int c = 0; c < KC; ++c) {
+            const float4v b0 = *reinterpret_cast<const float4v*>(vec + V_AA * D + 32 * c + 4 * fq);
+            const float4v b1 = *reinterpret_cast<const float4v*>(vec + V_AA * D + 32 * c + 16 + 4 * fq);
+#pragma unroll
+            for (int mt = 0; mt < TM; ++mt) {
+                half8 h;
+#pragma unroll
+                for (int j = 0; j < 4; ++j) {
+                    const float a = acc[2 * c][mt][j] + b0[j], b = acc[2 * c + 1][mt][j] + b1[j];
+                    h[j] = (half_t)(a * __builtin_amdgcn_rcpf(1.0f + __builtin_amdgcn_exp2f(-a * LOG2E)));
+                    h[4 + j] = (half_t)(b * __builtin_amdgcn_rcpf(1.0f + __builtin_amdgcn_exp2f(-b * LOG2E)));
+                }
+                xn[c][mt] = h;
+                asm volatile("" : "+v"(xn[c][mt]));
+            }
+        }
+        constexpr int HS = 4;
+        float4v hv[2 * HS][TM];
+#pragma unroll
+        for (int t = 0; t < 2 * HS; ++t)
+#pragma unroll
+            for (int mt = 0; mt < TM; ++mt) hv[t][mt] = (float4v){0.f, 0.f, 0.f, 0.f};
+        const int n_tiles = p.head_C / 16;
+#pragma unroll
+        for (int s = 0; s < HS; ++s) {
+            if (2 * s < n_tiles) {
+                const char* base = acquire();
+                stream_frags<NT, PF, TM, RFI>(base, [&](int f, half8 w) {
+#pragma unroll
+                    for (int mt = 0; mt < TM; ++mt) hv[2 * s + f / KC][mt] = MFMA(w, xn[f % KC][mt], hv[2 * s + f / KC][mt]);
+                }, refill);
+            }
+        }
+#pragma unroll
+        for (int mt = 0; mt < TM; ++mt)
+            if (rok[mt]) {
+#pragma unroll
+                for (int t = 0; t < 2 * HS; ++t)
+                    if (t < n_tiles) {
+                        const float4v b2 = *reinterpret_cast<const float4v*>(vec + V_BA * D + 16 * t + 4 * fq);
+                        float4v o;
+#pragma unroll
+                        for (int j = 0; j < 4; ++j) o[j] = hv[t][mt][j] + b2[j];
+                        *reinterpret_cast<float4v*>(p.v32 + grow[mt] * p.ldv + 16 * t + 4 * fq) = o;
+                    }
+            }
+    } else if (SEAM == PANEL_SEAM_NONE && p.do_final) {
         float rs[TM];
 #pragma unroll
         for (int mt = 0; mt < TM; ++mt) {
@@ -411,8 +515,8 @@
         }
     }
 
-    if (p.do_qkv) {
-        norm_to_xn(vec + V_AA * D, vec + V_BA * D);
+    if (DO_QKV) {
+        norm_to_xn(vec + V_AA * D, vec + V_BA * D, std::bool_constant<SEAM == PANEL_SEAM_MERGE>{});
         float rp[TM][16];
         int posl[TM];
 #pragma unroll
@@ -502,10 +606,13 @@
     asm volatile("s_waitcnt vmcnt(0)" ::: "memory");
 #undef FRAG
 #undef MFMA
+#undef DO_POST
+#undef DO_SKIP
+#undef DO_QKV
 }
 
 __global__ void pack_stream_kernel(half_t* __restrict__ dst, long n_elems, int mode, int D, int I, const float* __restrict__ w0,
-                                   const float* __restrict__ w1, const float* __restrict__ w2) {
+                                   const float* __restrict__ w1, const float* __restrict__ w2, int ldw, int kvalid) {
     const long e = (long)blockIdx.x * blockDim.x + threadIdx.x;
     if (e >= n_elems) return;
     const int NT = D / 16, KC = D / 32;
@@ -534,6 +641,17 @@
         const int kc = (int)(f / NT), t = (int)(f % NT);
         const int k = kc < KC ? 32 * kc + kperm : D + 32 * (kc - KC) + knat;
         v = w0[(long)(16 * t + fr) * (2 * D) + k];
+    } else if (mode == 4) {
+        const int kc = (int)(f / NT), t = (int)(f % NT);
+        const int k = 32 * kc + knat;
+        v = k < kvalid ? w0[(long)(16 * t + fr) * ldw + k] : 0.f;
+    } else if (mode == 5) {
+        const int kc = (int)(f / NT), t = (int)(f % NT);
+        v = w0[(long)(16 * t + fr) * ldw + 32 * kc + kperm];
+    } else if (mode == 6) {
+        const int t = (int)(f / KC), kc = (int)(f % KC);
+        const int n = 16 * t + fr;
+        v = n < kvalid ? w0[(long)n * D + 32 * kc + kperm] : 0.f;
     } else {
         const int grp = (int)(f / (4 * KC)), q = (int)(f % (4 * KC));
         const int kc = q / 4, t = q % 4;
@@ -553,6 +671,13 @@
 static long slots_post(int D, int I) { return D / 32 + 3L * (I / 32); }
 static long slots_skip(int D) { return 2L * (D / 32); }
 static long slots_qkv(int D) { return 2L * (3 * D / 64); }
+
+static long head_slots2(int C) { return (C / 16 + 1) / 2; }
+long fused_seam_slots(int D, int seam, int C) {
+    if (seam == PANEL_SEAM_MERGE) return PANEL_MERGE_K / 32;
+    if (seam == PANEL_SEAM_HEAD) return D / 32 + head_slots2(C);
+    return 0;
+}
 
 long fused_stream_halfs(int D, int I, bool post, bool skip, bool qkv) {
     const long slot_halfs = (long)(D / 16) * 512;
@@ -565,7 +690,7 @@
     long off = 0;
     auto run = [&](int mode, long slots, const float* a, const float* b, const float* c) -> bool {
         const long n = slots * slot_halfs;
-        hipLaunchKernelGGL(pack_stream_kernel, dim3(cdiv(n, 256)), dim3(256), 0, st, dst + off, n, mode, D, I, a, b, c);
+        hipLaunchKernelGGL(pack_stream_kernel, dim3(cdiv(n, 256)), dim3(256), 0, st, dst + off, n, mode, D, I, a, b, c, D, 0);
         off += n;
         return hipGetLastError() == hipSuccess;
     };
@@ -576,6 +701,21 @@
     if (wskip && !run(2, slots_skip(D), wskip, nullptr, nullptr)) return 0;
     if (wqkv && !run(3, slots_qkv(D), wqkv, nullptr, nullptr)) return 0;
     return off;
+}
+
+long fused_pack_merge(half_t* dst, int D, const float* w_merge, int ldw, int C, hipStream_t st) {
+    const long n = fused_seam_slots(D, PANEL_SEAM_MERGE, C) * (D / 16) * 512;
+    hipLaunchKernelGGL(pack_stream_kernel, dim3(cdiv(n, 256)), dim3(256), 0, st, dst, n, 4, D, 0, w_merge, nullptr, nullptr, ldw, C);
+    return hipGetLastError() == hipSuccess ? n : 0;
+}
+
+long fused_pack_head(half_t* dst, int D, const float* wa, const float* w2, int C, hipStream_t st) {
+    const long slot_halfs = (long)(D / 16) * 512;
+    const long n1 = (D / 32) * slot_halfs, n2 = head_slots2(C) * slot_halfs;
+    hipLaunchKernelGGL(pack_stream_kernel, dim3(cdiv(n1, 256)), dim3(256), 0, st, dst, n1, 5, D, 0, wa, nullptr, nullptr, D, D);
+    if (hipGetLastError() != hipSuccess) return 0;
+    hipLaunchKernelGGL(pack_stream_kernel, dim3(cdiv(n2, 256)), dim3(256), 0, st, dst + n1, n2, 6, D, 0, w2, nullptr, nullptr, D, C);
+    return hipGetLastError() == hipSuccess ? n1 + n2 : 0;
 }
 
 int fused_panel_launch(const PanelParams& p, int D, bool gated, hipStream_t st) {
@@ -585,20 +725,40 @@
     DeviceState* ds = device_state();
     if (!ds) return 1;
     if (!ds->fused_attr.load(std::memory_order_acquire)) {
-#define SVC_PANEL_ATTR(DD, GG, TT) SVC_CHECK_HIP(hipFuncSetAttribute(reinterpret_cast<const void*>(dit_panel_kernel<DD, GG, TT>), hipFuncAttributeMaxDynamicSharedMemorySize, PG<DD>::LDS))
+#define SVC_PANEL_ATTR1(DD, GG, TT, SS) SVC_CHECK_HIP(hipFuncSetAttribute(reinterpret_cast<const void*>(dit_panel_kernel<DD, GG, TT, SS>), hipFuncAttributeMaxDynamicSharedMemorySize, PG<DD>::LDS))
+#define SVC_PANEL_ATTR(DD, GG, TT) SVC_PANEL_ATTR1(DD, GG, TT, PANEL_SEAM_NONE); SVC_PANEL_ATTR1(DD, GG, TT, PANEL_SEAM_HEAD); if (!GG) SVC_PANEL_ATTR1(DD, false, TT, PANEL_SEAM_MERGE)
         SVC_PANEL_ATTR(384, false, 1); SVC_PANEL_ATTR(384, true, 1); SVC_PANEL_ATTR(512, false, 1); SVC_PANEL_ATTR(512, true, 1);
         SVC_PANEL_ATTR(384, false, 2); SVC_PANEL_ATTR(384, true, 2); SVC_PANEL_ATTR(512, false, 2); SVC_PANEL_ATTR(512, true, 2);
 #undef SVC_PANEL_ATTR
+#undef SVC_PANEL_ATTR1
         ds->fused_attr.store(true, std::memory_order_release);
     }
-    const long want = (p.do_post ? slots_post(D, p.I) : 0) + (p.do_skip ? slots_skip(D) : 0) + (p.do_qkv ? slots_qkv(D) : 0);
+    if (p.seam == PANEL_SEAM_MERGE) {
+        SVC_REQUIRE(!p.do_post && !p.do_skip && !p.do_final && p.do_qkv && p.row_off == 0, "fused panel kernel: the merge seam belongs to the first panel");
+        SVC_REQUIRE(p.x16 && p.st_term && p.zero_row && p.T >= 1 && p.npre >= 0 && p.npre + p.T <= p.seq_rows, "fused panel kernel: merge seam operands");
+        SVC_REQUIRE(p.npre == 0 || ((p.tok_time || !p.time_first) && (p.tok_style || (p.time_first && p.npre == 1))), "fused panel kernel: merge seam tokens");
+    } else if (p.seam == PANEL_SEAM_HEAD) {
+        SVC_REQUIRE(p.do_post && !p.do_skip && p.do_final && !p.do_qkv && !p.c16, "fused panel kernel: the head seam belongs to the last panel");
+        SVC_REQUIRE(p.head_b0 && p.head_b2 && p.v32 && p.head_C >= 16 && p.head_C % 16 == 0 && p.head_C <= 128 && p.ldv >= p.head_C && p.ldv % 4 == 0,
+                    "fused panel kernel: head seam operands");
+    } else {
+        SVC_REQUIRE(p.seam == PANEL_SEAM_NONE, "fused panel kernel: unknown seam");
+    }
+    const long want = (p.do_post ? slots_post(D, p.I) : 0) + (p.do_skip ? slots_skip(D) : 0) + (p.do_qkv ? slots_qkv(D) : 0) +
+                      fused_seam_slots(D, p.seam, p.head_C);
     SVC_REQUIRE(want == p.n_slots, "fused panel kernel: slot count does not match the enabled phases");
     const int grid = cdiv(p.M, 128);
     const bool prof = prof_enabled();
     if (prof) prof_begin(PROF_FUSED, st);
     static const int tm_env = [] { const char* e = getenv("SVC_FUSED_TM"); return e ? atoi(e) : 0; }();
     const int tm = (tm_env == 1 || tm_env == 2) ? tm_env : (D == 384 ? 2 : 1);
-#define SVC_PANEL_LAUNCH(DD, GG, TT) hipLaunchKernelGGL((dit_panel_kernel<DD, GG, TT>), dim3(grid), dim3(128 / (16 * TT) * 64), PG<DD>::LDS, st, p)
+#define SVC_PANEL_LAUNCH1(DD, GG, TT, SS) hipLaunchKernelGGL((dit_panel_kernel<DD, GG, TT, SS>), dim3(grid), dim3(128 / (16 * TT) * 64), PG<DD>::LDS, st, p)
+#define SVC_PANEL_LAUNCH(DD, GG, TT)                                              \
+    do {                                                                          \
+        if (p.seam == PANEL_SEAM_MERGE) SVC_PANEL_LAUNCH1(DD, false, TT, PANEL_SEAM_MERGE); \
+        else if (p.seam == PANEL_SEAM_HEAD) SVC_PANEL_LAUNCH1(DD, GG, TT, PANEL_SEAM_HEAD); \
+        else SVC_PANEL_LAUNCH1(DD, GG, TT, PANEL_SEAM_NONE);                      \
+    } while (0)
     if (tm == 2) {
         if (D == 384) { if (gated) SVC_PANEL_LAUNCH(384, true, 2); else SVC_PANEL_LAUNCH(384, false, 2); }
         else { if (gated) SVC_PANEL_LAUNCH(512, true, 2); else SVC_PANEL_LAUNCH(512, false, 2); }
@@ -607,6 +767,7 @@
         else { if (gated) SVC_PANEL_LAUNCH(512, true, 1); else SVC_PANEL_LAUNCH(512, false, 1); }
     }
 #undef SVC_PANEL_LAUNCH
+#undef SVC_PANEL_LAUNCH1
     SVC_CHECK_HIP(hipGetLastError());
     if (prof) {
         const double M = p.M, Dd = D;
@@ -614,11 +775,15 @@
         if (p.do_post) macs += Dd * Dd + 3.0 * Dd * p.I;
         if (p.do_skip) macs += 2.0 * Dd * Dd;
         if (p.do_qkv) macs += 3.0 * Dd * Dd;
+        if (p.seam == PANEL_SEAM_MERGE) macs += Dd * (double)PANEL_MERGE_K;
+        if (p.seam == PANEL_SEAM_HEAD) macs += Dd * Dd + Dd * p.head_C;
         double bytes = 2.0 * macs;
         bytes += M * Dd * ((p.do_post ? 4 + 2 : 4) + ((p.do_post && !p.do_skip) || p.do_skip ? 4 : 0) + (p.c16 ? 2 : 0) +
-                           (p.do_skip ? 2 : 0) + (p.do_qkv ? 6 : 0) + (p.do_final ? 2 : 0));
+                           (p.do_skip ? 2 : 0) + (p.do_qkv ? 6 : 0) + (p.do_final && !p.seam ? 2 : 0));
+        if (p.seam == PANEL_SEAM_MERGE) bytes += M * (2.0 * (double)PANEL_MERGE_K + 4.0 * Dd);
+        if (p.seam == PANEL_SEAM_HEAD) bytes += M * (4.0 * p.head_C - 4.0 * Dd);
         const unsigned long long tag = ((unsigned long long)p.M << 40) | ((unsigned long long)(D & 0xFFFFF) << 20) |
-                                       ((unsigned long long)(p.I & 0xFFFF) << 4) |
+                                       ((unsigned long long)((p.I + p.seam) & 0xFFFF) << 4) |
                                        (unsigned)((p.do_post ? 1 : 0) | (p.do_skip ? 2 : 0) | (p.do_qkv ? 4 : 0) | (p.do_final ? 8 : 0));
         prof_end(PROF_FUSED, 2.0 * M * macs, bytes, st, tag);
     }
```

Result: faster. 141,100 mel-frames/s, median of 6 (+1.4%).
